# JGI-Bioinformatics/Kmernator

Hardware: AMD Instinct MI355X
Metric: total k-mers/sec at k=31, 150 bp reads (spectrum build, inputs resident in HBM) (higher is better)
Workload: dtype u64

## Files before the change

### kmernator_amd/csrc/kmr_api.hip

```cpp
#include <hip/hip_runtime.h>
#include <dlfcn.h>
#include <unistd.h>
#include <rccl/rccl.h>

#include <algorithm>
#include <atomic>
#include <cmath>
#include <cstdio>
#include <cstdlib>
#include <cstring>
#include <cctype>
#include <memory>
#include <string>
#include <type_traits>
#include <vector>

#include "../../include/kmernator_amd.h"
#include "kmr_kernels.hpp"
#include "kmr_partition.hpp"
#include "kmr_ingest.hpp"
#include "kmr_artifact.hpp"
#include "kmr_select.hpp"
#include "kmr_pairs.hpp"
#include "kmr_dump.hpp"
#include "kmr_superkmer.hpp"
#include "kmr_buckets.hpp"
#include "kmr_synth.hpp"
#define KMR_INSTANCES_EXTERN
#include "kmr_instances.hpp"

using namespace kmr;

namespace {

std::string g_create_error;

thread_local char g_oom_note[160] = "";
std::atomic<long long> g_blocks_live{0};
hipError_t dev_malloc(void **p, size_t bytes) {
	hipError_t e = hipMalloc(p, bytes);
	if (e == hipSuccess) { if (*p) g_blocks_live++; return e; }
	if (e != hipErrorOutOfMemory) return e;
	size_t fr = 0, tot = 0;
	for (int attempt = 0; attempt < 6; attempt++) {
		(void)hipGetLastError();
		hipDeviceSynchronize();
		if (hipMemGetInfo(&fr, &tot) != hipSuccess || bytes > tot) break;
		usleep(20000u << attempt);
		e = hipMalloc(p, bytes);
		if (e == hipSuccess && *p) g_blocks_live++;
		if (e != hipErrorOutOfMemory) return e;
	}
	(void)hipGetLastError();
	hipMemGetInfo(&fr, &tot);
	snprintf(g_oom_note, sizeof(g_oom_note), " [requested %.3f GB; device has %.3f GB free of %.3f GB]", bytes / 1e9, fr / 1e9, tot / 1e9);
	*p = nullptr;
	return hipErrorOutOfMemory;
}

class DevBuf {
public:
	DevBuf() = default;
	DevBuf(DevBuf &&o) noexcept : p_(o.p_), cap_(o.cap_) { o.p_ = nullptr; o.cap_ = 0; }
	DevBuf &operator=(DevBuf &&o) noexcept { if (this != &o) { reset(); std::swap(p_, o.p_); std::swap(cap_, o.cap_); } return *this; }
	~DevBuf() { reset(); }
	void reset() { if (p_) { hipFree(p_); g_blocks_live--; } p_ = nullptr; cap_ = 0; }
	hipError_t alloc(size_t bytes) {
		reset();
		void *p = nullptr;
		const hipError_t e = dev_malloc(&p, bytes);
		if (e == hipSuccess) { p_ = p; cap_ = bytes; }
		return e;
	}
	int reserve(kmr_handle *h, const char *what, size_t need, size_t bytes = 0);
	template <class T = void> T *get() const { return (T *)p_; }
	size_t cap() const { return cap_; }
	explicit operator bool() const { return p_ != nullptr; }
private:
	void *p_ = nullptr;
	size_t cap_ = 0;
};

struct DevMap {
	uint64_t nb = 0, n = 0;
	DevBuf start;
	DevBuf keys;
	DevBuf vals;
	DevBuf sweight;
	DevBuf spkt;
	DevBuf image;
	bool present = false;
};

struct HostPool {
	DevBuf base, chunk_list, chunk_count, head;
	uint32_t cap = 0; size_t chunk_bytes = 0;
	uint64_t used_ub = 0;
	uint64_t presize = 0;
};

struct HandleMem {
	DevBuf slots, extslots;
	DevBuf dP, dstats, derr;
	DevMap weak, sing;
	DevBuf ix_start, ix_keys, ix_counts;
	DevBuf scratch_stats;
	DevBuf adopt_buf;
	DevBuf trk;
	DevBuf scan_sums;
	DevBuf score_buf;
	DevBuf lut;
	DevBuf dPk;
	DevBuf d_uni;
	DevBuf qrange;
	DevBuf sk_fine_state;
	struct Early { bool active = false; uint64_t hi = 0; uint32_t min_depth = 0; DevBuf ue, cursor, fc, err; } early;
	DevBuf xo_dev;
};
struct BuildMem {
	DevBuf sk_state;
	HostPool l1;
	DevBuf work_counter;
	DevBuf l1_state; bool l1_state_dirty = false;
	DevBuf arena; size_t arena_used = 0, arena_want = 0; std::vector<DevBuf> arena_overflow;
	DevBuf linear;
	DevBuf tile_count, kcap, koff;
	DevBuf ucnt, ufirst, u_start, u_end, u_read, umax;
	DevBuf tb_bases, tb_quals, tb_rel, tb_off, tb_len;
	uint64_t tb_quals_filled = 0; int tb_quals_char = -1;
	DevBuf tb_stage[2][8];
	DevBuf uw_keys, uw_vals, us_keys, us_b8, us_pkt;
	DevBuf ue, ue2;
};
struct ExchangeMem {
	DevBuf xc_small, xc_dcounts;
	DevBuf xc_send, xc_send2, xc_recv, xc_recv2;
};

}

struct Tuning {
	uint64_t target_list = 2048;
	uint64_t sub_batch_bases = 0;
	int recycle = -1;
	int part_blocks = 0;
	double entry_share = -1.0;
	double early_entry_share = -1.0;
	uint64_t saturated_batch_bytes = 0;
	bool no_lut = false, no_narrow = false, no_l1_state = false, no_stream_lookups = false;
	uint64_t long_list_chunks = 0;
	uint64_t binned_min = 1ull << 18;
	uint64_t twobit_piece_bases = 0;
	uint64_t list_aim = 0;
	bool pow2_lists = false;
	bool no_packed_direct = false;
	bool no_uniform_count = false;
	bool no_lean_extract = false;
	bool exchange_fail_once = false;
	uint64_t dump_piece_bytes = 0;
	bool dump_timing = false;
	bool select_timing = false;
	bool pairs_timing = false;
	uint32_t pair_hash_bits = 64;
	bool no_coarse_lists = true;
};

struct kmr_handle : HandleMem, BuildMem, ExchangeMem {
	kmr_config cfg;
	Tuning tune;
	uint32_t k = 0, kb = 0, hkb = 0, W = 0;
	bool ext = false;
	int device = 0, ncu = 0;
	hipStream_t stream = nullptr;
	std::string err;
	uint32_t log2cap = 0;
	uint64_t occupied = 0;
	uint64_t pending_kmers = 0;
	uint64_t stream_base = 0, reads = 0;
	uint64_t nb_weak = 0, nb_sing = 0;
	bool finalized = false, has_singletons = true;
	kmr_handle *subtract = nullptr;
	uint64_t subtracted = 0;
	kmr_stats stats;
	bool partition_mode = false;
	bool superkmer_mode = false;
	uint64_t ix_lists = 0, ix_gen = ~0ull;
	uint64_t trk_n = 0; std::vector<uint64_t> trk_elems;
	long trk_next = 128; uint64_t trk_raw = 0, trk_good = 0; std::vector<unsigned long long> trk_bounds; std::vector<uint64_t> trk_snap_raw, trk_snap_good;
	bool sk_fast_div = false;
	bool sender_launch = false;
	bool sk_exchange = false;
	bool auto_mode = false;
	int bits1 = 0;
	uint64_t inserted_records = 0;
	uint64_t call_bases_hint = 0;
	uint32_t lut_log2 = 0;
	uint64_t lut_gen = ~0ull, map_gen = 0;
	hipStream_t tb_copy_stream = nullptr; hipEvent_t tb_ready[2] = {nullptr, nullptr}, tb_consumed[2] = {nullptr, nullptr}; bool tb_set_used[2] = {false, false};
	const SkPacked *packed_direct = nullptr;
	int uniform_q_hint = -1;
	uint32_t sk_bits = 0, sk_m = 0, sk_off = 0, sk_win = 0;
	double hP[256], hPk[256];
	uint32_t sk_uni_w = 0xffffffffu; bool sk_uni_mixed = false; bool last_count_uniform = false;
	uint32_t peer_uni_w = 0xffffffffu; bool peer_uni_mixed = false, peers_declare = false;
	uint64_t xr_lo = 0, xr_hi = ~0ull;
	uint64_t last_early_hi = 0, last_early_entries = 0;
	bool last_early_overflowed = false;
	double last_score_ms = 0, last_select_ms = 0, last_write_ms = 0;
	double last_dump_size_ms = 0, last_dump_write_ms = 0;
	double last_pairs_ms = 0, last_pairs_parse_ms = 0, last_pairs_sort_ms = 0;
	uint64_t last_pair_hash_collisions = 0;
	uint64_t last_saturated_keys = 0, last_saturated_batches = 0;
	bool qual_mixed = false;
	uint32_t sk_fine_shift = 0;
	uint32_t sk_min_override = 0;
	uint64_t xo_segcap = 0; std::vector<uint64_t> xo_counts; const void *xo_batch = nullptr; uint64_t xo_first = 0;
	void *xc_comm = nullptr; kmr_transport xc_tr = {nullptr, nullptr, nullptr};
	uint64_t xc_job_bases = 0, xc_bytes_to_peers = 0;
	hipEvent_t ev0 = nullptr, ev1 = nullptr;
	double ms[KMR_TIME_GROUPS] = {0};
	uint64_t launches[KMR_TIME_GROUPS] = {0};
	std::vector<std::pair<hipEvent_t, hipEvent_t> > pending_events[KMR_TIME_GROUPS];
};

struct kmr_picks {
	int device = 0;
	DevBuf text, picked;
	uint64_t n = 0, n_picked = 0, bytes = 0;
};

struct kmr_pairs {
	int device = 0;
	DevBuf mate, read1, read2;
	uint64_t n = 0, n_pairs = 0, n_full = 0, n_seq = 0, n_conflicts = 0;
};

struct kmr_text {
	int device = 0;
	DevBuf text;
	uint64_t kept = 0, bytes = 0;
};

struct kmr_reads {
	int device = 0;
	DevBuf bases, quals;
	DevBuf offsets;
	DevBuf name_off, name_len;
	uint64_t n = 0, total = 0, filtered = 0;
	uint32_t input_base = 0;
};

namespace {

std::string oom_note() { std::string s(g_oom_note); g_oom_note[0] = 0; return s; }

std::string hip_err_text(hipError_t e) { return std::string(hipGetErrorString(e)) + (e == hipErrorOutOfMemory ? oom_note() : std::string()); }

#define HIPCHK(h, call) do { hipError_t e_ = (call); if (e_ != hipSuccess) { \
	(h)->err = std::string(#call) + ": " + hip_err_text(e_); \
	return e_ == hipErrorOutOfMemory ? KMR_ERR_OOM : KMR_ERR_HIP; } } while (0)

int DevBuf::reserve(kmr_handle *h, const char *what, size_t need, size_t bytes) {
	if (p_ && cap_ >= need) return 0;
	if (!bytes) bytes = need;
	hipError_t e = p_ ? hipStreamSynchronize(h->stream) : hipSuccess;
	if (e == hipSuccess) e = alloc(bytes);
	if (e == hipSuccess) return 0;
	h->err = std::string("device buffer ") + what + " (" + std::to_string(bytes) + " bytes): " + hip_err_text(e);
	return e == hipErrorOutOfMemory ? KMR_ERR_OOM : KMR_ERR_HIP;
}

#ifdef KMR_DEBUG_HOOKS
bool dbg() { static const bool d = getenv("KMR_DEBUG") != nullptr; return d; }
#else
constexpr bool dbg() { return false; }
#endif

int fail(kmr_handle *h, int code, const std::string &msg) { const std::string m = code == KMR_ERR_OOM ? msg + oom_note() : msg; if (h) h->err = m; else g_create_error = m; return code; }

uint64_t min_pow2(uint64_t n) {
	uint64_t p = n;
	if (p == 0) p = 1;
	else if ((p & (p - 1)) != 0) { p--; for (size_t i = 1; i < 64; i <<= 1) p |= p >> i; p++; }
	return p;
}
uint64_t resize_buckets(uint64_t n) { if (n > 67108864ull) n = 67108864ull; return min_pow2(n); }

void quality_table(double P[256], unsigned minQ, unsigned startChar) {
	for (int raw = 0; raw < 256; raw++) {
		int i = raw - (int)startChar + 33;
		if (i < 33 + (int)minQ) P[raw] = 0.0;
		else if (i < 103) P[raw] = 1.0 - pow(10.0, ((33 - i) / 10.0));
		else P[raw] = 1.0;
	}
}

template <int N> using int_c = std::integral_constant<int, N>;
template <class F> auto with_w(const kmr_handle *h, F &&f) {
	switch (h->W) { case 1: return f(int_c<1>()); case 2: return f(int_c<2>()); case 3: return f(int_c<3>()); default: return f(int_c<4>()); }
}
template <class F> auto with_w_ext(const kmr_handle *h, F &&f) {
	return with_w(h, [&](auto W) { return h->ext ? f(W, std::true_type()) : f(W, std::false_type()); });
}
template <int W, class F> auto with_win(uint32_t win, F &&f) {
	if (W > 1 && win == 32) return f(int_c<(W > 1 ? 32 : 16)>());
	return win == 16 ? f(int_c<16>()) : (win == 8 ? f(int_c<8>()) : f(int_c<4>()));
}

size_t slot_bytes(kmr_handle *h) { return with_w(h, [](auto W) { return sizeof(Slot<W()>); }); }

ReadsView reads_view(const void *bases, const void *quals, const void *offsets, uint64_t n_reads, const void *discarded = nullptr, uint64_t stream_base = 0, uint64_t first_read_idx = 0) {
	ReadsView rv{};
	rv.bases = (const uint8_t *)bases; rv.quals = (const uint8_t *)quals; rv.offsets = (const uint64_t *)offsets; rv.discarded = (const uint8_t *)discarded;
	rv.n_reads = n_reads; rv.stream_base = stream_base; rv.first_read_idx = first_read_idx;
	return rv;
}
ReadsView reads_slice(const ReadsView &all, uint64_t r, uint64_t m) {
	ReadsView rv = all;
	rv.offsets = all.offsets + r; rv.n_reads = m; rv.discarded = all.discarded ? all.discarded + r : nullptr; rv.first_read_idx = all.first_read_idx + r;
	return rv;
}
FinalizeParams finalize_params(kmr_handle *h, uint32_t min_depth) {
	FinalizeParams f{};
	f.kb = h->hkb; f.ext_min_q = h->cfg.ext_min_quality; f.min_depth = min_depth; f.has_singletons = h->cfg.separate_singletons ? 1 : 0; f.nb_weak = h->nb_weak; f.nb_sing = h->nb_sing;
	return f;
}

DevParams dev_params(kmr_handle *h) {
	DevParams p;
	p.k = h->k; p.kb = h->hkb; p.min_weight = h->cfg.min_weight; p.fastq_start = h->cfg.fastq_start_char; p.ext_min_q = h->cfg.ext_min_quality;
	p.qzero = h->cfg.fastq_start_char + std::max<uint32_t>(1u, h->cfg.min_quality_score);
	p.subsample = h->cfg.kmer_subsample; p.rank = h->cfg.rank; p.world = h->cfg.world_size; p.num_parts = h->cfg.num_parts; p.part_idx = h->cfg.part_idx;
	p.count_sender_bad = h->sender_launch ? 1u : 0u;
	p.P = h->dP.get<double>(); p.stats = h->dstats.get<DevStats>(); p.err = h->derr.get<uint32_t>();
	p.sub_wstart = p.sub_wkeys = p.sub_sstart = p.sub_skeys = nullptr; p.sub_wvals = nullptr; p.sub_sweight = nullptr; p.sub_wnb = p.sub_snb = 0; p.sub_vw = 0;
	if (h->subtract) {
		const kmr_handle *o = h->subtract;
		if (o->weak.present && o->weak.n) { p.sub_wstart = o->weak.start.get<uint64_t>(); p.sub_wkeys = o->weak.keys.get<uint64_t>(); p.sub_wvals = o->weak.vals.get<uint32_t>(); p.sub_wnb = o->weak.nb; p.sub_vw = o->ext ? 15 : 3; }
		if (o->sing.present && o->sing.n) { p.sub_sstart = o->sing.start.get<uint64_t>(); p.sub_skeys = o->sing.keys.get<uint64_t>(); p.sub_sweight = o->sing.sweight.get<uint8_t>(); p.sub_snb = o->sing.nb; }
	}
	return p;
}

int grid_for(uint64_t n, int block = 256, int maxBlocks = 256 * 16) {
	uint64_t g = (n + block - 1) / block;
	if (g < 1) g = 1;
	if (g > (uint64_t)maxBlocks) g = maxBlocks;
	return (int)g;
}

template <int W> Table<W> table_of(kmr_handle *h) { Table<W> t; t.slots = h->slots.get<Slot<W>>(); t.ext = h->extslots.get<ExtSlot>(); t.log2cap = h->log2cap; return t; }

template <int W> int clear_table(kmr_handle *h, void *slots, ExtSlot *ext, uint32_t log2cap) {
	hipLaunchKernelGGL(table_clear_kernel<W>, dim3(grid_for(1ull << log2cap)), dim3(256), 0, h->stream, (Slot<W> *)slots, ext, 1ull << log2cap);
	HIPCHK(h, hipGetLastError());
	return 0;
}
int clear_table_any(kmr_handle *h, void *slots, ExtSlot *ext, uint32_t log2cap) { return with_w(h, [&](auto W) { return clear_table<W()>(h, slots, ext, log2cap); }); }

int alloc_table(kmr_handle *h, uint32_t log2cap, DevBuf &slots, DevBuf &ext) {
	DevBuf s, x;
	HIPCHK(h, s.alloc(slot_bytes(h) << log2cap));
	if (h->ext) HIPCHK(h, x.alloc(sizeof(ExtSlot) << log2cap));
	const int rc = clear_table_any(h, s.get(), x.get<ExtSlot>(), log2cap);
	if (rc) return rc;
	slots = std::move(s); ext = std::move(x);
	return 0;
}

int sync_state(kmr_handle *h) {
	HIPCHK(h, hipStreamSynchronize(h->stream));
	for (int which = 0; which < KMR_TIME_GROUPS; which++) {
		for (auto &pr : h->pending_events[which]) {
			float ms = 0; hipEventElapsedTime(&ms, pr.first, pr.second);
			h->ms[which] += ms; h->launches[which]++;
			hipEventDestroy(pr.first); hipEventDestroy(pr.second);
		}
		h->pending_events[which].clear();
	}
	uint32_t e = 0; DevStats s;
	HIPCHK(h, hipMemcpy(&e, h->derr.get<uint32_t>(), sizeof(e), hipMemcpyDeviceToHost));
	HIPCHK(h, hipMemcpy(&s, h->dstats.get<DevStats>(), sizeof(s), hipMemcpyDeviceToHost));
#ifdef KMR_DEBUG_HOOKS
	if (h->superkmer_mode) { if (dbg()) fprintf(stderr, "sk_extract windows: %llu general, %llu fast\n", s.claimed, s.inserted); s.claimed = 0; s.inserted = 0; }
#endif
	h->stats.raw_kmers = s.raw + s.inserted + s.sender_bad; h->stats.raw_good_kmers = s.good + s.inserted; h->stats.discarded = s.raw - s.good + s.sender_bad;
	h->occupied = s.claimed; h->pending_kmers = 0; h->subtracted = s.subtracted;
	if (e & ERR_READ_TOO_LONG) return fail(h, KMR_ERR_UNSUPPORTED, "a read is longer than the per-wavefront LDS tile (" + std::to_string(TILE_SPAN) + " bases)");
	if (e & ERR_TABLE_FULL) return fail(h, KMR_ERR_CAPACITY, "device k-mer table is full; raise kmr_config.max_table_entries / estimated_raw_kmers");
	if (e & ERR_SEGMENT_OVERFLOW) return fail(h, KMR_ERR_CAPACITY, "an owner segment overflowed seg_capacity");
	if (e & ERR_POOL_FULL) return fail(h, KMR_ERR_CAPACITY, "record pool overflow (internal sizing error)");
	if (e & ERR_ENTRIES_FULL) return fail(h, KMR_ERR_CAPACITY, "entry buffer overflow (internal sizing error)");
	return 0;
}

template <int W, bool EXT> int grow_table_t(kmr_handle *h, uint32_t newlog) {
	DevBuf ns, ne;
	int rc = alloc_table(h, newlog, ns, ne);
	if (rc) return rc;
	Table<W> src = table_of<W>(h), dst; dst.slots = ns.get<Slot<W>>(); dst.ext = ne.get<ExtSlot>(); dst.log2cap = newlog;
	hipLaunchKernelGGL((rehash_kernel<W, EXT>), dim3(grid_for(1ull << h->log2cap)), dim3(256), 0, h->stream, src, dst, h->hkb, h->derr.get<uint32_t>());
	HIPCHK(h, hipGetLastError());
	HIPCHK(h, hipStreamSynchronize(h->stream));
	h->slots = std::move(ns); h->extslots = std::move(ne); h->log2cap = newlog;
	return 0;
}
int grow_table(kmr_handle *h, uint32_t newlog) { return with_w_ext(h, [&](auto W, auto EXT) { return grow_table_t<W(), EXT()>(h, newlog); }); }

int ensure_capacity(kmr_handle *h, uint64_t incoming) {
	const uint64_t cap = 1ull << h->log2cap;
	if ((double)(h->occupied + h->pending_kmers + incoming) <= 0.85 * (double)cap) { h->pending_kmers += incoming; return 0; }
	int rc = sync_state(h);
	if (rc) return rc;
	if ((double)(h->occupied + incoming) > 0.85 * (double)cap) {
		uint32_t nl = h->log2cap;
		while ((double)(h->occupied + incoming) > 0.6 * (double)(1ull << nl)) nl++;
		rc = grow_table(h, nl);
		if (rc) return rc;
	}
	h->pending_kmers = incoming;
	return 0;
}

void time_begin(kmr_handle *h, int which, hipEvent_t *a, hipEvent_t *b) {
	hipEventCreate(a); hipEventCreate(b);
	hipEventRecord(*a, h->stream);
	(void)which;
}
void time_end(kmr_handle *h, int which, hipEvent_t a, hipEvent_t b) {
	hipEventRecord(b, h->stream);
	h->pending_events[which].push_back(std::make_pair(a, b));
}

const size_t EXTRACT_SMEM = (size_t)WAVES_PER_BLOCK * 2 * TILE_BUF;

int exclusive_scan(kmr_handle *h, const uint32_t *in, uint64_t n, uint64_t *out);

int prepare_units(kmr_handle *h, ReadsView &rv, uint32_t span = (uint32_t)TILE_SPAN) {
	rv.u_start = rv.u_end = rv.u_read = nullptr; rv.n_units = 0;
	const uint64_t n = rv.n_reads;
	if (n == 0) return 0;
	int rc = h->umax.reserve(h, "umax", 4); if (rc) return rc;
	HIPCHK(h, hipMemsetAsync(h->umax.get<unsigned int>(), 0, 4, h->stream));
	rc = h->ucnt.reserve(h, "ucnt", 4 * (n + 1)); if (rc) return rc;
	hipLaunchKernelGGL(unit_count_kernel, dim3(grid_for(n)), dim3(256), 0, h->stream, rv.offsets, n, h->k, span, h->ucnt.get<uint32_t>(), h->umax.get<unsigned int>());
	HIPCHK(h, hipGetLastError());
	unsigned int mx = 0;
	HIPCHK(h, hipMemcpyAsync(&mx, h->umax.get<unsigned int>(), 4, hipMemcpyDeviceToHost, h->stream));
	HIPCHK(h, hipStreamSynchronize(h->stream));
	if (mx <= span) return 0;
	rc = h->ufirst.reserve(h, "ufirst", 8 * (n + 1)); if (rc) return rc;
	rc = exclusive_scan(h, h->ucnt.get<uint32_t>(), n, h->ufirst.get<uint64_t>()); if (rc) return rc;
	uint64_t U = 0;
	HIPCHK(h, hipMemcpy(&U, h->ufirst.get<uint64_t>() + n, 8, hipMemcpyDeviceToHost));
	if (h->u_read.cap() < 8 * U) {
		h->u_start.reset(); h->u_end.reset(); h->u_read.reset();
		HIPCHK(h, h->u_start.alloc(8 * U)); HIPCHK(h, h->u_end.alloc(8 * U)); HIPCHK(h, h->u_read.alloc(8 * U));
	}
	hipLaunchKernelGGL(unit_fill_kernel, dim3(grid_for(n)), dim3(256), 0, h->stream, rv.offsets, n, h->k, span, h->ufirst.get<uint64_t>(), h->u_start.get<uint64_t>(), h->u_end.get<uint64_t>(), h->u_read.get<uint64_t>());
	HIPCHK(h, hipGetLastError());
	rv.u_start = h->u_start.get<uint64_t>(); rv.u_end = h->u_end.get<uint64_t>(); rv.u_read = h->u_read.get<uint64_t>(); rv.n_units = U;
	return 0;
}

template <int W, bool EXT, class Op> int launch_extract(kmr_handle *h, const ReadsView &rv, const Op &op, uint64_t max_blocks = 0) {
	const DevParams dp = dev_params(h);
	const bool sub = Op::NEEDS_WEIGHT && (dp.sub_wnb | dp.sub_snb) != 0;
	auto kern = sub ? extract_kernel<W, EXT, Op, true> : extract_kernel<W, EXT, Op, false>;
	HIPCHK(h, hipFuncSetAttribute((const void *)kern, hipFuncAttributeMaxDynamicSharedMemorySize, (int)EXTRACT_SMEM));
	if (dbg()) { int nb = 0; hipOccupancyMaxActiveBlocksPerMultiprocessor(&nb, (const void *)kern, WAVES_PER_BLOCK * 64, EXTRACT_SMEM); fprintf(stderr, "extract: %d blocks of %d waves per CU (dynamic LDS %zu)\n", nb, WAVES_PER_BLOCK, EXTRACT_SMEM);
		for (size_t tr : {(size_t)79872, (size_t)65536, (size_t)52000, (size_t)38000}) { hipOccupancyMaxActiveBlocksPerMultiprocessor(&nb, (const void *)kern, WAVES_PER_BLOCK * 64, tr); fprintf(stderr, "   with %zu bytes: %d blocks\n", tr, nb); } }
	const uint64_t tiles = ((rv.u_start ? rv.n_units : rv.n_reads) + 63) / 64;
	uint64_t blocks = (tiles + WAVES_PER_BLOCK - 1) / WAVES_PER_BLOCK;
	if (blocks == 0) return 0;
	if (max_blocks && blocks > max_blocks) blocks = max_blocks;
	if (blocks > 0x7fffffffull) return fail(h, KMR_ERR_INVALID_ARG, "too many reads in one batch");
	hipLaunchKernelGGL(kern, dim3((unsigned)blocks), dim3(WAVES_PER_BLOCK * 64), EXTRACT_SMEM, h->stream, rv, dp, op);
	HIPCHK(h, hipGetLastError());
	return 0;
}

template <int W, bool EXT> int add_reads_dev_t(kmr_handle *h, const ReadsView &rvAll, uint64_t total_bases) {
	const uint64_t n = rvAll.n_reads;
	const uint64_t avg = n ? std::max<uint64_t>(1, total_bases / n) : 1;
	uint64_t chunk = std::max<uint64_t>(64, ((1ull << 27) / avg) & ~63ull);
	std::vector<uint64_t> off2(2);
	for (uint64_t r = 0; r < n; r += chunk) {
		const uint64_t m = std::min(chunk, n - r);
		HIPCHK(h, hipMemcpyAsync(&off2[0], rvAll.offsets + r, 8, hipMemcpyDeviceToHost, h->stream));
		HIPCHK(h, hipMemcpyAsync(&off2[1], rvAll.offsets + r + m, 8, hipMemcpyDeviceToHost, h->stream));
		HIPCHK(h, hipStreamSynchronize(h->stream));
		const uint64_t bases = off2[1] - off2[0];
		int rc = ensure_capacity(h, bases);
		if (rc) return rc;
		ReadsView rv = reads_slice(rvAll, r, m);
		rc = prepare_units(h, rv); if (rc) return rc;
		InsertOp<W, EXT> op; op.table = table_of<W>(h);
		hipEvent_t a, b; time_begin(h, 0, &a, &b);
		rc = launch_extract<W, EXT>(h, rv, op);
		time_end(h, 0, a, b);
		if (rc) return rc;
	}
	return 0;
}

int add_reads_dev_any(kmr_handle *h, const ReadsView &rv, uint64_t total_bases) { return with_w_ext(h, [&](auto W, auto EXT) { return add_reads_dev_t<W(), EXT()>(h, rv, total_bases); }); }

int exclusive_scan(kmr_handle *h, const uint32_t *in, uint64_t n, uint64_t *out ) {
	const uint64_t nblocks = (n + SCAN_ITEMS - 1) / SCAN_ITEMS;
	const size_t eb = sizeof(unsigned long long);
	int rc = h->scan_sums.reserve(h, "scan_sums", eb * (nblocks + 1), eb * std::max<uint64_t>(nblocks + 1, 4096)); if (rc) return rc;
	unsigned long long *sums = h->scan_sums.get<unsigned long long>(), *total = sums + nblocks;
	hipLaunchKernelGGL(scan_block_sums_kernel, dim3((unsigned)nblocks), dim3(256), 0, h->stream, in, n, sums);
	hipLaunchKernelGGL(scan_sums_kernel, dim3(1), dim3(256), 0, h->stream, sums, nblocks, total);
	hipLaunchKernelGGL(scan_apply_kernel, dim3((unsigned)nblocks), dim3(256), 0, h->stream, in, n, sums, out);
	HIPCHK(h, hipGetLastError());
	HIPCHK(h, hipStreamSynchronize(h->stream));
	return 0;
}

int arena_alloc(kmr_handle *h, void **out, size_t bytes) {
	const size_t need = (bytes + 255) & ~(size_t)255;
	if (h->arena && h->arena_used + need <= h->arena.cap()) { *out = h->arena.get<uint8_t>() + h->arena_used; h->arena_used += need; h->arena_want += need; return 0; }
	h->arena_want += need;
	DevBuf b;
	HIPCHK(h, b.alloc(std::max<size_t>(need, 256)));
	*out = b.get();
	h->arena_overflow.push_back(std::move(b));
	return 0;
}
int arena_reset(kmr_handle *h) {
	HIPCHK(h, hipStreamSynchronize(h->stream));
	h->arena_overflow.clear();
	if (h->arena_want > h->arena.cap()) {
		if (h->arena.alloc(h->arena_want + h->arena_want / 8 + (1 << 20)) != hipSuccess) (void)hipGetLastError();
	}
	h->arena_used = 0; h->arena_want = 0;
	return 0;
}
template <class T> int arena_get(kmr_handle *h, T **out, size_t count) { return arena_alloc(h, (void **)out, count * sizeof(T)); }

void clear_map(DevMap &m) { m.image.reset(); m.n = 0; m.present = false; }


template <int W> MapView<W> view_of(const DevMap &m, uint32_t vw) {
	MapView<W> v; v.start = m.start.get<uint64_t>(); v.keys = m.keys.get<uint64_t>(); v.vals = m.vals.get<uint32_t>(); v.sweight = m.sweight.get<uint8_t>(); v.nb = m.present ? m.nb : 0; v.vw = vw;
	return v;
}

template <int W, bool EXT> int finalize_t(kmr_handle *h, uint32_t min_depth) {
	int rc = sync_state(h);
	if (rc) return rc;
	hipEvent_t ea, eb; time_begin(h, 1, &ea, &eb);
	const FinalizeParams f = finalize_params(h, min_depth);
	const bool keepSing = f.has_singletons && min_depth <= 1;
	DevBuf wcb, scb, fcb;
	HIPCHK(h, wcb.alloc(4 * h->nb_weak)); HIPCHK(h, scb.alloc(4 * h->nb_sing)); HIPCHK(h, fcb.alloc(sizeof(FinalizeCounters)));
	uint32_t *wc = wcb.get<uint32_t>(), *sc = scb.get<uint32_t>(); FinalizeCounters *fc = fcb.get<FinalizeCounters>();
	HIPCHK(h, hipMemsetAsync(wc, 0, 4 * h->nb_weak, h->stream)); HIPCHK(h, hipMemsetAsync(sc, 0, 4 * h->nb_sing, h->stream)); HIPCHK(h, hipMemsetAsync(fc, 0, sizeof(FinalizeCounters), h->stream));
	Table<W> t = table_of<W>(h);
	const int g = grid_for(1ull << h->log2cap);
	hipLaunchKernelGGL(classify_kernel<W>, dim3(g), dim3(256), 0, h->stream, t, f, wc, sc, fc);
	HIPCHK(h, hipGetLastError());
	FinalizeCounters c;
	HIPCHK(h, hipMemcpyAsync(&c, fc, sizeof(c), hipMemcpyDeviceToHost, h->stream));
	HIPCHK(h, hipStreamSynchronize(h->stream));
	h->stats.unique_kmers = c.unique;
	h->stats.singleton_kmers = f.has_singletons ? c.singletons : 0;
	DevMap &wm = h->weak, &sm = h->sing;
	wm = DevMap(); sm = DevMap();
	wm.nb = h->nb_weak; wm.n = c.weak_kept; wm.present = true;
	sm.nb = h->nb_sing; sm.n = c.sing_kept; sm.present = keepSing;
	const uint32_t vw = EXT ? 15 : 3;
	HIPCHK(h, wm.start.alloc(8 * (wm.nb + 1))); HIPCHK(h, sm.start.alloc(8 * (sm.nb + 1)));
	rc = exclusive_scan(h, wc, wm.nb, wm.start.get<uint64_t>()); if (rc) return rc;
	rc = exclusive_scan(h, sc, sm.nb, sm.start.get<uint64_t>()); if (rc) return rc;
	HIPCHK(h, wm.keys.alloc(std::max<uint64_t>(8, 8ull * W * wm.n))); HIPCHK(h, wm.vals.alloc(std::max<uint64_t>(8, 4ull * vw * wm.n)));
	HIPCHK(h, sm.keys.alloc(std::max<uint64_t>(8, 8ull * W * sm.n))); HIPCHK(h, sm.sweight.alloc(std::max<uint64_t>(8, sm.n)));
	if (EXT) HIPCHK(h, sm.spkt.alloc(std::max<uint64_t>(8, 4ull * sm.n)));
	HIPCHK(h, hipMemsetAsync(wc, 0, 4 * h->nb_weak, h->stream)); HIPCHK(h, hipMemsetAsync(sc, 0, 4 * h->nb_sing, h->stream));
	hipLaunchKernelGGL((scatter_kernel<W, EXT>), dim3(g), dim3(256), 0, h->stream, t, f, wm.start.get<uint64_t>(), wc, wm.keys.get<uint64_t>(), wm.vals.get<uint32_t>(), sm.start.get<uint64_t>(), sc, sm.keys.get<uint64_t>(), sm.sweight.get<uint8_t>(), sm.spkt.get<uint32_t>());
	HIPCHK(h, hipGetLastError());
	SortView<W> sv; sv.keys = wm.keys.get<uint64_t>(); sv.vals = wm.vals.get<uint32_t>(); sv.b8 = nullptr; sv.pkt = nullptr; sv.vw = vw;
	hipLaunchKernelGGL((sort_buckets_kernel<W, EXT ? 15 : 3>), dim3(grid_for(wm.nb, 4, 1 << 20)), dim3(256), 0, h->stream, sv, wm.start.get<uint64_t>(), wm.nb);
	if (sm.n) {
		SortView<W> ss; ss.keys = sm.keys.get<uint64_t>(); ss.vals = nullptr; ss.b8 = sm.sweight.get<uint8_t>(); ss.pkt = sm.spkt.get<uint32_t>(); ss.vw = 0;
		hipLaunchKernelGGL((sort_buckets_kernel<W, 0>), dim3(grid_for(sm.nb, 4, 1 << 20)), dim3(256), 0, h->stream, ss, sm.start.get<uint64_t>(), sm.nb);
	}
	HIPCHK(h, hipGetLastError());
	time_end(h, 1, ea, eb);
	HIPCHK(h, hipStreamSynchronize(h->stream));
	h->has_singletons = keepSing;
	if (!keepSing) { sm.n = 0; }
	h->stats.weak_entries = wm.n; h->stats.singleton_entries = keepSing ? sm.n : 0;
	h->finalized = true; h->map_gen++;
	return sync_state(h);
}

template <int W> int build_image_t(kmr_handle *h, DevMap &m, bool weakMap) {
	if (m.image) return 0;
	const uint32_t vw = h->ext ? 15 : 3;
	const uint32_t vbytes = weakMap ? (h->ext ? 60 : 12) : (h->ext ? 5 : 1);
	HIPCHK(h, m.image.alloc(8 * (2 + m.nb) + 4 * m.nb + m.n * (h->kb + vbytes)));
	hipLaunchKernelGGL(image_header_kernel, dim3(grid_for(m.nb)), dim3(256), 0, h->stream, m.image.get<uint8_t>(), m.start.get<uint64_t>(), m.nb, h->kb, vbytes);
	if (m.n) hipLaunchKernelGGL(image_entries_kernel<W>, dim3(grid_for(m.n)), dim3(256), 0, h->stream, m.image.get<uint8_t>(), m.start.get<uint64_t>(), m.nb, h->kb, vbytes,
	                           m.keys.get<uint64_t>(), weakMap ? m.vals.get<uint32_t>() : nullptr, vw, m.sweight.get<uint8_t>(), m.spkt.get<uint32_t>(), m.n);
	HIPCHK(h, hipGetLastError());
	HIPCHK(h, hipStreamSynchronize(h->stream));
	return 0;
}
int build_image(kmr_handle *h, DevMap &m, bool weakMap) { return with_w(h, [&](auto W) { return build_image_t<W()>(h, m, weakMap); }); }

template <int W> int load_image_t(kmr_handle *h, DevMap &m, bool weakMap, const uint8_t *src, uint64_t len) {
	if (len < 16) return fail(h, KMR_ERR_INVALID_ARG, "image too short");
	uint64_t nb, mask; memcpy(&nb, src, 8); memcpy(&mask, src + 8, 8);
	if (nb == 0 || (nb & (nb - 1)) || mask != nb - 1 || len < 8 * (2 + nb) + 4 * nb) return fail(h, KMR_ERR_INVALID_ARG, "bad image header");
	const uint32_t vw = h->ext ? 15 : 3;
	const uint32_t vbytes = weakMap ? (h->ext ? 60 : 12) : (h->ext ? 5 : 1);
	if ((len - 8 * (2 + nb) - 4 * nb) % (h->kb + vbytes) != 0) return fail(h, KMR_ERR_INVALID_ARG, "image size does not match k / value type");
	m = DevMap();
	m.nb = nb; m.n = (len - 8 * (2 + nb) - 4 * nb) / (h->kb + vbytes); m.present = true;
	const uint64_t *offs = (const uint64_t *)(src + 16);
	uint64_t expect = 8 * (2 + nb);
	for (uint64_t b = 0; b < nb; b++) {
		if (offs[b] != expect || expect + 4 > len) return fail(h, KMR_ERR_INVALID_ARG, "image offsets are not the packed store() layout");
		uint32_t cnt; memcpy(&cnt, src + expect, 4);
		expect += 4 + (uint64_t)cnt * (h->kb + vbytes);
		if (expect > len) return fail(h, KMR_ERR_INVALID_ARG, "image bucket runs past the end");
	}
	if (expect != len) return fail(h, KMR_ERR_INVALID_ARG, "image length mismatch");
	HIPCHK(h, m.image.alloc(len));
	HIPCHK(h, hipMemcpy(m.image.get<uint8_t>(), src, len, hipMemcpyHostToDevice));
	{
		DevBuf counts; HIPCHK(h, counts.alloc(4 * nb));
		hipLaunchKernelGGL(image_counts_kernel, dim3(grid_for(nb)), dim3(256), 0, h->stream, m.image.get<uint8_t>(), nb, counts.get<uint32_t>());
		HIPCHK(h, m.start.alloc(8 * (nb + 1)));
		int rc = exclusive_scan(h, counts.get<uint32_t>(), nb, m.start.get<uint64_t>()); if (rc) return rc;
	}
	HIPCHK(h, m.keys.alloc(std::max<uint64_t>(8, 8ull * W * m.n)));
	if (weakMap) HIPCHK(h, m.vals.alloc(std::max<uint64_t>(8, 4ull * vw * m.n)));
	else { HIPCHK(h, m.sweight.alloc(std::max<uint64_t>(8, m.n))); if (h->ext) HIPCHK(h, m.spkt.alloc(std::max<uint64_t>(8, 4 * m.n))); }
	if (m.n) hipLaunchKernelGGL(image_unpack_kernel<W>, dim3(grid_for(m.n)), dim3(256), 0, h->stream, m.image.get<uint8_t>(), m.start.get<uint64_t>(), nb, h->kb, vbytes, m.keys.get<uint64_t>(), m.vals.get<uint32_t>(), vw, m.sweight.get<uint8_t>(), m.spkt.get<uint32_t>(), m.n);
	SortView<W> sv; sv.keys = m.keys.get<uint64_t>(); sv.vals = m.vals.get<uint32_t>(); sv.b8 = m.sweight.get<uint8_t>(); sv.pkt = m.spkt.get<uint32_t>(); sv.vw = weakMap ? vw : 0;
	if (!weakMap) hipLaunchKernelGGL((sort_buckets_kernel<W, 0>), dim3(grid_for(nb, 4, 1 << 20)), dim3(256), 0, h->stream, sv, m.start.get<uint64_t>(), nb);
	else if (h->ext) hipLaunchKernelGGL((sort_buckets_kernel<W, 15>), dim3(grid_for(nb, 4, 1 << 20)), dim3(256), 0, h->stream, sv, m.start.get<uint64_t>(), nb);
	else hipLaunchKernelGGL((sort_buckets_kernel<W, 3>), dim3(grid_for(nb, 4, 1 << 20)), dim3(256), 0, h->stream, sv, m.start.get<uint64_t>(), nb);
	HIPCHK(h, hipGetLastError());
	HIPCHK(h, hipStreamSynchronize(h->stream));
	m.image.reset();

	return 0;
}

template <int W, int VW> void launch_sort(kmr_handle *h, DevMap &m, bool weakMap) {
	SortView<W> sv; sv.keys = m.keys.get<uint64_t>(); sv.vals = weakMap ? m.vals.get<uint32_t>() : nullptr; sv.b8 = m.sweight.get<uint8_t>(); sv.pkt = m.spkt.get<uint32_t>(); sv.vw = weakMap ? VW : 0;
	hipLaunchKernelGGL((sort_buckets_kernel<W, VW>), dim3(grid_for(m.nb, 4, 1 << 20)), dim3(256), 0, h->stream, sv, m.start.get<uint64_t>(), m.nb);
}
template <int W> int merge_image_t(kmr_handle *h, DevMap &m, bool weakMap, const uint8_t *src, uint64_t len) {
	DevMap t;
	int rc = load_image_t<W>(h, t, weakMap, src, len);
	if (rc) return rc;
	if (t.nb != m.nb) return fail(h, KMR_ERR_INVALID_ARG, "Can not merge two maps of differing sizes (src/Kmer.h:3210)");
	const uint32_t vw = h->ext ? 15 : 3;
	DevMap d; d.nb = m.nb; d.n = m.n + t.n; d.present = true;
	DevBuf countsb, dupb;
	HIPCHK(h, countsb.alloc(4 * m.nb)); HIPCHK(h, dupb.alloc(4));
	uint32_t *counts = countsb.get<uint32_t>(), *dup = dupb.get<uint32_t>();
	HIPCHK(h, hipMemsetAsync(dup, 0, 4, h->stream));
	HIPCHK(h, d.start.alloc(8 * (m.nb + 1)));
	hipLaunchKernelGGL(merge_counts_kernel, dim3(grid_for(m.nb)), dim3(256), 0, h->stream, m.start.get<uint64_t>(), t.start.get<uint64_t>(), m.nb, counts);
	rc = exclusive_scan(h, counts, m.nb, d.start.get<uint64_t>()); if (rc) return rc;
	HIPCHK(h, d.keys.alloc(std::max<uint64_t>(8, 8ull * W * d.n)));
	if (weakMap) HIPCHK(h, d.vals.alloc(std::max<uint64_t>(8, 4ull * vw * d.n)));
	else { HIPCHK(h, d.sweight.alloc(std::max<uint64_t>(8, d.n))); if (h->ext) HIPCHK(h, d.spkt.alloc(std::max<uint64_t>(8, 4 * d.n))); }
	if (m.n) hipLaunchKernelGGL(merge_copy_kernel<W>, dim3(grid_for(m.n)), dim3(256), 0, h->stream, m.start.get<uint64_t>(), t.start.get<uint64_t>(), false, m.nb, m.n, m.keys.get<uint64_t>(), weakMap ? m.vals.get<uint32_t>() : nullptr, vw, m.sweight.get<uint8_t>(), m.spkt.get<uint32_t>(), d.start.get<uint64_t>(), d.keys.get<uint64_t>(), d.vals.get<uint32_t>(), d.sweight.get<uint8_t>(), d.spkt.get<uint32_t>());
	if (t.n) hipLaunchKernelGGL(merge_copy_kernel<W>, dim3(grid_for(t.n)), dim3(256), 0, h->stream, t.start.get<uint64_t>(), m.start.get<uint64_t>(), true, m.nb, t.n, t.keys.get<uint64_t>(), weakMap ? t.vals.get<uint32_t>() : nullptr, vw, t.sweight.get<uint8_t>(), t.spkt.get<uint32_t>(), d.start.get<uint64_t>(), d.keys.get<uint64_t>(), d.vals.get<uint32_t>(), d.sweight.get<uint8_t>(), d.spkt.get<uint32_t>());
	if (!weakMap) launch_sort<W, 0>(h, d, false); else if (h->ext) launch_sort<W, 15>(h, d, true); else launch_sort<W, 3>(h, d, true);
	hipLaunchKernelGGL(duplicate_keys_kernel<W>, dim3(grid_for(d.nb)), dim3(256), 0, h->stream, d.start.get<uint64_t>(), d.nb, d.keys.get<uint64_t>(), dup);
	HIPCHK(h, hipGetLastError());
	uint32_t hdup = 0;
	HIPCHK(h, hipMemcpyAsync(&hdup, dup, 4, hipMemcpyDeviceToHost, h->stream)); HIPCHK(h, hipStreamSynchronize(h->stream));
	if (hdup && !weakMap) return fail(h, KMR_ERR_UNSUPPORTED, "the two singleton maps share k-mers: merging them means promoting those into the weak map (mergePromote, which the reference refuses too)");
	if (hdup) {
		DevMap d2; d2.nb = d.nb; d2.present = true;
		hipLaunchKernelGGL(merge_distinct_kernel<W>, dim3(grid_for(d.nb)), dim3(256), 0, h->stream, d.start.get<uint64_t>(), d.nb, d.keys.get<uint64_t>(), counts);
		HIPCHK(h, d2.start.alloc(8 * (d.nb + 1)));
		rc = exclusive_scan(h, counts, d.nb, d2.start.get<uint64_t>()); if (rc) return rc;
		HIPCHK(h, hipMemcpyAsync(&d2.n, d2.start.get<uint64_t>() + d.nb, 8, hipMemcpyDeviceToHost, h->stream)); HIPCHK(h, hipStreamSynchronize(h->stream));
		HIPCHK(h, d2.keys.alloc(std::max<uint64_t>(8, 8ull * W * d2.n)));
		HIPCHK(h, d2.vals.alloc(std::max<uint64_t>(8, 4ull * vw * d2.n)));
		hipLaunchKernelGGL(merge_add_kernel<W>, dim3(grid_for(d.nb)), dim3(256), 0, h->stream, d.start.get<uint64_t>(), d.nb, d.keys.get<uint64_t>(), d.vals.get<uint32_t>(), vw, d2.start.get<uint64_t>(), d2.keys.get<uint64_t>(), d2.vals.get<uint32_t>());
		HIPCHK(h, hipGetLastError()); HIPCHK(h, hipStreamSynchronize(h->stream));
		d = std::move(d2);
	}
	m = std::move(d);
	return 0;
}

template <int W> int lookup_t(kmr_handle *h, const uint8_t *packed, uint64_t n, uint32_t *counts, double *weights = nullptr) {
	const uint64_t ob = counts ? 4 : 8;
	DevBuf dk, dc;
	HIPCHK(h, dk.alloc(std::max<uint64_t>(8, n * h->kb))); HIPCHK(h, dc.alloc(std::max<uint64_t>(8, ob * n)));
	HIPCHK(h, hipMemcpyAsync(dk.get(), packed, n * h->kb, hipMemcpyHostToDevice, h->stream));
	const uint32_t vw = h->ext ? 15 : 3;
	hipLaunchKernelGGL(lookup_keys_kernel<W>, dim3(grid_for(n)), dim3(256), 0, h->stream, view_of<W>(h->weak, vw), view_of<W>(h->sing, vw), dk.get<uint8_t>(), n, h->hkb,
	                   counts ? dc.get<uint32_t>() : nullptr, counts ? nullptr : dc.get<double>());
	HIPCHK(h, hipGetLastError());
	HIPCHK(h, hipMemcpyAsync(counts ? (void *)counts : (void *)weights, dc.get(), ob * n, hipMemcpyDeviceToHost, h->stream));
	HIPCHK(h, hipStreamSynchronize(h->stream));
	return 0;
}

template <int W> LutView<W> lut_of(kmr_handle *h) {
	LutView<W> v; v.slots = nullptr; v.mask = 0; v.shift = 0;
	if (h->tune.no_lut || !h->weak.present || h->weak.n == 0) return v;
	if (!(h->lut && h->lut_gen == h->map_gen)) {
		uint32_t l2 = 10; while ((1ull << l2) < 2 * h->weak.n) l2++;
		const size_t bytes = (size_t)(W + 1) * 8 << l2;
		if (h->lut.cap() < bytes) {
			if (h->lut) { hipStreamSynchronize(h->stream); h->lut.reset(); }
			size_t fr = 0, tot = 0;
			if (hipMemGetInfo(&fr, &tot) != hipSuccess || fr < bytes + (1ull << 30) || h->lut.alloc(bytes) != hipSuccess) { (void)hipGetLastError(); return v; }
		}

		const uint32_t vw = h->ext ? 15 : 3;
		hipLaunchKernelGGL(lut_clear_kernel, dim3(4096), dim3(256), 0, h->stream, h->lut.get<uint64_t>(), 1ull << l2, (uint32_t)(W + 1));
		hipLaunchKernelGGL(lut_build_kernel<W>, dim3(grid_for(h->weak.n)), dim3(256), 0, h->stream, view_of<W>(h->weak, vw), h->weak.n, h->lut.get<uint64_t>(), (1ull << l2) - 1, 64 - l2, h->hkb);
		if (hipGetLastError() != hipSuccess) return v;
		h->lut_log2 = l2; h->lut_gen = h->map_gen;
	}
	v.slots = h->lut.get<uint64_t>(); v.mask = (1ull << h->lut_log2) - 1; v.shift = 64 - h->lut_log2;
	return v;
}

template <int W> int lookup_reads_t(kmr_handle *h, const ReadsView &rv, uint32_t *dout, const uint64_t *dout_off, bool weak_only = false) {
	LookupOp<W> op; const uint32_t vw = h->ext ? 15 : 3; op.weak_only = weak_only;
	op.lut = weak_only ? lut_of<W>(h) : LutView<W>{nullptr, 0, 0};
	op.weak = view_of<W>(h->weak, vw); op.sing = view_of<W>(h->sing, vw); op.out = dout; op.out_offsets = dout_off; op.first_read_idx = rv.first_read_idx;
	return launch_extract<W, false>(h, rv, op);
}
template <int W> int lookup_reads_weighted_t(kmr_handle *h, const ReadsView &rv, double *dout, const uint64_t *dout_off) {
	LookupWeightOp<W> op; const uint32_t vw = h->ext ? 15 : 3;
	op.weak = view_of<W>(h->weak, vw); op.sing = view_of<W>(h->sing, vw); op.out = dout; op.out_offsets = dout_off; op.first_read_idx = rv.first_read_idx;
	return launch_extract<W, false>(h, rv, op);
}

int stage_reads(kmr_handle *h, const char *bases, const uint64_t *offsets, uint64_t n, DevBuf &b, DevBuf &o) {
	const uint64_t total = n ? offsets[n] - offsets[0] : 0;
	HIPCHK(h, b.alloc(total + 64)); HIPCHK(h, o.alloc(8 * (n + 1)));
	HIPCHK(h, hipMemcpyAsync(b.get(), bases + (n ? offsets[0] : 0), total, hipMemcpyHostToDevice, h->stream));
	std::vector<uint64_t> rel(n + 1);
	for (uint64_t i = 0; i <= n; i++) rel[i] = n ? offsets[i] - offsets[0] : 0;
	HIPCHK(h, hipMemcpyAsync(o.get(), rel.data(), 8 * (n + 1), hipMemcpyHostToDevice, h->stream));
	HIPCHK(h, hipStreamSynchronize(h->stream));
	return 0;
}


#define TARGET_LIST_RECORDS (h->tune.target_list)
const double MAX_LIST_DISTINCT = 600.0;
const uint64_t L2_ITEM_CHUNKS = 16384;
const uint64_t SUB_BATCH_BASES = 1ull << 30;

size_t rec_bytes(kmr_handle *h) { return h->superkmer_mode ? 16 : 8 * h->W + (h->ext ? 16 : 8); }
uint64_t key_entries(kmr_handle *h, const DevBuf &keys) { return keys.cap() / (8ull * h->W); }
uint64_t packed_entries(kmr_handle *h, const DevBuf &ue) { return ue.cap() / (8ull * (h->W + 1)); }
int max_part_bits(kmr_handle *h) { return rec_bytes(h) <= 24 ? 10 : 9; }
PoolView pool_view(kmr_handle *h, HostPool &p) { PoolView v; v.base = p.base.get<uint8_t>(); v.chunk_list = p.chunk_list.get<uint32_t>(); v.chunk_count = p.chunk_count.get<uint32_t>(); v.head = p.head.get<unsigned int>(); v.cap = p.cap; v.err = h->derr.get<uint32_t>(); return v; }
uint32_t part_rot(kmr_handle *h) { uint32_t r = 0; while ((1ull << (r + 1)) <= h->nb_weak) r++; return r; }
template <int W, bool EXT, int LEVEL> int launch_partition(kmr_handle *h, const PartSource<W> &S, HostPool &pool, int grid, int bits, int shift) {
	auto kern = partition_direct_kernel<W, EXT, LEVEL, PD_THREADS, PD_RPT, PD_LINE>;
	const size_t smem = partition_direct_smem_bytes<W, EXT, PD_THREADS, PD_RPT, PD_LINE>(bits);
	if (dbg()) fprintf(stderr, "partition level %d W=%d bits=%d shift=%d smem=%zu grid=%d\n", LEVEL, W, bits, shift, smem, grid);
	HIPCHK(h, hipFuncSetAttribute((const void *)kern, hipFuncAttributeMaxDynamicSharedMemorySize,
	                              (int)partition_direct_smem_bytes<W, EXT, PD_THREADS, PD_RPT, PD_LINE>(max_part_bits(h))));
	hipLaunchKernelGGL(kern, dim3(grid), dim3(PD_THREADS), smem, h->stream, S, pool_view(h, pool), h->work_counter.get<unsigned int>(), bits, shift);
	HIPCHK(h, hipGetLastError());
	return 0;
}

int pool_reserve(kmr_handle *h, HostPool &p, uint64_t extra, bool keep) {
	unsigned int used = 0;
	if (!keep) p.used_ub = 0;
	if (p.head && keep) {
		if (p.base && p.used_ub + extra + 64 <= p.cap) { p.used_ub += extra; return 0; }
		HIPCHK(h, hipStreamSynchronize(h->stream)); HIPCHK(h, hipMemcpy(&used, p.head.get<unsigned int>(), 4, hipMemcpyDeviceToHost)); if (used > p.cap) used = p.cap;
	}
	p.used_ub = (uint64_t)used + extra;
	const uint64_t need = (uint64_t)used + extra + 64;
	if (need >= 0xffffffffull) return fail(h, KMR_ERR_CAPACITY, "record pool would exceed 2^32 chunks");
	if (!p.head) { HIPCHK(h, p.head.alloc(4)); HIPCHK(h, hipMemset(p.head.get(), 0, 4)); }
	if (!keep) HIPCHK(h, hipMemsetAsync(p.head.get<unsigned int>(), 0, 4, h->stream));
	if (need <= p.cap) return 0;
	uint64_t ncap = keep && used ? need + need / 4 : need;
	if (p.presize && need + p.presize < 0xffffffffull) ncap = std::max(ncap, need + p.presize);
	p.presize = 0;
	p.chunk_bytes = (size_t)CH * rec_bytes(h);
	DevBuf nb, nl, nc;
	HIPCHK(h, nb.alloc(ncap * p.chunk_bytes));
	HIPCHK(h, nl.alloc(4 * ncap)); HIPCHK(h, nc.alloc(4 * ncap));
	if (used) {
		HIPCHK(h, hipMemcpy(nb.get(), p.base.get(), (size_t)used * p.chunk_bytes, hipMemcpyDeviceToDevice));
		HIPCHK(h, hipMemcpy(nl.get(), p.chunk_list.get(), 4ull * used, hipMemcpyDeviceToDevice));
		HIPCHK(h, hipMemcpy(nc.get(), p.chunk_count.get(), 4ull * used, hipMemcpyDeviceToDevice));
		HIPCHK(h, hipDeviceSynchronize());
	}
	p.base = std::move(nb); p.chunk_list = std::move(nl); p.chunk_count = std::move(nc); p.cap = (uint32_t)ncap;
	return 0;
}


int zero_work_counter(kmr_handle *h) {
	int rc = h->work_counter.reserve(h, "work_counter", 4); if (rc) return rc;
	HIPCHK(h, hipMemsetAsync(h->work_counter.get<unsigned int>(), 0, 4, h->stream));
	return 0;
}

int num_cus(kmr_handle *h) {
	if (h->ncu <= 0) {
		hipDeviceProp_t pr; h->ncu = 256;
		if (hipGetDeviceProperties(&pr, h->device) == hipSuccess) h->ncu = pr.multiProcessorCount;
	}
	return h->ncu;
}
int part_grid(kmr_handle *h) { return num_cus(h) * 2; }
int partition_blocks(kmr_handle *h) { return h->tune.part_blocks > 0 ? h->tune.part_blocks : num_cus(h); }

template <int W, bool EXT> int ensure_l1_state(kmr_handle *h) {
	const size_t stride = partition_state_bytes<W, EXT, PD_LINE>(h->bits1), need = stride * (size_t)partition_blocks(h);
	if (h->l1_state.cap() == need) return 0;
	if (h->l1_state) HIPCHK(h, hipStreamSynchronize(h->stream));
	HIPCHK(h, h->l1_state.alloc(need));
	hipLaunchKernelGGL(partition_state_init_kernel, dim3(partition_blocks(h)), dim3(256), 0, h->stream, h->l1_state.get<uint8_t>(), stride, h->bits1, (uint32_t)partition_blocks(h));
	HIPCHK(h, hipGetLastError());
	h->l1_state_dirty = false;
	return 0;
}
template <int W, bool EXT> int flush_l1_state(kmr_handle *h) {
	if (!h->l1_state || !h->l1_state_dirty) return 0;
	int rc = pool_reserve(h, h->l1, (uint64_t)partition_blocks(h) * ((1ull << h->bits1) + 512) + 64, true); if (rc) return rc;
	rc = zero_work_counter(h); if (rc) return rc;
	PartSource<W> S; memset(&S, 0, sizeof(S));
	S.kb = h->hkb; S.rot = part_rot(h); S.state = h->l1_state.get<uint8_t>(); S.state_final = 1;
	rc = launch_partition<W, EXT, 1>(h, S, h->l1, partition_blocks(h), h->bits1, 0);
	h->l1_state_dirty = false;
	return rc;
}

template <int W, bool EXT> int partition_level1(kmr_handle *h, const void *linear, const uint64_t *ext_start, const uint32_t *ext_count,
                                      uint64_t n_ext, uint32_t ext_stride, uint64_t ext_len, uint64_t total, uint64_t max_records,
                                      unsigned long long *valid_counter = nullptr, uint32_t packed_words = 0, uint64_t ordinal_base = 0) {
	if (n_ext == 0) return 0;
	const int grid = (int)std::min<uint64_t>(partition_blocks(h), n_ext);
	if (!h->l1.base) {
		const uint64_t est = std::max<uint64_t>(max_records, h->cfg.estimated_raw_kmers / std::max<uint32_t>(1, h->cfg.world_size));
		const uint64_t launches = est / std::max<uint64_t>(1, max_records) + 2;
		const uint64_t l2_allowance = (est / CH / L2_ITEM_CHUNKS + (1ull << h->bits1) + 1) * (1ull << max_part_bits(h)) + (uint64_t)part_grid(h) * 512;
		{
			const uint64_t chunks = est / CH + launches * (uint64_t)grid * ((1ull << h->bits1) + 512) + 64 + l2_allowance;
			size_t mfree = 0, mtotal = 0;
			if (hipMemGetInfo(&mfree, &mtotal) == hipSuccess && (double)mfree < (double)chunks * CH * rec_bytes(h) * 1.02 + (double)(2ull << 30)) {
				HIPCHK(h, hipStreamSynchronize(h->stream));
				h->uw_keys.reset(); h->uw_vals.reset(); h->us_keys.reset(); h->us_b8.reset(); h->us_pkt.reset(); h->ue.reset(); h->ue2.reset();
			}
		}
		uint64_t want = est / CH + launches * (uint64_t)grid * ((1ull << h->bits1) + 512) + 64 + l2_allowance;
		{
			size_t mfree = 0, mtotal = 0;
			const double twice = (double)(want + est / CH) * CH * rec_bytes(h) * 1.02;
			if (hipMemGetInfo(&mfree, &mtotal) == hipSuccess && twice + (double)(8ull << 30) < (double)mfree * 0.5) want += est / CH;
		}
		int rc0 = pool_reserve(h, h->l1, want, true);
		if (rc0) return rc0;
	}
	int rc = pool_reserve(h, h->l1, max_records / CH + (uint64_t)grid * ((1ull << h->bits1) + 512) + 64, true);
	if (rc) return rc;
	rc = zero_work_counter(h); if (rc) return rc;
	PartSource<W> S; memset(&S, 0, sizeof(S));
	S.linear = linear; S.ext_start = ext_start; S.ext_count = ext_count; S.n_ext = n_ext; S.ext_stride = ext_stride; S.ext_len = ext_len; S.total = total;
	S.valid_counter = valid_counter; S.kb = h->hkb; S.rot = part_rot(h); S.packed_words = packed_words; S.ordinal_base = ordinal_base;
	if (!h->tune.no_l1_state) {
		rc = ensure_l1_state<W, EXT>(h); if (rc) return rc;
		S.state = h->l1_state.get<uint8_t>(); S.state_final = 0; h->l1_state_dirty = true;
	}
	hipEvent_t ta, tb; time_begin(h, KMR_TIME_PARTITION1, &ta, &tb);
	rc = launch_partition<W, EXT, 1>(h, S, h->l1, grid, h->bits1, 0);
	time_end(h, KMR_TIME_PARTITION1, ta, tb);
	return rc;
}

void choose_bits1(kmr_handle *h, uint64_t records_hint) {
	uint64_t est = std::max<uint64_t>(records_hint, h->cfg.estimated_raw_kmers / std::max<uint32_t>(1, h->cfg.world_size));
	const int mb = max_part_bits(h);
	int T = 0; while (T < 2 * mb && (est >> T) > TARGET_LIST_RECORDS) T++;
	h->bits1 = std::max(0, std::min(mb, T + 2 - mb));
}

template <int W, bool EXT> int extract_by_owner_t(kmr_handle *h, const ReadsView &rvAll, uint64_t total_bases, void *dev_records, uint64_t seg_capacity, void *dev_seg_counts, uint32_t *dev_pos = nullptr) {
	const uint64_t n = rvAll.n_reads;
	const uint64_t avg = n ? std::max<uint64_t>(1, total_bases / n) : 1;
	const uint64_t chunk = std::max<uint64_t>(64, (SUB_BATCH_BASES / avg) & ~63ull);
	for (uint64_t r = 0; r < n; r += chunk) {
		const uint64_t m = std::min(chunk, n - r);
		ReadsView rv = reads_slice(rvAll, r, m);
		int rc = prepare_units(h, rv); if (rc) return rc;
		const uint64_t nu = rv.u_start ? rv.n_units : m;
		rc = h->kcap.reserve(h, "kcap", 4 * std::max<uint64_t>(nu + 1, 16)); if (rc) return rc;
		rc = h->koff.reserve(h, "koff", 8 * std::max<uint64_t>(nu + 1, 16)); if (rc) return rc;
		hipLaunchKernelGGL(kmer_capacity_kernel, dim3(grid_for(nu)), dim3(256), 0, h->stream, rv, h->k, h->kcap.get<uint32_t>());
		HIPCHK(h, hipGetLastError());
		rc = exclusive_scan(h, h->kcap.get<uint32_t>(), nu, h->koff.get<uint64_t>()); if (rc) return rc;
		uint64_t total_cap = 0;
		HIPCHK(h, hipMemcpy(&total_cap, h->koff.get<uint64_t>() + nu, 8, hipMemcpyDeviceToHost));
		const uint64_t tiles = (nu + 63) / 64;
		rc = h->linear.reserve(h, "linear", sizeof(typename PoolRec<W, EXT>::type) * std::max<uint64_t>(total_cap, 16)); if (rc) return rc;
		rc = h->tile_count.reserve(h, "tile_count", 4 * std::max<uint64_t>(tiles, 16)); if (rc) return rc;
		LinearOp<W, EXT, false> op; op.records = (typename PoolRec<W, EXT>::type *)h->linear.get(); op.koff = h->koff.get<uint64_t>(); op.tile_count = h->tile_count.get<uint32_t>(); op.first_read_idx = rv.first_read_idx;
		h->sender_launch = dev_pos == nullptr;
		rc = launch_extract<W, EXT>(h, rv, op);
		h->sender_launch = false;
		if (rc) return rc;
		rc = zero_work_counter(h); if (rc) return rc;
		const int grid = (int)std::min<uint64_t>((uint64_t)num_cus(h) * 8, tiles);
		OwnerFn of; of.m = 0; of.off = of.win = of.list_bits = 0;
		if (h->superkmer_mode && h->sk_exchange) { of.m = h->sk_m; of.off = h->sk_off; of.win = h->sk_win; of.list_bits = h->sk_bits; }
		if (dev_pos)
			hipLaunchKernelGGL((owner_scatter_kernel<W, EXT, true>), dim3(grid), dim3(OWNER_THREADS), 0, h->stream, (const typename PoolRec<W, EXT>::type *)h->linear.get(), h->koff.get<uint64_t>(), h->tile_count.get<uint32_t>(), tiles, h->hkb,
			                   h->cfg.world_size, (uint32_t *)dev_records, seg_capacity, (unsigned long long *)dev_seg_counts, h->work_counter.get<unsigned int>(), h->derr.get<uint32_t>(), dev_pos, of);
		else
			hipLaunchKernelGGL((owner_scatter_kernel<W, EXT>), dim3(grid), dim3(OWNER_THREADS), 0, h->stream, (const typename PoolRec<W, EXT>::type *)h->linear.get(), h->koff.get<uint64_t>(), h->tile_count.get<uint32_t>(), tiles, h->hkb,
			                   h->cfg.world_size, (uint32_t *)dev_records, seg_capacity, (unsigned long long *)dev_seg_counts, h->work_counter.get<unsigned int>(), h->derr.get<uint32_t>(), (uint32_t *)nullptr, of);
		HIPCHK(h, hipGetLastError());
	}
	return 0;
}

template <int W, bool EXT> int add_reads_partition_t(kmr_handle *h, const ReadsView &rvAll, uint64_t total_bases) {
	const uint64_t n = rvAll.n_reads;
	if (!h->l1.head) choose_bits1(h, total_bases);
	const uint64_t avg = n ? std::max<uint64_t>(1, total_bases / n) : 1;
	const uint64_t sub_bases = h->tune.sub_batch_bases ? h->tune.sub_batch_bases : SUB_BATCH_BASES;
	const uint64_t chunk = std::max<uint64_t>(64, (sub_bases / avg) & ~63ull);
	for (uint64_t r = 0; r < n; r += chunk) {
		const uint64_t m = std::min(chunk, n - r);
		ReadsView rv = reads_slice(rvAll, r, m);
		int rc = prepare_units(h, rv); if (rc) return rc;
		const uint64_t nu = rv.u_start ? rv.n_units : m;
		rc = h->kcap.reserve(h, "kcap", 4 * std::max<uint64_t>(nu + 1, 16)); if (rc) return rc;
		rc = h->koff.reserve(h, "koff", 8 * std::max<uint64_t>(nu + 1, 16)); if (rc) return rc;
		hipLaunchKernelGGL(kmer_capacity_kernel, dim3(grid_for(nu)), dim3(256), 0, h->stream, rv, h->k, h->kcap.get<uint32_t>());
		HIPCHK(h, hipGetLastError());
		rc = exclusive_scan(h, h->kcap.get<uint32_t>(), nu, h->koff.get<uint64_t>()); if (rc) return rc;
		uint64_t total_cap = 0;
		HIPCHK(h, hipMemcpy(&total_cap, h->koff.get<uint64_t>() + nu, 8, hipMemcpyDeviceToHost));
		const uint64_t tiles = (nu + 63) / 64;
		rc = h->linear.reserve(h, "linear", rec_bytes(h) * std::max<uint64_t>(total_cap, 16)); if (rc) return rc;
		rc = h->tile_count.reserve(h, "tile_count", 4 * std::max<uint64_t>(tiles, 16)); if (rc) return rc;
		LinearOp<W, EXT> op; op.records = (typename PoolRec<W, EXT>::type *)h->linear.get(); op.koff = h->koff.get<uint64_t>(); op.tile_count = h->tile_count.get<uint32_t>(); op.first_read_idx = rv.first_read_idx;
		hipEvent_t a, b, a2, b2; time_begin(h, KMR_TIME_BUILD, &a, &b);
		time_begin(h, KMR_TIME_EXTRACT, &a2, &b2);
		rc = launch_extract<W, EXT>(h, rv, op);
		time_end(h, KMR_TIME_EXTRACT, a2, b2);
#ifdef KMR_DEBUG_HOOKS
		if (!rc && getenv("KMR_DEBUG_SAME_TILE")) {
			const uint64_t distinct = std::max<uint64_t>(1, strtoull(getenv("KMR_DEBUG_SAME_TILE"), nullptr, 10));
			hipLaunchKernelGGL(same_tile_kernel, dim3(grid_for(tiles)), dim3(256), 0, h->stream, h->koff.get<uint64_t>(), tiles, distinct, total_cap / std::max<uint64_t>(tiles, 1));
		}
#endif
		if (!rc) rc = partition_level1<W, EXT>(h, h->linear.get(), h->koff.get<uint64_t>(), h->tile_count.get<uint32_t>(), tiles, 64, 0, 0, total_cap);
		time_end(h, KMR_TIME_BUILD, a, b);
		if (rc) return rc;
	}
	return 0;
}
int add_reads_partition(kmr_handle *h, const ReadsView &rv, uint64_t total_bases) { return with_w_ext(h, [&](auto W, auto EXT) { return add_reads_partition_t<W(), EXT()>(h, rv, total_bases); }); }

int build_csr(kmr_handle *h, HostPool &p, uint64_t nl, uint32_t first, uint64_t **list_start, uint64_t **list_chunks, uint32_t *n_chunks_out) {
	unsigned int used = 0;
	HIPCHK(h, hipStreamSynchronize(h->stream));
	HIPCHK(h, hipMemcpy(&used, p.head.get<unsigned int>(), 4, hipMemcpyDeviceToHost));
	if (used > p.cap) used = p.cap;
	used = used > first ? used - first : 0;
	uint32_t *cnt;
	{ int arc = arena_get(h, &cnt, nl); if (arc) return arc; arc = arena_get(h, list_start, nl + 1); if (arc) return arc;
	  arc = arena_get(h, list_chunks, std::max<unsigned>(used, 1)); if (arc) return arc; }
	HIPCHK(h, hipMemsetAsync(cnt, 0, 4 * nl, h->stream));
	const unsigned csr_grid = (unsigned)(((uint64_t)used + CSR_THREADS * CSR_ITEMS - 1) / (CSR_THREADS * CSR_ITEMS));
	if (used) hipLaunchKernelGGL(chunk_hist_kernel, dim3(csr_grid), dim3(CSR_THREADS), 0, h->stream, p.chunk_list.get<uint32_t>() + first, used, cnt, (uint32_t)nl);
	int rc = exclusive_scan(h, cnt, nl, *list_start); if (rc) return rc;
	HIPCHK(h, hipMemsetAsync(cnt, 0, 4 * nl, h->stream));
	if (used) hipLaunchKernelGGL(chunk_scatter_kernel, dim3(csr_grid), dim3(CSR_THREADS), 0, h->stream, p.chunk_list.get<uint32_t>() + first, p.chunk_count.get<uint32_t>() + first, used, first, *list_start, cnt, *list_chunks, (uint32_t)nl);
	HIPCHK(h, hipGetLastError());
	*n_chunks_out = used;
	if (dbg()) {
		unsigned long long hv[2] = {0, 0};
		DevBuf db; HIPCHK(h, db.alloc(16)); HIPCHK(h, hipMemset(db.get(), 0, 16));
		unsigned long long *d = db.get<unsigned long long>();
		if (used) hipLaunchKernelGGL(pool_records_kernel, dim3(grid_for(used)), dim3(256), 0, h->stream, p.chunk_list.get<uint32_t>(), p.chunk_count.get<uint32_t>(), used, d, d + 1);
		HIPCHK(h, hipStreamSynchronize(h->stream));
		HIPCHK(h, hipMemcpy(hv, d, 16, hipMemcpyDeviceToHost));
		fprintf(stderr, "build_csr: lists %llu chunks %u valid %llu records %llu (expected %llu)\n", (unsigned long long)nl, used, hv[1], hv[0], (unsigned long long)h->stats.raw_good_kmers);
		unsigned long long vv[3] = {0, 0, 0};
		int bits = 0; while ((1ull << bits) < nl) bits++;
		DevBuf vb; HIPCHK(h, vb.alloc(24)); HIPCHK(h, hipMemset(vb.get(), 0, 24));
		unsigned long long *v = vb.get<unsigned long long>();
		PoolView pvw = pool_view(h, p);
		with_w_ext(h, [&](auto W, auto EXT) { hipLaunchKernelGGL((verify_lists_kernel<W(), EXT()>), dim3(4096), dim3(256), 0, h->stream, pvw, *list_start, *list_chunks, nl, bits, h->hkb, part_rot(h), v, v + 1, v + 2); });
		HIPCHK(h, hipStreamSynchronize(h->stream));
		HIPCHK(h, hipMemcpy(vv, v, 24, hipMemcpyDeviceToHost));
		fprintf(stderr, "verify_lists: records via CSR %llu misfiled %llu zero-weight %llu\n", vv[0], vv[1], vv[2]);
	}
	return 0;
}

int finish_maps_from_entries(kmr_handle *h, uint32_t *wc, uint32_t *sc, uint64_t wslots, uint64_t sslots, uint64_t wn, uint64_t sn, bool keepSing, bool weak_uncounted = false);
CountOut count_out(kmr_handle *h, bool packed, unsigned long long *cursors, uint32_t *wc, uint32_t *sc, FinalizeCounters *fc);

template <int W, bool EXT, int LOG2S, bool NARROW = false> int launch_count(kmr_handle *h, int grid, const uint64_t *ls, const uint64_t *lc, uint64_t nl, const CountOut &out, const FinalizeParams &f, int list_filter) {
	auto kern = count_kernel<W, EXT, LOG2S, NARROW>;
	const size_t smem = count_smem_bytes<W, EXT, LOG2S, NARROW>();
	HIPCHK(h, hipFuncSetAttribute((const void *)kern, hipFuncAttributeMaxDynamicSharedMemorySize, (int)smem));
	hipLaunchKernelGGL(kern, dim3(grid), dim3(COUNT_THREADS), smem, h->stream, pool_view(h, h->l1), ls, lc, nl, out, f, h->work_counter.get<unsigned int>(), list_filter);
	return 0;
}

template <int W, bool EXT> int finalize_partition_t(kmr_handle *h, uint32_t min_depth) {
	int rc = sync_state(h);
	if (rc) return rc;
	hipEvent_t ea, eb; time_begin(h, 1, &ea, &eb);
	const uint64_t G = h->stats.raw_good_kmers;
	const FinalizeParams f = finalize_params(h, min_depth);
	const bool keepSing = f.has_singletons && min_depth <= 1;
	if (!h->l1.head) { rc = pool_reserve(h, h->l1, 0, false); if (rc) return rc; }
	rc = arena_reset(h); if (rc) return rc;
	rc = flush_l1_state<W, EXT>(h); if (rc) return rc;
	const uint64_t nl1 = 1ull << h->bits1;
	uint64_t *ls1 = nullptr; uint64_t *lc1 = nullptr; uint32_t nch1 = 0;
	rc = build_csr(h, h->l1, nl1, 0, &ls1, &lc1, &nch1); if (rc) return rc;
	double distinct_share = 1.0, repeated_share = 0.5;
	if (G) {
		unsigned long long *dpr, hpr[4] = {0, 0, 0, 0};
		const uint32_t n_probes = (uint32_t)std::min<uint64_t>(PROBE_LISTS, nl1);
		const size_t tbytes = 8 * ((size_t)n_probes * PROBE_SLOTS + 4);
		rc = arena_alloc(h, (void **)&dpr, tbytes); if (rc) return rc;
		HIPCHK(h, hipMemsetAsync(dpr, 0, tbytes, h->stream));
		hipLaunchKernelGGL((distinct_probe_kernel<W, EXT>), dim3(n_probes * PROBE_SPLIT), dim3(256), 0, h->stream, pool_view(h, h->l1), ls1, lc1, nl1, h->hkb, part_rot(h),
		                   (int)h->bits1, n_probes, dpr + 4, dpr);
		HIPCHK(h, hipGetLastError());
		HIPCHK(h, hipMemcpyAsync(hpr, dpr, 32, hipMemcpyDeviceToHost, h->stream)); HIPCHK(h, hipStreamSynchronize(h->stream));
		if (hpr[0] >= 256) { distinct_share = std::min(1.0, std::max(0.01, (double)hpr[1] / (double)hpr[0])); repeated_share = std::min(0.5, (double)hpr[2] / (double)hpr[0]); }
		if (dbg()) fprintf(stderr, "distinct probe: %llu records, %llu distinct (%llu repeated) -> shares %.3f %.3f\n", hpr[0], hpr[1], hpr[2], distinct_share, repeated_share);
	}
	const int mb = max_part_bits(h);
	int T = 0; while (T < 40 && ((G >> T) > TARGET_LIST_RECORDS || (double)(G >> T) * distinct_share > MAX_LIST_DISTINCT)) T++;
	T = std::min(T, 28);
	int cur_bits = h->bits1;
	uint64_t *ls2 = ls1, *lc2 = lc1;
	uint32_t valid_from = 0;
	for (int level = 2; cur_bits < T; level++) {
		const int nbits = std::min(mb, T - cur_bits);
		const uint64_t nl_prev = 1ull << cur_bits;
		std::vector<uint64_t> hs(nl_prev + 1);
		HIPCHK(h, hipMemcpy(hs.data(), ls2, 8 * (nl_prev + 1), hipMemcpyDeviceToHost));
		std::vector<uint64_t> ib, ie; std::vector<uint32_t> il;
		for (uint64_t l = 0; l < nl_prev; l++) {
			const uint64_t nch = hs[l + 1] - hs[l];
			if (!nch) continue;
			const uint64_t nit = (nch + L2_ITEM_CHUNKS - 1) / L2_ITEM_CHUNKS, per = (nch + nit - 1) / nit;
			for (uint64_t c = hs[l]; c < hs[l + 1]; c += per) { ib.push_back(c); ie.push_back(std::min(hs[l + 1], c + per)); il.push_back((uint32_t)l); }
		}
		if (ib.empty()) { cur_bits += nbits; rc = build_csr(h, h->l1, 1ull << cur_bits, valid_from, &ls2, &lc2, &nch1); if (rc) return rc; continue; }
		const uint64_t partials = ib.size() * (1ull << nbits) + (uint64_t)part_grid(h) * 512 + 64;
		unsigned int head_before = 0;
		HIPCHK(h, hipMemcpy(&head_before, h->l1.head.get<unsigned int>(), 4, hipMemcpyDeviceToHost));
		const bool recycle = h->tune.recycle >= 0 ? h->tune.recycle != 0 : (uint64_t)head_before + G / CH + partials + 64 > h->l1.cap;
		h->l1.used_ub = head_before;
		rc = pool_reserve(h, h->l1, (recycle ? 0 : G / CH) + partials, true); if (rc) return rc;
		uint64_t *dib, *die; uint32_t *dil;
		rc = arena_get(h, &dib, ib.size()); if (rc) return rc; rc = arena_get(h, &die, ie.size()); if (rc) return rc; rc = arena_get(h, &dil, il.size()); if (rc) return rc;
		HIPCHK(h, hipMemcpyAsync(dib, ib.data(), 8 * ib.size(), hipMemcpyHostToDevice, h->stream)); HIPCHK(h, hipMemcpyAsync(die, ie.data(), 8 * ie.size(), hipMemcpyHostToDevice, h->stream));
		HIPCHK(h, hipMemcpyAsync(dil, il.data(), 4 * il.size(), hipMemcpyHostToDevice, h->stream));
		rc = zero_work_counter(h); if (rc) return rc;
		PartSource<W> S; memset(&S, 0, sizeof(S));
		S.src = pool_view(h, h->l1); S.list_chunks = lc2; S.item_begin = dib; S.item_end = die; S.item_list = dil; S.n_items = ib.size(); S.kb = h->hkb; S.rot = part_rot(h);
		S.recycle = recycle ? 1 : 0;
		const int grid = (int)std::min<uint64_t>(partition_blocks(h), ib.size());
		if (dbg()) fprintf(stderr, "level %d: %d bits after %d, %zu items, %s\n", level, nbits, cur_bits, ib.size(), recycle ? "recycling chunks" : "fresh chunks");
		hipEvent_t ta, tb; time_begin(h, KMR_TIME_PARTITION2, &ta, &tb);
		rc = launch_partition<W, EXT, 2>(h, S, h->l1, grid, nbits, cur_bits);
		time_end(h, KMR_TIME_PARTITION2, ta, tb);
		if (rc) return rc;
		HIPCHK(h, hipStreamSynchronize(h->stream));
		cur_bits += nbits;
		if (!recycle) valid_from = head_before;
		rc = build_csr(h, h->l1, 1ull << cur_bits, valid_from, &ls2, &lc2, &nch1); if (rc) return rc;
	}
	const uint64_t nl2 = 1ull << cur_bits;
	const int count_log2s = (!EXT && (double)(G >> cur_bits) * distinct_share > MAX_LIST_DISTINCT) ? 11 : COUNT_LOG2S;
	if (dbg()) fprintf(stderr, "count pass: %llu lists of ~%llu records, table 2^%d\n", (unsigned long long)nl2, (unsigned long long)(G >> cur_bits), count_log2s);
	const uint32_t vw = EXT ? 15 : 3;
	const uint64_t slack = (uint64_t)part_grid(h) * 8 * 8192 + 16;
	const uint64_t wbound = f.has_singletons ? G / 2 : G, sbound = keepSing ? G : 0;
	const uint64_t wmax = wbound + wbound / 8 + slack, smax = keepSing ? sbound + sbound / 8 + slack : 16;
	uint64_t wcap = std::min<uint64_t>(wmax, (uint64_t)((double)G * (f.has_singletons ? repeated_share : distinct_share) * 1.5) + G / 64 + slack);
	uint64_t scap = keepSing ? std::min<uint64_t>(smax, (uint64_t)((double)G * std::max(0.0, distinct_share - repeated_share) * 1.5) + G / 64 + slack) : 16;
	if (h->tune.entry_share >= 0) {
		const double sh = h->tune.entry_share;
		wcap = std::min<uint64_t>(wmax, (uint64_t)((double)G * sh) + 16384); if (keepSing) scap = std::min<uint64_t>(smax, (uint64_t)((double)G * sh) + 16384);
		h->uw_keys.reset(); h->uw_vals.reset(); h->us_keys.reset(); h->us_b8.reset(); h->us_pkt.reset();
	}
	wcap = std::max(wcap, key_entries(h, h->uw_keys)); scap = std::max(scap, key_entries(h, h->us_keys));
	uint32_t *wc = nullptr, *sc = nullptr; FinalizeCounters *fc = nullptr; unsigned long long *cursors = nullptr;
	rc = arena_get(h, &wc, h->nb_weak); if (rc) return rc; rc = arena_get(h, &sc, h->nb_sing); if (rc) return rc;
	rc = arena_get(h, &fc, 1); if (rc) return rc; rc = arena_get(h, &cursors, 2); if (rc) return rc;
	FinalizeCounters c; unsigned long long cur[2];
	hipEvent_t tca, tcb; time_begin(h, KMR_TIME_COUNT, &tca, &tcb);
	for (int attempt = 0; ; attempt++) {
	{
		const double need = (key_entries(h, h->uw_keys) < wcap ? (8.0 * W + 4.0 * vw) * (double)wcap : 0.0) + (key_entries(h, h->us_keys) < scap ? (8.0 * W + 1.0) * (double)scap : 0.0);
		size_t mfree = 0, mtotal = 0;
		if (need > 0 && h->linear && hipMemGetInfo(&mfree, &mtotal) == hipSuccess && (double)mfree < need + (double)G * 0.3 * (8.0 * W + 12.0) + (double)(2ull << 30)) {
			HIPCHK(h, hipStreamSynchronize(h->stream));
			h->linear.reset();
		}
	}
	if (key_entries(h, h->uw_keys) < wcap || !h->uw_vals) {
		h->uw_keys.reset(); h->uw_vals.reset();
		HIPCHK(h, h->uw_keys.alloc(8ull * W * wcap)); HIPCHK(h, h->uw_vals.alloc(4ull * vw * wcap));
	}
	if (key_entries(h, h->us_keys) < scap || !h->us_b8 || (EXT && !h->us_pkt)) {
		h->us_keys.reset(); h->us_b8.reset(); h->us_pkt.reset();
		HIPCHK(h, h->us_keys.alloc(8ull * W * scap)); HIPCHK(h, h->us_b8.alloc(scap)); if (EXT) HIPCHK(h, h->us_pkt.alloc(4 * scap));
	}
	HIPCHK(h, hipMemsetAsync(wc, 0, 4 * h->nb_weak, h->stream)); HIPCHK(h, hipMemsetAsync(sc, 0, 4 * h->nb_sing, h->stream));
	HIPCHK(h, hipMemsetAsync(fc, 0, sizeof(FinalizeCounters), h->stream)); HIPCHK(h, hipMemsetAsync(cursors, 0, 16, h->stream));
	const CountOut out = count_out(h, false, cursors, wc, sc, fc);
	rc = zero_work_counter(h); if (rc) return rc;
	#ifdef KMR_DEBUG_HOOKS
	const int count_reps = getenv("KMR_COUNT_CHECK") ? atoi(getenv("KMR_COUNT_CHECK")) : 0;
#else
	const int count_reps = 0;
#endif
	for (int cr = 0; cr <= count_reps; cr++) {
		if (cr) {
			FinalizeCounters c0; unsigned long long cur0[2];
			HIPCHK(h, hipStreamSynchronize(h->stream));
			HIPCHK(h, hipMemcpy(&c0, fc, sizeof(c0), hipMemcpyDeviceToHost)); HIPCHK(h, hipMemcpy(cur0, cursors, 16, hipMemcpyDeviceToHost));
			fprintf(stderr, "count pass %d: unique %llu singletons %llu weak_kept %llu sing_kept %llu slots %llu/%llu\n", cr - 1, (unsigned long long)c0.unique,
			        (unsigned long long)c0.singletons, (unsigned long long)c0.weak_kept, (unsigned long long)c0.sing_kept, cur0[0], cur0[1]);
			HIPCHK(h, hipMemsetAsync(wc, 0, 4 * h->nb_weak, h->stream)); HIPCHK(h, hipMemsetAsync(sc, 0, 4 * h->nb_sing, h->stream));
			HIPCHK(h, hipMemsetAsync(fc, 0, sizeof(FinalizeCounters), h->stream)); HIPCHK(h, hipMemsetAsync(cursors, 0, 16, h->stream));
			rc = zero_work_counter(h); if (rc) return rc;
		}
		const int grid = (int)std::min<uint64_t>((uint64_t)part_grid(h) * 2, nl2);
		if (count_log2s == 11) {
			rc = launch_count<W, EXT, 11>(h, grid, ls2, lc2, nl2, out, f, 0); if (rc) return rc;
		} else if (EXT && W == 1 && !h->tune.no_narrow) {
			rc = launch_count<W, EXT, COUNT_LOG2S, true>(h, grid, ls2, lc2, nl2, out, f, 1); if (rc) return rc;
			HIPCHK(h, hipGetLastError());
			rc = zero_work_counter(h); if (rc) return rc;
			hipLaunchKernelGGL(max_list_chunks_kernel, dim3(grid_for(nl2)), dim3(256), 0, h->stream, ls2, nl2, h->work_counter.get<unsigned int>());
			unsigned int longest = 0;
			HIPCHK(h, hipMemcpyAsync(&longest, h->work_counter.get<unsigned int>(), 4, hipMemcpyDeviceToHost, h->stream));
			HIPCHK(h, hipStreamSynchronize(h->stream));
			rc = zero_work_counter(h); if (rc) return rc;
			if (longest > COUNT_NARROW_CHUNKS) { rc = launch_count<W, EXT, COUNT_LOG2S>(h, std::min(grid, part_grid(h)), ls2, lc2, nl2, out, f, 2); if (rc) return rc; }
		} else {
			rc = launch_count<W, EXT, COUNT_LOG2S>(h, grid, ls2, lc2, nl2, out, f, 0); if (rc) return rc;
		}
		HIPCHK(h, hipGetLastError());
	}
	uint32_t cerr = 0;
	HIPCHK(h, hipMemcpyAsync(&c, fc, sizeof(c), hipMemcpyDeviceToHost, h->stream)); HIPCHK(h, hipMemcpyAsync(cur, cursors, 16, hipMemcpyDeviceToHost, h->stream));
	HIPCHK(h, hipMemcpyAsync(&cerr, h->derr.get<uint32_t>(), 4, hipMemcpyDeviceToHost, h->stream));
	HIPCHK(h, hipStreamSynchronize(h->stream));
	if (!(cerr & ERR_ENTRIES_FULL) || (wcap >= wmax && scap >= smax) || attempt >= 8) break;
	cerr &= ~(uint32_t)ERR_ENTRIES_FULL;
	HIPCHK(h, hipMemcpy(h->derr.get<uint32_t>(), &cerr, 4, hipMemcpyHostToDevice));
	wcap = std::min<uint64_t>(wmax, wcap * 2); if (keepSing) scap = std::min<uint64_t>(smax, scap * 2);
	if (dbg()) fprintf(stderr, "count pass: entry buffers too small, retrying with %llu / %llu\n", (unsigned long long)wcap, (unsigned long long)scap);
	}
	time_end(h, KMR_TIME_COUNT, tca, tcb);
	{
		uint32_t cerr2 = 0;
		HIPCHK(h, hipMemcpy(&cerr2, h->derr.get<uint32_t>(), 4, hipMemcpyDeviceToHost));
		if (cerr2 & ERR_ENTRIES_FULL) { time_end(h, 1, ea, eb); return fail(h, KMR_ERR_CAPACITY, "entry buffers of the count pass overflowed at their upper bound (internal sizing error)"); }
	}

	h->stats.unique_kmers = c.unique;
	h->stats.singleton_kmers = f.has_singletons ? c.singletons : 0;
	hipEvent_t tma, tmb; time_begin(h, KMR_TIME_BUCKETS, &tma, &tmb);
	rc = finish_maps_from_entries(h, wc, sc, cur[0], cur[1], c.weak_kept, c.sing_kept, keepSing);
	time_end(h, KMR_TIME_BUCKETS, tma, tmb);
	if (rc) return rc;
	time_end(h, 1, ea, eb);
	h->has_singletons = keepSing;
	h->stats.weak_entries = h->weak.n; h->stats.singleton_entries = keepSing ? h->sing.n : 0;
	h->finalized = true; h->map_gen++;
	rc = sync_state(h);
	if (!rc && !h->arena_overflow.empty()) rc = arena_reset(h);
	return rc;
}

template <int W> int binned_buckets_t(kmr_handle *h, uint64_t wslots, uint64_t wn, bool &done) {
	done = false;
	DevMap &wm = h->weak;
	const uint64_t nb = wm.nb;
	uint32_t B = 0; while ((1ull << (B + 1)) <= nb) B++;
	if (h->ext || wn < h->tune.binned_min || wn == 0 || (1ull << B) != nb || wslots >= (1ull << 40)) return 0;
	uint32_t g = 0; while (g < std::min<uint32_t>(B, BB_MAX_GROUP_BITS) && (wn >> (B - g)) < 512) g++;
	const uint32_t R = B - g;
	if (R < 1 || R > 2 * BB_MAX_BITS || (wn >> R) > 1024) return 0;
	const uint32_t bits1 = R <= (uint32_t)BB_MAX_BITS ? R : (R + 1) / 2, bits2 = R - bits1;
	const uint64_t bins1 = 1ull << bits1, groups = 1ull << R;
	uint32_t *hist1 = nullptr, *hist2 = nullptr, *pad1 = nullptr; uint64_t *start1 = nullptr, *gstart = nullptr; unsigned long long *cursor = nullptr; unsigned int *dmax = nullptr;
	int rc = arena_get(h, &hist1, bins1); if (rc) return rc;
	rc = arena_get(h, &start1, bins1 + 1); if (rc) return rc;
	rc = arena_get(h, &cursor, groups); if (rc) return rc;
	rc = arena_get(h, &dmax, 1); if (rc) return rc;
	if (bits2) { rc = arena_get(h, &hist2, groups); if (rc) return rc; rc = arena_get(h, &pad1, bins1); if (rc) return rc; rc = arena_get(h, &gstart, groups + 1); if (rc) return rc; }
	HIPCHK(h, hipMemsetAsync(hist1, 0, 4 * bins1, h->stream)); HIPCHK(h, hipMemsetAsync(dmax, 0, 4, h->stream));
	BbInput in1; in1.entries = h->ue.get<uint64_t>(); in1.seg_start = nullptr; in1.seg_count = nullptr; in1.n_seg = 1; in1.n_slots = wslots; in1.holes = 1;
	auto hist_grid = [&](uint64_t n_slots, uint32_t &tpb) { const uint64_t tiles = (n_slots + BB_TILE - 1) / BB_TILE; tpb = (uint32_t)std::max<uint64_t>(1, (tiles + 2047) / 2048); return (unsigned)((tiles + tpb - 1) / tpb); };
	auto scatter_grid = [&](uint64_t n_slots) { const uint64_t tiles = (n_slots + BB_TILE - 1) / BB_TILE; return (unsigned)std::min<uint64_t>(tiles, (uint64_t)num_cus(h) * 8); };
	auto scratch = [&](uint64_t entries) { return h->ue2.reserve(h, "ue2", 8ull * (W + 1) * entries); };
	auto group_launch = [&](const uint64_t *entries, const uint64_t *gs, const uint32_t *gc) -> int {
		int rc2 = wm.keys.reserve(h, "weak map keys", std::max<uint64_t>(8ull * W * wn, 8)); if (rc2) return rc2;
		rc2 = wm.vals.reserve(h, "weak map vals", std::max<uint64_t>(12ull * wn, 8)); if (rc2) return rc2;
		auto gk = bb_group_kernel<W>;
		HIPCHK(h, hipFuncSetAttribute((const void *)gk, hipFuncAttributeMaxDynamicSharedMemorySize, (int)bb_group_smem_bytes<W>()));
		int per_cu = 0;
		if (hipOccupancyMaxActiveBlocksPerMultiprocessor(&per_cu, (const void *)gk, BB_GROUP_THREADS, bb_group_smem_bytes<W>()) != hipSuccess || per_cu < 1) per_cu = 4;
		if (dbg()) fprintf(stderr, "bb_group<W=%d>: %d blocks per CU, %llu groups\n", W, per_cu, (unsigned long long)groups);
		hipLaunchKernelGGL(gk, dim3((unsigned)std::min<uint64_t>(groups, (uint64_t)num_cus(h) * per_cu)), dim3(BB_GROUP_THREADS), bb_group_smem_bytes<W>(), h->stream, entries, wm.keys.get<uint64_t>(), wm.vals.get<uint32_t>(), gs, gc, groups, g, h->hkb, nb, wm.start.get<uint64_t>(), wn, h->derr.get<uint32_t>());
		HIPCHK(h, hipGetLastError());
		return 0;
	};
	const uint32_t shift1 = B - bits1;
	uint32_t tpb = 1; unsigned grid = hist_grid(wslots, tpb);
	hipLaunchKernelGGL(bb_hist_kernel<W>, dim3(grid), dim3(BB_THREADS), 0, h->stream, in1, shift1, bits1, h->hkb, nb, tpb, hist1);
	unsigned int mx = 0;
	if (!bits2) {
		hipLaunchKernelGGL(bb_pad_kernel, dim3(grid_for(bins1)), dim3(256), 0, h->stream, (const uint32_t *)hist1, bins1, (uint32_t *)nullptr, dmax);
		HIPCHK(h, hipMemcpyAsync(&mx, dmax, 4, hipMemcpyDeviceToHost, h->stream));
		rc = exclusive_scan(h, hist1, bins1, start1); if (rc) return rc;
		if (mx > bb_group_cap<W>()) return 0;
		rc = scratch(wn); if (rc) return rc;
		hipLaunchKernelGGL(bb_cursor_init_kernel, dim3(grid_for(bins1)), dim3(256), 0, h->stream, (const uint64_t *)start1, bins1, cursor);
		hipLaunchKernelGGL(bb_scatter_kernel<W>, dim3(scatter_grid(wslots)), dim3(BB_THREADS), 0, h->stream, in1, shift1, bits1, h->hkb, nb, cursor, h->ue2.get<uint64_t>());
		rc = group_launch(h->ue2.get<uint64_t>(), start1, hist1); if (rc) return rc;
		done = true;
		return 0;
	}
	hipLaunchKernelGGL(bb_pad_kernel, dim3(grid_for(bins1)), dim3(256), 0, h->stream, (const uint32_t *)hist1, bins1, pad1, dmax);
	rc = exclusive_scan(h, pad1, bins1, start1); if (rc) return rc;
	uint64_t padded_total = 0;
	HIPCHK(h, hipMemcpy(&padded_total, start1 + bins1, 8, hipMemcpyDeviceToHost));
	rc = scratch(std::max(padded_total, wn)); if (rc) return rc;
	hipLaunchKernelGGL(bb_cursor_init_kernel, dim3(grid_for(bins1)), dim3(256), 0, h->stream, (const uint64_t *)start1, bins1, cursor);
	hipLaunchKernelGGL(bb_scatter_kernel<W>, dim3(scatter_grid(wslots)), dim3(BB_THREADS), 0, h->stream, in1, shift1, bits1, h->hkb, nb, cursor, h->ue2.get<uint64_t>());
	BbInput in2; in2.entries = h->ue2.get<uint64_t>(); in2.seg_start = start1; in2.seg_count = hist1; in2.n_seg = (uint32_t)bins1; in2.n_slots = padded_total; in2.holes = 0;
	const uint32_t shift2 = g;
	HIPCHK(h, hipMemsetAsync(hist2, 0, 4 * groups, h->stream)); HIPCHK(h, hipMemsetAsync(dmax, 0, 4, h->stream));
	grid = hist_grid(padded_total, tpb);
	hipLaunchKernelGGL(bb_hist_kernel<W>, dim3(grid), dim3(BB_THREADS), 0, h->stream, in2, shift2, bits2, h->hkb, nb, tpb, hist2);
	hipLaunchKernelGGL(bb_pad_kernel, dim3(grid_for(groups)), dim3(256), 0, h->stream, (const uint32_t *)hist2, groups, (uint32_t *)nullptr, dmax);
	HIPCHK(h, hipMemcpyAsync(&mx, dmax, 4, hipMemcpyDeviceToHost, h->stream));
	rc = exclusive_scan(h, hist2, groups, gstart); if (rc) return rc;
	if (mx > bb_group_cap<W>() || packed_entries(h, h->ue) < wn) return 0;
	hipLaunchKernelGGL(bb_cursor_init_kernel, dim3(grid_for(groups)), dim3(256), 0, h->stream, (const uint64_t *)gstart, groups, cursor);
	hipLaunchKernelGGL(bb_scatter_kernel<W>, dim3(scatter_grid(padded_total)), dim3(BB_THREADS), 0, h->stream, in2, shift2, bits2, h->hkb, nb, cursor, h->ue.get<uint64_t>());
	rc = group_launch(h->ue.get<uint64_t>(), gstart, hist2); if (rc) return rc;
	done = true;
	return 0;
}

template <int W> int finish_maps_t(kmr_handle *h, uint32_t *wc, uint32_t *sc, uint64_t wslots, uint64_t sslots, uint64_t wn, uint64_t sn, bool keepSing, bool weak_uncounted) {
	const uint32_t vw = h->ext ? 15 : 3;
	DevMap &wm = h->weak, &sm = h->sing;
	clear_map(wm); clear_map(sm);
	wm.nb = h->nb_weak; wm.n = wn; wm.present = true;
	sm.nb = h->nb_sing; sm.n = keepSing ? sn : 0; sm.present = keepSing;
	int rc = wm.start.reserve(h, "weak map start", 8 * (wm.nb + 1)); if (rc) return rc;
	rc = sm.start.reserve(h, "singleton map start", 8 * (sm.nb + 1)); if (rc) return rc;
	bool weakDone = false;
	if (weak_uncounted) {
		rc = binned_buckets_t<W>(h, wslots, wn, weakDone); if (rc) return rc;
		if (!weakDone) {
			if (key_entries(h, h->uw_keys) < wslots || !h->uw_vals) {
				h->uw_keys.reset(); h->uw_vals.reset();
				const uint64_t cap = std::max<uint64_t>(wslots, 16);
				HIPCHK(h, h->uw_keys.alloc(8ull * W * cap)); HIPCHK(h, h->uw_vals.alloc(12ull * cap));
			}
			HIPCHK(h, hipMemsetAsync(wc, 0, 4 * wm.nb, h->stream));
			if (wslots) hipLaunchKernelGGL(bb_unpack_kernel<W>, dim3(grid_for(wslots)), dim3(256), 0, h->stream, (const uint64_t *)h->ue.get<uint64_t>(), wslots, h->hkb, wm.nb, (uint64_t *)h->uw_keys.get(), (uint32_t *)h->uw_vals.get(), wc);
			HIPCHK(h, hipGetLastError());
		}
	}
	if (!weakDone) { rc = exclusive_scan(h, wc, wm.nb, wm.start.get<uint64_t>()); if (rc) return rc; }
	if (keepSing) { rc = exclusive_scan(h, sc, sm.nb, sm.start.get<uint64_t>()); if (rc) return rc; }
	else HIPCHK(h, hipMemsetAsync(sm.start.get<uint64_t>(), 0, 8 * (sm.nb + 1), h->stream));
	if (!weakDone) {
		rc = wm.keys.reserve(h, "weak map keys", std::max<uint64_t>(8ull * W * wm.n, 8)); if (rc) return rc;
		rc = wm.vals.reserve(h, "weak map vals", std::max<uint64_t>(4ull * vw * wm.n, 8)); if (rc) return rc;
	}
	rc = sm.keys.reserve(h, "singleton map keys", std::max<uint64_t>(8ull * W * sm.n, 8)); if (rc) return rc;
	rc = sm.sweight.reserve(h, "singleton map sweight", std::max<uint64_t>(sm.n, 8)); if (rc) return rc;
	if (h->ext) { rc = sm.spkt.reserve(h, "singleton map spkt", std::max<uint64_t>(4 * sm.n, 8)); if (rc) return rc; }
	HIPCHK(h, hipMemsetAsync(wc, 0, 4 * wm.nb, h->stream)); HIPCHK(h, hipMemsetAsync(sc, 0, 4 * sm.nb, h->stream));
	if (weakDone) {  }
	else if (wm.n && vw > 4) hipLaunchKernelGGL((entry_scatter_kernel<W, true>), dim3(grid_for(wslots)), dim3(256), 0, h->stream, (const uint64_t *)h->uw_keys.get(), (const uint32_t *)h->uw_vals.get(),
	                            (const uint8_t *)nullptr, (const uint32_t *)nullptr, wslots, vw, h->hkb, wm.nb, wm.start.get<uint64_t>(), wc, wm.keys.get<uint64_t>(), wm.vals.get<uint32_t>(), (uint8_t *)nullptr, (uint32_t *)nullptr);
	else if (wm.n) {
		unsigned long long *cur64 = nullptr;
		if (h->superkmer_mode && arena_get(h, &cur64, wm.nb) == 0) HIPCHK(h, hipMemcpyAsync(cur64, wm.start.get<uint64_t>(), 8 * wm.nb, hipMemcpyDeviceToDevice, h->stream));
		else cur64 = nullptr;
		hipLaunchKernelGGL(entry_scatter_kernel<W>, dim3(grid_for(wslots)), dim3(256), 0, h->stream, (const uint64_t *)h->uw_keys.get(), (const uint32_t *)h->uw_vals.get(),
		                            (const uint8_t *)nullptr, (const uint32_t *)nullptr, wslots, vw, h->hkb, wm.nb, wm.start.get<uint64_t>(), wc, wm.keys.get<uint64_t>(), wm.vals.get<uint32_t>(), (uint8_t *)nullptr, (uint32_t *)nullptr, cur64, 6);
	}
	if (sm.n) hipLaunchKernelGGL(entry_scatter_kernel<W>, dim3(grid_for(sslots)), dim3(256), 0, h->stream, (const uint64_t *)h->us_keys.get(), (const uint32_t *)nullptr,
	                            (const uint8_t *)h->us_b8.get(), (const uint32_t *)h->us_pkt.get(), sslots, 0u, h->hkb, sm.nb, sm.start.get<uint64_t>(), sc, sm.keys.get<uint64_t>(), (uint32_t *)nullptr, sm.sweight.get<uint8_t>(), h->ext ? sm.spkt.get<uint32_t>() : (uint32_t *)nullptr);
	HIPCHK(h, hipGetLastError());
	SortView<W> sv; sv.keys = wm.keys.get<uint64_t>(); sv.vals = wm.vals.get<uint32_t>(); sv.b8 = nullptr; sv.pkt = nullptr; sv.vw = vw;
	if (weakDone) {  }
	else if (h->ext) hipLaunchKernelGGL((sort_buckets_kernel<W, 15>), dim3(grid_for(wm.nb, 4, 1 << 20)), dim3(256), 0, h->stream, sv, wm.start.get<uint64_t>(), wm.nb);
	else hipLaunchKernelGGL((sort_buckets_kernel<W, 3>), dim3(grid_for(wm.nb, 4, 1 << 20)), dim3(256), 0, h->stream, sv, wm.start.get<uint64_t>(), wm.nb);
	if (sm.n) {
		SortView<W> ss; ss.keys = sm.keys.get<uint64_t>(); ss.vals = nullptr; ss.b8 = sm.sweight.get<uint8_t>(); ss.pkt = h->ext ? sm.spkt.get<uint32_t>() : nullptr; ss.vw = 0;
		hipLaunchKernelGGL((sort_buckets_kernel<W, 0>), dim3(grid_for(sm.nb, 4, 1 << 20)), dim3(256), 0, h->stream, ss, sm.start.get<uint64_t>(), sm.nb);
	}
	HIPCHK(h, hipGetLastError());
	HIPCHK(h, hipStreamSynchronize(h->stream));
	return 0;
}
int finish_maps_from_entries(kmr_handle *h, uint32_t *wc, uint32_t *sc, uint64_t wslots, uint64_t sslots, uint64_t wn, uint64_t sn, bool keepSing, bool weak_uncounted) {
	return with_w(h, [&](auto W) { return finish_maps_t<W()>(h, wc, sc, wslots, sslots, wn, sn, keepSing, weak_uncounted); });
}
int finalize_partition(kmr_handle *h, uint32_t min_depth) { return with_w_ext(h, [&](auto W, auto EXT) { return finalize_partition_t<W(), EXT()>(h, min_depth); }); }
template <int W, bool EXT> int insert_records_partition_t(kmr_handle *h, const void *recs, uint64_t n) {
	if (!h->l1.head) choose_bits1(h, n);
	hipEvent_t a, b; time_begin(h, 0, &a, &b);
	int rc = partition_level1<W, EXT>(h, recs, nullptr, nullptr, (n + 8191) / 8192, 0, 8192, n, n, &h->dstats.get<DevStats>()->inserted,
	                             2 * W + (h->ext ? 2 : 1), h->stream_base);
	time_end(h, 0, a, b);
	return rc;
}
int insert_records_partition(kmr_handle *h, const void *recs, uint64_t n) { return with_w_ext(h, [&](auto W, auto EXT) { return insert_records_partition_t<W(), EXT()>(h, recs, n); }); }
bool sk_geometry(uint32_t k, uint32_t m_wish, uint32_t &win, uint32_t &m, uint32_t &off, uint32_t win_max = 16) {
	for (uint32_t w : {32u, 16u, 8u, 4u}) {
		if (w > win_max) continue;
		if (w == 32u && (k < 45u || (m_wish && m_wish < 14u))) continue;
		if (k < w + 9) continue;
		uint32_t mm = std::min<uint32_t>(m_wish ? m_wish : 16u, k - w + 1);
		if (mm > 16) mm = 16;
		if (((k - mm + 1 - w) & 1u) != 0) mm--;
		if (mm < 10 && !m_wish) continue;
		if (mm < 4) continue;
		win = w; m = mm; off = (k - mm + 1 - w) / 2;
		return true;
	}
	return false;
}
const uint64_t SK_EXTRACT_WAVES_PER_CU = std::max(2 * SK_WAVES, SKL_MIN_BLOCKS * SKL_WAVES);
template <int W, int WIN, bool FILT, bool EXT = false> int launch_sk_extract(kmr_handle *h, const ReadsView &rv, const SkParams &sp, const DevParams *override_params = nullptr) {
	auto kern = sk_extract_kernel<W, WIN, FILT, EXT>;
	HIPCHK(h, hipFuncSetAttribute((const void *)kern, hipFuncAttributeMaxDynamicSharedMemorySize, (int)SK_EXTRACT_SMEM));
	const uint64_t tiles = ((rv.u_start ? rv.n_units : rv.n_reads) + 63) / 64;
	uint64_t blocks = (tiles + SK_WAVES - 1) / SK_WAVES;
	if (blocks == 0) return 0;
	blocks = std::min<uint64_t>(blocks, (uint64_t)num_cus(h) * 2);
	if (dbg()) { int nb = 0; hipOccupancyMaxActiveBlocksPerMultiprocessor(&nb, (const void *)kern, SK_WAVES * 64, SK_EXTRACT_SMEM); fprintf(stderr, "sk_extract<W=%d,WIN=%d>: %d blocks of %d waves per CU (LDS %zu), grid %llu, m=%u off=%u bits=%u\n", W, WIN, nb, SK_WAVES, SK_EXTRACT_SMEM, (unsigned long long)blocks, sp.m, sp.off, sp.list_bits); }
	hipLaunchKernelGGL(kern, dim3((unsigned)blocks), dim3(SK_WAVES * 64), SK_EXTRACT_SMEM, h->stream, rv, override_params ? *override_params : dev_params(h), sp, pool_view(h, h->l1));
	HIPCHK(h, hipGetLastError());
	return 0;
}
uint32_t sk_dbg_flags(const char *name);
bool sp_debug_extract(kmr_handle *h) { (void)h; return sk_dbg_flags("KMR_SK_EXTRACT_DBG") != 0; }
template <int W, int WIN, bool PACKED = false> int launch_sk_extract_lean(kmr_handle *h, const ReadsView &rv, const SkParams &sp, float wK, const DevParams *override_params = nullptr, const SkPacked *packed = nullptr) {
	auto kern = sk_extract_lean_kernel<W, WIN, PACKED>;
	SkPacked pkd{};
	if (PACKED) pkd = *packed;
	HIPCHK(h, hipFuncSetAttribute((const void *)kern, hipFuncAttributeMaxDynamicSharedMemorySize, (int)SKL_EXTRACT_SMEM));
	const uint64_t tiles = ((rv.u_start ? rv.n_units : rv.n_reads) + 63) / 64;
	uint64_t blocks = (tiles + SKL_WAVES - 1) / SKL_WAVES;
	if (blocks == 0) return 0;
	blocks = std::min<uint64_t>(blocks, (uint64_t)num_cus(h) * SKL_MIN_BLOCKS);
	hipLaunchKernelGGL(kern, dim3((unsigned)blocks), dim3(SKL_WAVES * 64), SKL_EXTRACT_SMEM, h->stream, rv, override_params ? *override_params : dev_params(h), sp, pool_view(h, h->l1), wK, pkd);
	HIPCHK(h, hipGetLastError());
	return 0;
}
int sk_uniform_weight(kmr_handle *h, const ReadsView &rv, bool &lean, float &wK) {
	lean = false; wK = 1.0f;
	if (h->tune.no_lean_extract) return 0;
	if (!rv.quals && h->uniform_q_hint < 0) { lean = true; return 0; }
	if (h->qual_mixed || rv.n_reads == 0) return 0;
	if (h->uniform_q_hint >= 0) {
		const unsigned int q0 = (unsigned int)h->uniform_q_hint;
		if (q0 == 127) { lean = true; wK = 1.0f; return 0; }
		if (!(h->hP[q0] > 0.0)) return 0;
		lean = true; wK = (float)h->hPk[q0];
		return 0;
	}
	{ int rc = h->qrange.reserve(h, "qrange", 8); if (rc) return rc; }
	const unsigned int init[2] = {255u, 0u};
	HIPCHK(h, hipMemcpyAsync(h->qrange.get<unsigned int>(), init, 8, hipMemcpyHostToDevice, h->stream));
	hipLaunchKernelGGL(sk_qual_range_kernel, dim3(num_cus(h) * 8), dim3(256), 0, h->stream, rv.quals, rv.offsets, rv.n_reads, h->qrange.get<unsigned int>());
	HIPCHK(h, hipGetLastError());
	unsigned int got[2] = {0, 0};
	HIPCHK(h, hipMemcpyAsync(got, h->qrange.get<unsigned int>(), 8, hipMemcpyDeviceToHost, h->stream));
	HIPCHK(h, hipStreamSynchronize(h->stream));
	if (got[0] != got[1]) { h->qual_mixed = got[0] < got[1]; return 0; }
	const unsigned int q0 = got[0];
	if (q0 == 127) { lean = true; wK = 1.0f; return 0; }
	if (!(h->hP[q0] > 0.0)) return 0;
	lean = true; wK = (float)h->hPk[q0];
	return 0;
}
uint32_t sk_dbg_flags(const char *name) {
#ifdef KMR_DEBUG_HOOKS
	const char *e = getenv(name); return e ? (uint32_t)atoi(e) : 0u;
#else
	(void)name; return 0u;
#endif
}
SkParams sk_params(kmr_handle *h) { SkParams sp; sp.dbg = sk_dbg_flags("KMR_SK_EXTRACT_DBG"); sp.keep_all_owners = h->sk_exchange ? 1u : 0u; sp.track = nullptr; sp.m = h->sk_m; sp.off = h->sk_off; sp.list_bits = h->sk_bits; sp.state = h->sk_state.get<unsigned long long>(); sp.Pk = h->dPk.get<double>(); sp.Rp = h->dPk.get<double>() + 256; sp.fast_div = h->sk_fast_div ? 1u : 0u; return sp; }
template <int W> int add_reads_superkmer_t(kmr_handle *h, const ReadsView &rvAll, uint64_t total_bases) {
	const uint64_t n = rvAll.n_reads;
	const DevParams dp = dev_params(h);
	const bool filt = dp.subsample > 1 || dp.num_parts > 1 || (dp.sub_wnb | dp.sub_snb) != 0 || (dp.world > 1 && !h->sk_exchange);
	bool lean = false; float wK = 1.0f;
	if (!filt && !h->ext && !sp_debug_extract(h)) { int rcq = sk_uniform_weight(h, rvAll, lean, wK); if (rcq) return rcq; }
	if (h->packed_direct && (!lean || h->cfg.size_tracker)) return fail(h, KMR_ERR_STATE, "internal: a packed batch handed to an extraction that wants text");
	if (rvAll.n_reads) {
		uint32_t wb; memcpy(&wb, &wK, 4);
		if (!lean) h->sk_uni_mixed = true;
		else if (h->sk_uni_w == SK_UNI_NONE) h->sk_uni_w = wb;
		else if (h->sk_uni_w != wb) h->sk_uni_mixed = true;
	}
	if (!h->sk_state) {
		const uint64_t est = h->cfg.estimated_raw_kmers ? h->cfg.estimated_raw_kmers : std::max<uint64_t>(total_bases, h->call_bases_hint) * std::max<uint32_t>(1, h->cfg.world_size);
		const uint64_t per_list = h->ext ? (W > 1 ? 400 : 600) : ((h->tune.target_list == 2048 && W > 1) ? 700 : h->tune.target_list * 3 / 4);
		uint32_t bits = 6; while (bits < 24 && (est >> bits) > per_list) bits++;
		h->sk_fine_shift = 0;
		if (h->sk_exchange && h->cfg.world_size > 1 && !h->tune.no_coarse_lists) {
			uint32_t sh = 0; while ((1u << sh) < h->cfg.world_size) sh++;
			if (bits >= 6 + sh) { h->sk_fine_shift = sh; bits -= sh; }
		}
		h->sk_bits = bits;
		if (h->cfg.world_size <= 1 && !h->sk_exchange && h->tune.target_list == 2048 && !h->tune.pow2_lists) {
			const uint64_t aim = h->tune.list_aim ? h->tune.list_aim : (W == 1 ? (h->ext ? 800 : (lean ? 1450 : 1700)) : per_list * 19 / 20);
			const uint64_t nlists = (est / aim + 63) & ~63ull;
			if (nlists > 64 && (nlists < (1ull << bits) || h->tune.list_aim) && nlists < (1ull << 31)) h->sk_bits = (uint32_t)nlists;
		}
		const uint64_t nl0 = sk_list_count(h->sk_bits);
		HIPCHK(h, h->sk_state.alloc(8 * nl0));
		hipLaunchKernelGGL(sk_state_init_kernel, dim3(grid_for(nl0)), dim3(256), 0, h->stream, h->sk_state.get<unsigned long long>(), nl0);
		HIPCHK(h, hipGetLastError());
	}
	const uint64_t avg = n ? std::max<uint64_t>(1, total_bases / n) : 1;
	const uint64_t sub_bases = h->tune.sub_batch_bases ? h->tune.sub_batch_bases : (1ull << 31);
	const uint64_t chunk = std::max<uint64_t>(64, (sub_bases / avg) & ~63ull);
	if (h->cfg.size_tracker && n) {
		h->trk_n = 0;
		{ int rc = h->trk.reserve(h, "trk", n * sizeof(SkTrackRec)); if (rc) return rc; }
		HIPCHK(h, hipMemsetAsync(h->trk.get<SkTrackRec>(), 0, n * sizeof(SkTrackRec), h->stream));
	}
	for (uint64_t r = 0; r < n; r += chunk) {
		const uint64_t m = std::min(chunk, n - r);
		ReadsView rv = reads_slice(rvAll, r, m);
		int rc = prepare_units(h, rv, h->packed_direct ? SK_PACKED_SPAN : (uint32_t)TILE_SPAN); if (rc) return rc;
		const uint64_t bases = m * avg + avg;
		if (!h->l1.base && r == 0 && h->cfg.world_size <= 1 && !h->sk_exchange && (h->cfg.estimated_raw_kmers || h->call_bases_hint > total_bases)) {
			const double job_bases = h->cfg.estimated_raw_kmers ? (double)h->cfg.estimated_raw_kmers * (double)avg / (double)(avg > h->k ? avg - h->k + 1 : 1) : (double)h->call_bases_hint;
			const double rest = job_bases - (double)total_bases;
			size_t fr = 0, tot = 0;
			if (rest > 0 && hipMemGetInfo(&fr, &tot) == hipSuccess) {
				const uint64_t want = (uint64_t)(rest * (h->ext ? 2.0 : 1.0) * (lean ? 0.3 : 0.65) / SK_CHUNK_G);
				h->l1.presize = std::min<uint64_t>(want, (uint64_t)(fr / 4) / ((size_t)CH * rec_bytes(h)));
			}
		}
		rc = pool_reserve(h, h->l1, (h->ext ? 2 : 1) * bases / SK_CHUNK_G + ((h->l1.base && !h->sk_exchange) ? 0 : sk_list_count(h->sk_bits)) + (uint64_t)num_cus(h) * SK_EXTRACT_WAVES_PER_CU * 130 + 64, true); if (rc) return rc;
		hipEvent_t a, b, a2, b2; time_begin(h, KMR_TIME_BUILD, &a, &b); time_begin(h, KMR_TIME_EXTRACT, &a2, &b2);
		SkParams sp = sk_params(h);
		if (h->cfg.size_tracker) sp.track = h->trk.get<SkTrackRec>() + r;
		if (h->packed_direct) {
			SkPacked pkd = *h->packed_direct; pkd.off += r; if (pkd.mk_off) pkd.mk_off += r;
			rc = with_win<W>(h->sk_win, [&](auto WIN) { return launch_sk_extract_lean<W, WIN(), true>(h, rv, sp, wK, nullptr, &pkd); });
		} else rc = with_win<W>(h->sk_win, [&](auto WIN) {
			if (h->ext) return filt ? launch_sk_extract<W, WIN(), true, true>(h, rv, sp) : launch_sk_extract<W, WIN(), false, true>(h, rv, sp);
			if (filt) return launch_sk_extract<W, WIN(), true>(h, rv, sp);
			return lean ? launch_sk_extract_lean<W, WIN()>(h, rv, sp, wK) : launch_sk_extract<W, WIN(), false>(h, rv, sp);
		});
		time_end(h, KMR_TIME_EXTRACT, a2, b2); time_end(h, KMR_TIME_BUILD, a, b);
		if (rc) return rc;
	}
	if (h->cfg.size_tracker && n) {
		std::vector<SkTrackRec> recs(n);
		HIPCHK(h, hipMemcpyAsync(recs.data(), h->trk.get<SkTrackRec>(), n * sizeof(SkTrackRec), hipMemcpyDeviceToHost, h->stream));
		HIPCHK(h, hipStreamSynchronize(h->stream));
		std::vector<SkBoundary> bd; std::vector<uint64_t> good_before;
		const bool walkable = (dp.sub_wnb | dp.sub_snb) == 0;
		for (uint64_t r = 0; r < n; r++) {
			while ((uint64_t)h->trk_next <= h->trk_raw + recs[r].raw) {
				SkBoundary b; b.read = r; b.t = (uint32_t)((uint64_t)h->trk_next - h->trk_raw); b.good = 0; b.ordinal = 0;
				if (!walkable) { b.t = recs[r].raw; b.good = recs[r].good; b.ordinal = recs[r].end_ordinal; }
				bd.push_back(b); good_before.push_back(h->trk_good);
				h->trk_snap_raw.push_back(walkable ? (uint64_t)h->trk_next : h->trk_raw + recs[r].raw);
				h->trk_next = (long)((double)h->trk_next * 1.05);
				if (!walkable) break;
			}
			if (!walkable) while ((uint64_t)h->trk_next <= h->trk_raw + recs[r].raw) h->trk_next = (long)((double)h->trk_next * 1.05);
			h->trk_raw += recs[r].raw; h->trk_good += recs[r].good;
		}
		if (h->trk_bounds.size() + bd.size() > SK_TRACK_MAX) return fail(h, KMR_ERR_UNSUPPORTED, "size tracker: more than 512 elements");
		if (!bd.empty() && walkable) {
			DevBuf dbdb; HIPCHK(h, dbdb.alloc(bd.size() * sizeof(SkBoundary)));
			SkBoundary *dbd = dbdb.get<SkBoundary>();
			hipError_t e = hipMemcpyAsync(dbd, bd.data(), bd.size() * sizeof(SkBoundary), hipMemcpyHostToDevice, h->stream);
			if (e == hipSuccess) {
				ReadsView rv = rvAll; rv.u_start = rv.u_end = rv.u_read = nullptr; rv.n_units = 0;
				hipLaunchKernelGGL(sk_track_boundary_kernel<W>, dim3((unsigned)((bd.size() + 63) / 64)), dim3(64), 0, h->stream, rv, dp, dbd, (uint32_t)bd.size());
				e = hipGetLastError();
			}
			if (e == hipSuccess) e = hipMemcpyAsync(bd.data(), dbd, bd.size() * sizeof(SkBoundary), hipMemcpyDeviceToHost, h->stream);
			if (e == hipSuccess) e = hipStreamSynchronize(h->stream);
			if (e != hipSuccess) return fail(h, KMR_ERR_HIP, std::string("size tracker boundaries: ") + hipGetErrorString(e));
		}
		for (size_t i = 0; i < bd.size(); i++) { h->trk_bounds.push_back(bd[i].ordinal); h->trk_snap_good.push_back(good_before[i] + bd[i].good); }
	}
	return 0;
}
int add_reads_superkmer(kmr_handle *h, const ReadsView &rv, uint64_t total_bases) { return with_w(h, [&](auto W) { return add_reads_superkmer_t<W()>(h, rv, total_bases); }); }
static const uint64_t SAT_BATCH_BYTES = 1ull << 30;
static const uint64_t SAT_BATCH_KEYS = (1ull << 23) - 1;
static const uint64_t SAT_PAIR_BYTES = 24;
template <int W> int saturated_fix_t(kmr_handle *h, const uint64_t *ls, const uint64_t *lc, uint64_t nl, unsigned long long n_clamped, unsigned long long n_sightings, uint32_t has_singletons) {
	DevMap &wm = h->weak;
	h->last_saturated_keys = 0; h->last_saturated_batches = 0;
	if (!n_clamped || !wm.n) return 0;
	uint32_t list_bits = 0; while ((1ull << list_bits) < nl) list_bits++;
	if ((1ull << list_bits) != nl) list_bits = (uint32_t)nl;
	auto no_mem = [&](const char *what, size_t bytes) { return fail(h, KMR_ERR_OOM, std::string("saturated-key pass (weights of k-mers seen 256 times or more): no device memory for ") + what + " (" + std::to_string(bytes) + " bytes)"); };
	auto dalloc = [](DevBuf &b, size_t bytes) { return b.alloc(std::max<size_t>(bytes, 256)); };
	DevBuf bfound, bentry, blist;
	if (dalloc(bfound, 8) != hipSuccess) return no_mem("a counter", 8);
	unsigned long long *dfound = bfound.get<unsigned long long>(); uint64_t *d_entry = nullptr; uint32_t *d_list = nullptr;
	uint64_t cap = std::min<uint64_t>(wm.n, 4 * n_clamped + 1024);
	unsigned long long found = 0;
	for (;;) {
		if (dalloc(bentry, 8 * cap) != hipSuccess || dalloc(blist, 4 * cap) != hipSuccess) return no_mem("the key list", 12 * cap);
		d_entry = bentry.get<uint64_t>(); d_list = blist.get<uint32_t>();
		HIPCHK(h, hipMemsetAsync(dfound, 0, 8, h->stream));
		hipLaunchKernelGGL(sat_find_kernel<W>, dim3(grid_for(wm.n)), dim3(256), 0, h->stream, (const uint64_t *)wm.keys.get<uint64_t>(), (const uint32_t *)wm.vals.get<uint32_t>(), wm.n, h->sk_m, h->sk_off, h->sk_win, list_bits, dfound, cap, d_entry, d_list, h->ext ? 15u : 3u);
		HIPCHK(h, hipGetLastError());
		HIPCHK(h, hipMemcpyAsync(&found, dfound, 8, hipMemcpyDeviceToHost, h->stream)); HIPCHK(h, hipStreamSynchronize(h->stream));
		if (found <= cap) break;
		cap = found;
	}
	if (!found) return 0;
	std::vector<uint64_t> entry(found); std::vector<uint32_t> lst(found);
	HIPCHK(h, hipMemcpy(entry.data(), d_entry, 8 * found, hipMemcpyDeviceToHost)); HIPCHK(h, hipMemcpy(lst.data(), d_list, 4 * found, hipMemcpyDeviceToHost));
	std::vector<uint64_t> order(found);
	for (uint64_t i = 0; i < found; i++) order[i] = i;
	std::sort(order.begin(), order.end(), [&](uint64_t a, uint64_t b) { return lst[a] != lst[b] ? lst[a] < lst[b] : entry[a] < entry[b]; });
	std::vector<uint64_t> sentry(found); std::vector<uint32_t> dl; std::vector<uint64_t> le0, le1;
	for (uint64_t i = 0; i < found; i++) {
		sentry[i] = entry[order[i]];
		const uint32_t l = lst[order[i]];
		if (dl.empty() || dl.back() != l) { dl.push_back(l); le0.push_back(i); le1.push_back(i + 1); } else le1.back() = i + 1;
	}
	std::vector<uint64_t>().swap(entry); std::vector<uint32_t>().swap(lst); std::vector<uint64_t>().swap(order);
	HIPCHK(h, hipMemcpy(d_entry, sentry.data(), 8 * found, hipMemcpyHostToDevice));
	HIPCHK(h, hipMemcpy(d_list, dl.data(), 4 * dl.size(), hipMemcpyHostToDevice));
	std::vector<uint64_t> c0(dl.size()), c1(dl.size());
	{
		DevBuf bc0, bc1;
		if (dalloc(bc0, 8 * dl.size()) != hipSuccess || dalloc(bc1, 8 * dl.size()) != hipSuccess) return no_mem("the chunk ranges", 16 * dl.size());
		hipLaunchKernelGGL(sat_gather_kernel, dim3(grid_for(dl.size())), dim3(256), 0, h->stream, ls, (const uint32_t *)d_list, (uint64_t)dl.size(), bc0.get<uint64_t>(), bc1.get<uint64_t>());
		HIPCHK(h, hipGetLastError());
		HIPCHK(h, hipMemcpy(c0.data(), bc0.get<uint64_t>(), 8 * dl.size(), hipMemcpyDeviceToHost)); HIPCHK(h, hipMemcpy(c1.data(), bc1.get<uint64_t>(), 8 * dl.size(), hipMemcpyDeviceToHost));
	}
	blist = DevBuf();
	struct Seg { uint32_t li; uint64_t e0, e1, est; };
	std::vector<Seg> segs;
	uint64_t all_chunks = 0;
	for (size_t i = 0; i < dl.size(); i++) all_chunks += c1[i] - c0[i];
	const double per_chunk = all_chunks ? (double)n_sightings / (double)all_chunks : 0.0;
	for (size_t i = 0; i < dl.size(); i++)
		for (uint64_t a = le0[i]; a < le1[i]; a += SAT_BATCH_KEYS) {
			const uint64_t b = std::min<uint64_t>(le1[i], a + SAT_BATCH_KEYS);
			const double share = (double)(b - a) / (double)(le1[i] - le0[i]);
			segs.push_back(Seg{(uint32_t)i, a, b, (uint64_t)(per_chunk * (double)(c1[i] - c0[i]) * share) + 1});
		}
	const uint64_t budget = h->tune.saturated_batch_bytes ? h->tune.saturated_batch_bytes : SAT_BATCH_BYTES;
	uint64_t batches = 0;
	for (size_t s0 = 0; s0 < segs.size(); ) {
		size_t s1 = s0 + 1; uint64_t est = segs[s0].est;
		while (s1 < segs.size() && segs[s1].e1 - segs[s0].e0 <= SAT_BATCH_KEYS && (est + segs[s1].est) * SAT_PAIR_BYTES <= budget) est += segs[s1++].est;
		const uint64_t k0 = segs[s0].e0, nk = segs[s1 - 1].e1 - k0;
		std::vector<uint64_t> items;
		for (size_t g = s0; g < s1; g++)
			for (uint64_t a = c0[segs[g].li]; a < c1[segs[g].li]; a += 256) { items.push_back(a); items.push_back(std::min(c1[segs[g].li], a + 256)); items.push_back(segs[g].e0 - k0); items.push_back(segs[g].e1 - k0); }
		const size_t ni = items.size() / 4;
		std::vector<uint64_t> soa(4 * ni);
		for (size_t i = 0; i < ni; i++) for (int q = 0; q < 4; q++) soa[q * ni + i] = items[4 * i + q];
		uint64_t pcap = est + est / 4 + 1024;
		for (int attempt = 0; ni; attempt++) {
			DevBuf bitems, bk_in, bk_out, bv_in, bv_out, btmp;
			if (dalloc(bitems, 32 * ni) != hipSuccess) return no_mem("its work items", 32 * ni);
			uint64_t *d_items = bitems.get<uint64_t>();
			HIPCHK(h, hipMemcpy(d_items, soa.data(), 32 * ni, hipMemcpyHostToDevice));
			if (dalloc(bk_in, 8 * pcap) != hipSuccess || dalloc(bk_out, 8 * pcap) != hipSuccess || dalloc(bv_in, 4 * pcap) != hipSuccess || dalloc(bv_out, 4 * pcap) != hipSuccess)
				return no_mem("the sightings of one batch", SAT_PAIR_BYTES * pcap);
			unsigned long long *pk_in = bk_in.get<unsigned long long>(), *pk_out = bk_out.get<unsigned long long>(); uint32_t *pv_in = bv_in.get<uint32_t>(), *pv_out = bv_out.get<uint32_t>();
			HIPCHK(h, hipMemsetAsync(dfound, 0, 8, h->stream));
			int rc = zero_work_counter(h); if (rc) return rc;
			hipLaunchKernelGGL(sat_collect_kernel<W>, dim3((unsigned)std::min<uint64_t>(ni, (uint64_t)num_cus(h) * 4)), dim3(256), 0, h->stream, pool_view(h, h->l1), lc, h->k, (const uint64_t *)wm.keys.get<uint64_t>(), (const uint64_t *)(d_entry + k0),
			                   (const uint64_t *)d_items, (const uint64_t *)(d_items + ni), (const uint64_t *)(d_items + 2 * ni), (const uint64_t *)(d_items + 3 * ni), (uint64_t)ni, dfound, pcap, pk_in, pv_in, h->work_counter.get<unsigned int>());
			HIPCHK(h, hipGetLastError());
			unsigned long long n_pairs = 0;
			HIPCHK(h, hipMemcpyAsync(&n_pairs, dfound, 8, hipMemcpyDeviceToHost, h->stream)); HIPCHK(h, hipStreamSynchronize(h->stream));
			if (n_pairs > pcap) {
				if (attempt) return fail(h, KMR_ERR_CAPACITY, "saturated-key pass: sightings of a batch changed between two passes (internal error)");
				pcap = n_pairs;
				continue;
			}
			size_t tmp_bytes = 0;
			if (kmr::sort_pairs_u64_u32(nullptr, &tmp_bytes, pk_in, pk_out, pv_in, pv_out, n_pairs, h->stream) != 0) return fail(h, KMR_ERR_HIP, "saturated-key pass: radix sort (size query)");
			if (dalloc(btmp, tmp_bytes) != hipSuccess) return no_mem("the sort's temporary storage", tmp_bytes);
			if (kmr::sort_pairs_u64_u32(btmp.get(), &tmp_bytes, pk_in, pk_out, pv_in, pv_out, n_pairs, h->stream) != 0) return fail(h, KMR_ERR_HIP, "saturated-key pass: radix sort");
			hipLaunchKernelGGL(sat_reduce_kernel, dim3((unsigned)std::min<uint64_t>(nk, 4096)), dim3(256), 0, h->stream, (const unsigned long long *)pk_out, (const uint32_t *)pv_out, (uint64_t)n_pairs, (const uint64_t *)(d_entry + k0), (uint64_t)nk, has_singletons, wm.vals.get<uint32_t>(), h->ext ? 15u : 3u);
			HIPCHK(h, hipGetLastError());
			HIPCHK(h, hipStreamSynchronize(h->stream));
			break;
		}
		batches++;
		s0 = s1;
	}
	h->last_saturated_keys = found; h->last_saturated_batches = batches;
	return 0;
}


template <int W> int sk_count_uniform(kmr_handle *h, bool tracking, bool &uni, uint32_t &uni_wbits) {
	uni = false; uni_wbits = 0;
	if (tracking || h->ext || h->sk_uni_mixed || h->tune.no_uniform_count) return 0;
	if (W > 1 && (h->k & 31u) == 0) return 0;
	uint32_t w = h->sk_uni_w; bool mixed = false;
	if (h->peer_uni_mixed) mixed = true;
	else if (h->peer_uni_w != SK_UNI_NONE) { if (w == SK_UNI_NONE) w = h->peer_uni_w; else if (w != h->peer_uni_w) mixed = true; }
	if (h->d_uni) {
		uint32_t dv[2] = {SK_UNI_NONE, 0u};
		HIPCHK(h, hipMemcpy(dv, h->d_uni.get<uint32_t>(), 8, hipMemcpyDeviceToHost));
		if (dv[1]) mixed = true;
		else if (dv[0] != SK_UNI_NONE) { if (w == SK_UNI_NONE) w = dv[0]; else if (w != dv[0]) mixed = true; }
	}
	if (!mixed && w != SK_UNI_NONE) { uni = true; uni_wbits = w; }
	return 0;
}
template <int W> SkLong<W> sk_own_lists(kmr_handle *h, bool refined) {
	SkLong<W> lg{};
	lg.list_first = 0; lg.list_stride = 1;
	if (h->sk_exchange && h->cfg.world_size > 1 && !refined) { lg.list_first = h->cfg.rank; lg.list_stride = h->cfg.world_size; }
	return lg;
}
template <int W> struct SkCountLaunch {
	void (*kern)(PoolView, const uint64_t *, const uint64_t *, uint64_t, uint32_t, CountOut, FinalizeParams, unsigned int *, uint32_t, SkTrackView, SkLong<W>);
	size_t smem;
};
template <int W, int LOG2S, bool TRACK, bool EXT, bool UNI> SkCountLaunch<W> sk_count_form() { return {sk_count_kernel<W, LOG2S, TRACK, EXT, UNI>, sk_count_smem_bytes<W, LOG2S, TRACK, EXT, UNI>()}; }
template <int W> int sk_count_select(kmr_handle *h, bool ext, bool tracking, bool uni, SkCountLaunch<W> &k) {
	k = ext ? sk_count_form<W, COUNT_LOG2S_EXT, false, true, false>() : (tracking ? sk_count_form<W, COUNT_LOG2S, true, false, false>() :
	    (uni ? sk_count_form<W, COUNT_LOG2S, false, false, true>() : sk_count_form<W, COUNT_LOG2S, false, false, false>()));
	const auto kern = k.kern; const size_t smem = k.smem;
	HIPCHK(h, hipFuncSetAttribute((const void *)kern, hipFuncAttributeMaxDynamicSharedMemorySize, (int)smem));
	return 0;
}

template <int W> struct SkFinalize {
	FinalizeParams f{}; bool keepSing = false, ext = false, tracking = false, refined = false, uni = false;
	uint64_t nl = 1; uint64_t *ls = nullptr, *lc = nullptr; uint32_t nch = 0;
	uint64_t wcap = 0, scap = 0, wmax = 0, smax = 0;
	uint32_t *wc = nullptr, *sc = nullptr; FinalizeCounters *fc = nullptr; unsigned long long *cursors = nullptr;
	SkTrackView tv{};
	SkLong<W> lgMain{}, lgItems{}; uint64_t n_items = 0;
	uint64_t early_slots = 0; FinalizeCounters early_c{};
	FinalizeCounters c{}; unsigned long long cur[2] = {0, 0};
};

int sk_refine_lists(kmr_handle *h, uint64_t &nl) {
	const uint32_t fine_bits = h->sk_bits + h->sk_fine_shift;
	const uint64_t nlf = 1ull << fine_bits;
	unsigned int head = 0;
	HIPCHK(h, hipStreamSynchronize(h->stream));
	HIPCHK(h, hipMemcpy(&head, h->l1.head.get<unsigned int>(), 4, hipMemcpyDeviceToHost));
	if (head > h->l1.cap) head = h->l1.cap;
	int rc = h->sk_fine_state.reserve(h, "sk_fine_state", 8 * nlf); if (rc) return rc;
	hipLaunchKernelGGL(sk_state_init_kernel, dim3(grid_for(nlf)), dim3(256), 0, h->stream, h->sk_fine_state.get<unsigned long long>(), nlf);
	const int rgrid = (int)std::min<uint64_t>(((uint64_t)head + SK_REFINE_WAVES - 1) / SK_REFINE_WAVES + 1, (uint64_t)num_cus(h) * 8);
	rc = pool_reserve(h, h->l1, (uint64_t)head * 2 + nlf / h->cfg.world_size + (uint64_t)rgrid * SK_REFINE_WAVES * 130 + 64, true); if (rc) return rc;
	if (head) hipLaunchKernelGGL(sk_refine_kernel, dim3(rgrid), dim3(SK_REFINE_WAVES * 64), 0, h->stream, pool_view(h, h->l1), head, fine_bits, h->sk_fine_state.get<unsigned long long>());
	hipLaunchKernelGGL(sk_close_kernel, dim3(grid_for(nlf)), dim3(256), 0, h->stream, h->sk_fine_state.get<unsigned long long>(), nlf, h->l1.chunk_count.get<uint32_t>(), h->l1.cap);
	HIPCHK(h, hipGetLastError());
	nl = nlf;
	return 0;
}
template <int W> int sk_entry_buffers(kmr_handle *h, SkFinalize<W> &p, uint64_t G) {
	const FinalizeParams &f = p.f; const bool keepSing = p.keepSing;
	const uint64_t slack = (uint64_t)num_cus(h) * 4 * 8192 + 16;
	const uint64_t wbound = f.has_singletons ? G / 2 : G, sbound = keepSing ? G : 0;
	const bool adopted = h->sk_exchange && h->cfg.world_size > 1;
	p.wmax = adopted ? (1ull << 40) : wbound + wbound / 8 + slack; p.smax = keepSing ? (adopted ? (1ull << 40) : sbound + sbound / 8 + slack) : 16;
	p.wcap = std::min<uint64_t>(p.wmax, G / (f.has_singletons ? 8 : 3) + slack); p.scap = keepSing ? std::min<uint64_t>(p.smax, G / 3 + slack) : 16;
	if (h->tune.entry_share >= 0) { p.wcap = std::min<uint64_t>(p.wmax, (uint64_t)((double)G * h->tune.entry_share) + 16384); if (keepSing) p.scap = std::min<uint64_t>(p.smax, (uint64_t)((double)G * h->tune.entry_share) + 16384);
		h->ue.reset(); h->us_keys.reset(); h->us_b8.reset(); h->us_pkt.reset(); }
	p.wcap = std::max(p.wcap, p.ext ? key_entries(h, h->uw_keys) : packed_entries(h, h->ue)); p.scap = std::max(p.scap, key_entries(h, h->us_keys));
	int rc = arena_get(h, &p.wc, h->nb_weak); if (rc) return rc; rc = arena_get(h, &p.sc, h->nb_sing); if (rc) return rc;
	rc = arena_get(h, &p.fc, 1); if (rc) return rc; rc = arena_get(h, &p.cursors, 2); if (rc) return rc;
	return 0;
}
int sk_track_view(kmr_handle *h, SkTrackView &tv) {
	const std::vector<unsigned long long> &bounds = h->trk_bounds;
	if (bounds.size() > SK_TRACK_MAX) return fail(h, KMR_ERR_UNSUPPORTED, "size tracker: more than 512 elements");
	unsigned long long *db = nullptr; unsigned int *dd = nullptr;
	int rc = arena_get(h, &db, bounds.size() + 1); if (rc) return rc;
	rc = arena_get(h, &dd, 2 * (bounds.size() + 1)); if (rc) return rc;
	if (!bounds.empty()) HIPCHK(h, hipMemcpyAsync(db, bounds.data(), 8 * bounds.size(), hipMemcpyHostToDevice, h->stream));
	tv.bounds = db; tv.n = (uint32_t)bounds.size(); tv.d_unique = dd; tv.d_single = dd + bounds.size() + 1;
	return 0;
}
int sk_track_elements(kmr_handle *h, const SkTrackView &tv, uint32_t has_singletons) {
	std::vector<unsigned int> dd(2 * (tv.n + 1), 0);
	HIPCHK(h, hipMemcpy(dd.data(), tv.d_unique, 8 * (tv.n + 1), hipMemcpyDeviceToHost));
	h->trk_elems.clear();
	uint64_t uniq = 0; int64_t single = 0;
	const uint64_t sub = h->cfg.kmer_subsample > 1 ? h->cfg.kmer_subsample : 1;
	for (uint32_t i = 0; i < tv.n; i++) {
		uniq += dd[i]; single += (int32_t)dd[tv.n + 1 + i];
		h->trk_elems.push_back(h->trk_snap_raw[i] * sub); h->trk_elems.push_back(h->trk_snap_good[i] * sub);
		h->trk_elems.push_back(uniq * sub); h->trk_elems.push_back(has_singletons ? (uint64_t)single * sub : 0);
	}
	return 0;
}
template <int W> int sk_early_takeover(kmr_handle *h, SkFinalize<W> &p, uint32_t min_depth, bool &device_error) {
	device_error = false;
	FinalizeCounters &early_c = p.early_c;
	h->last_early_hi = 0; h->last_early_entries = 0; h->last_early_overflowed = false;
	if (!h->early.active) return 0;
	uint32_t eerr = 0;
	HIPCHK(h, hipMemcpy(&eerr, h->early.err.get<uint32_t>(), 4, hipMemcpyDeviceToHost));
	unsigned long long ecur = 0;
	HIPCHK(h, hipMemcpy(&ecur, h->early.cursor.get<unsigned long long>(), 8, hipMemcpyDeviceToHost)); HIPCHK(h, hipMemcpy(&early_c, h->early.fc.get(), sizeof(early_c), hipMemcpyDeviceToHost));
	if (eerr & ~(uint32_t)ERR_ENTRIES_FULL) {
		uint32_t e = 0; HIPCHK(h, hipMemcpy(&e, h->derr.get<uint32_t>(), 4, hipMemcpyDeviceToHost)); e |= eerr & ~(uint32_t)ERR_ENTRIES_FULL;
		HIPCHK(h, hipMemcpy(h->derr.get<uint32_t>(), &e, 4, hipMemcpyHostToDevice)); h->early.active = false;
		device_error = true;
		return 0;
	}
	const bool overflowed = (eerr & ERR_ENTRIES_FULL) || ecur > packed_entries(h, h->early.ue);
	const bool ok = !overflowed && h->early.min_depth == min_depth && !p.tracking && !p.ext && !p.keepSing && !p.refined;
	h->last_early_overflowed = overflowed;
	if (ok) {
		p.early_slots = ecur;
		h->last_early_hi = h->early.hi; h->last_early_entries = early_c.weak_kept;
		const uint64_t stride0 = p.lgMain.list_stride, first0 = p.lgMain.list_first;
		uint64_t first = h->early.hi;
		if (stride0 > 1) first += (first0 + stride0 - first % stride0) % stride0;
		p.lgMain.list_first = first;
	} else { h->early.active = false; memset(&early_c, 0, sizeof(early_c)); }
	return 0;
}
template <int W> int sk_long_items(kmr_handle *h, SkFinalize<W> &p) {
	p.lgItems = p.lgMain; p.n_items = 0;
	const uint64_t LONG_CHUNKS = p.ext ? std::min<uint64_t>(h->tune.long_list_chunks ? h->tune.long_list_chunks : SK_EXT_LONG_CHUNKS, SK_EXT_LONG_CHUNKS) : (h->tune.long_list_chunks ? h->tune.long_list_chunks : 1024), PIECE = std::max<uint64_t>(1, LONG_CHUNKS / 2);
	if (p.tracking || p.nch <= LONG_CHUNKS) return 0;
	const uint64_t cap = (uint64_t)p.nch / PIECE + 2 * 1024 + 16;
	uint64_t *ic0 = nullptr, *ic1 = nullptr; unsigned long long *dn = nullptr;
	int rc = arena_get(h, &ic0, cap); if (rc) return rc; rc = arena_get(h, &ic1, cap); if (rc) return rc; rc = arena_get(h, &dn, 1); if (rc) return rc;
	HIPCHK(h, hipMemsetAsync(dn, 0, 8, h->stream));
	hipLaunchKernelGGL(sk_long_items_kernel, dim3(grid_for(p.nl)), dim3(256), 0, h->stream, p.ls, p.nl, LONG_CHUNKS, PIECE, ic0, ic1, cap, dn);
	HIPCHK(h, hipGetLastError());
	unsigned long long hn = 0;
	HIPCHK(h, hipMemcpyAsync(&hn, dn, 8, hipMemcpyDeviceToHost, h->stream)); HIPCHK(h, hipStreamSynchronize(h->stream));
	if (hn > cap) return fail(h, KMR_ERR_CAPACITY, "long-list work items (internal sizing error)");
	p.n_items = hn;
	if (p.n_items) {
		p.lgMain.long_threshold = LONG_CHUNKS;
		p.lgItems.item_c0 = ic0; p.lgItems.item_c1 = ic1; p.lgItems.n_items = p.n_items; p.lgItems.merge_used = dn;
	}
	return 0;
}
CountOut count_out(kmr_handle *h, bool packed, unsigned long long *cursors, uint32_t *wc, uint32_t *sc, FinalizeCounters *fc) {
	CountOut out{};
	if (packed) { out.wentries = h->ue.get<uint64_t>(); out.wcap = packed_entries(h, h->ue); }
	else { out.wkeys = h->uw_keys.get<uint64_t>(); out.wvals = h->uw_vals.get<uint32_t>(); out.wcap = key_entries(h, h->uw_keys); out.spkt = h->us_pkt.get<uint32_t>(); out.weakCount = wc; }
	out.wcursor = cursors; out.scursor = cursors + 1;
	out.skeys = h->us_keys.get<uint64_t>(); out.sweight = h->us_b8.get<uint8_t>(); out.scap = key_entries(h, h->us_keys);
	out.singCount = sc; out.fc = fc; out.err = h->derr.get<uint32_t>();
	return out;
}
template <int W> int sk_count_pass(kmr_handle *h, SkFinalize<W> &p, bool &overflowed) {
	overflowed = false;
	const bool ext = p.ext, keepSing = p.keepSing, tracking = p.tracking; const uint32_t vw = ext ? 15 : 3;
	uint64_t &wcap = p.wcap, &scap = p.scap; const uint64_t wmax = p.wmax, smax = p.smax, nl = p.nl, n_items = p.n_items;
	uint32_t *wc = p.wc, *sc = p.sc; FinalizeCounters *fc = p.fc; unsigned long long *cursors = p.cursors;
	FinalizeCounters &c = p.c; unsigned long long *cur = p.cur; const SkTrackView &tv = p.tv; const FinalizeParams &f = p.f;
	int rc = 0;
	uint32_t merge_log2 = 16;
	hipEvent_t tca, tcb; time_begin(h, KMR_TIME_COUNT, &tca, &tcb);
	for (int attempt = 0; ; attempt++) {
		if (!ext && packed_entries(h, h->ue) < wcap) { h->ue.reset(); HIPCHK(h, h->ue.alloc(8ull * (W + 1) * wcap)); }
		if (ext && (key_entries(h, h->uw_keys) < wcap || !h->uw_vals)) {
			h->uw_keys.reset(); h->uw_vals.reset();
			HIPCHK(h, h->uw_keys.alloc(8ull * W * wcap)); HIPCHK(h, h->uw_vals.alloc(4ull * vw * wcap));
		}
		if (key_entries(h, h->us_keys) < scap || !h->us_b8 || (ext && !h->us_pkt)) {
			h->us_keys.reset(); h->us_b8.reset(); h->us_pkt.reset();
			HIPCHK(h, h->us_keys.alloc(8ull * W * scap)); HIPCHK(h, h->us_b8.alloc(scap)); if (ext) HIPCHK(h, h->us_pkt.alloc(4 * scap));
		}
		HIPCHK(h, hipMemsetAsync(wc, 0, 4 * h->nb_weak, h->stream)); HIPCHK(h, hipMemsetAsync(sc, 0, 4 * h->nb_sing, h->stream));
		HIPCHK(h, hipMemsetAsync(fc, 0, sizeof(FinalizeCounters), h->stream)); HIPCHK(h, hipMemsetAsync(cursors, 0, 16, h->stream));
		const CountOut out = count_out(h, !ext, cursors, wc, sc, fc);
		rc = zero_work_counter(h); if (rc) return rc;
		const int grid = (int)std::min<uint64_t>((uint64_t)num_cus(h) * 4, (nl / p.lgMain.list_stride + SK_LBATCH) / SK_LBATCH);
		SkCountLaunch<W> k;
		rc = sk_count_select<W>(h, ext, tracking, p.uni, k); if (rc) return rc;
		if (tracking) HIPCHK(h, hipMemsetAsync(tv.d_unique, 0, 8 * (tv.n + 1), h->stream));
		if (dbg()) { int nb = 0; hipOccupancyMaxActiveBlocksPerMultiprocessor(&nb, (const void *)k.kern, SKC_THREADS, k.smem); fprintf(stderr, "sk_count<W=%d>: %d blocks per CU (LDS %zu), %llu lists, %u chunks\n", W, nb, k.smem, (unsigned long long)nl, p.nch); }
		hipLaunchKernelGGL(k.kern, dim3(grid), dim3(SKC_THREADS), k.smem, h->stream, pool_view(h, h->l1), p.ls, p.lc, nl, h->k, out, f, h->work_counter.get<unsigned int>(), sk_dbg_flags("KMR_SK_COUNT_DBG"), tv, p.lgMain);
		HIPCHK(h, hipGetLastError());
		DevBuf mslots, mext;
		if (n_items) {
			SkLong<W> &lgItems = p.lgItems;
			if (mslots.alloc(sizeof(Slot<W>) << merge_log2) != hipSuccess) return fail(h, KMR_ERR_OOM, "merge table of the long lists");
			if (ext && mext.alloc(sizeof(ExtSlot) << merge_log2) != hipSuccess) return fail(h, KMR_ERR_OOM, "merge table of the long lists");
			hipLaunchKernelGGL(table_clear_kernel<W>, dim3(grid_for(1ull << merge_log2)), dim3(256), 0, h->stream, mslots.get<Slot<W>>(), mext.get<ExtSlot>(), 1ull << merge_log2);
			lgItems.merge.slots = mslots.get<Slot<W>>(); lgItems.merge.ext = mext.get<ExtSlot>(); lgItems.merge.log2cap = merge_log2;
			HIPCHK(h, hipMemsetAsync(lgItems.merge_used, 0, 8, h->stream));
			rc = zero_work_counter(h); if (rc) return rc;
			const int grid2 = (int)std::min<uint64_t>((uint64_t)num_cus(h) * 4, n_items);
			hipLaunchKernelGGL(k.kern, dim3(grid2), dim3(SKC_THREADS), k.smem, h->stream, pool_view(h, h->l1), p.ls, p.lc, nl, h->k, out, f, h->work_counter.get<unsigned int>(), sk_dbg_flags("KMR_SK_COUNT_DBG"), tv, lgItems);
			hipLaunchKernelGGL(sk_merge_emit_kernel<W>, dim3(grid_for(1ull << merge_log2)), dim3(256), 0, h->stream, lgItems.merge, out, f);
			if (hipGetLastError() != hipSuccess) return fail(h, KMR_ERR_HIP, "long-list launches");
		}
		uint32_t cerr = 0;
		HIPCHK(h, hipMemcpyAsync(&c, fc, sizeof(c), hipMemcpyDeviceToHost, h->stream)); HIPCHK(h, hipMemcpyAsync(cur, cursors, 16, hipMemcpyDeviceToHost, h->stream));
		HIPCHK(h, hipMemcpyAsync(&cerr, h->derr.get<uint32_t>(), 4, hipMemcpyDeviceToHost, h->stream));
		HIPCHK(h, hipStreamSynchronize(h->stream));
		if (n_items && (cerr & ERR_TABLE_FULL) && merge_log2 < 30) {
			cerr &= ~(uint32_t)(ERR_TABLE_FULL | ERR_ENTRIES_FULL);
			HIPCHK(h, hipMemcpy(h->derr.get<uint32_t>(), &cerr, 4, hipMemcpyHostToDevice));
			merge_log2 += 3;
			continue;
		}
		if (!(cerr & ERR_ENTRIES_FULL)) break;
		if ((wcap >= wmax && scap >= smax) || attempt >= 8) { overflowed = true; break; }
		cerr &= ~(uint32_t)ERR_ENTRIES_FULL;
		HIPCHK(h, hipMemcpy(h->derr.get<uint32_t>(), &cerr, 4, hipMemcpyHostToDevice));
		wcap = std::min<uint64_t>(wmax, wcap * 2); if (keepSing) scap = std::min<uint64_t>(smax, scap * 2);
		if (dbg()) fprintf(stderr, "sk count pass: entry buffers too small, retrying with %llu / %llu\n", (unsigned long long)wcap, (unsigned long long)scap);
	}
	time_end(h, KMR_TIME_COUNT, tca, tcb);
	return 0;
}
template <int W> int sk_append_early(kmr_handle *h, SkFinalize<W> &p) {
	FinalizeCounters &c = p.c; const FinalizeCounters &early_c = p.early_c; unsigned long long *cur = p.cur; const uint64_t early_slots = p.early_slots;
	const size_t eb = 8ull * (W + 1);
	if (cur[0] + early_slots > packed_entries(h, h->ue)) {
		DevBuf bigger;
		HIPCHK(h, bigger.alloc(eb * (cur[0] + early_slots + 4096)));
		HIPCHK(h, hipMemcpyAsync(bigger.get(), h->ue.get(), eb * cur[0], hipMemcpyDeviceToDevice, h->stream)); HIPCHK(h, hipStreamSynchronize(h->stream));
		h->ue = std::move(bigger);
	}
	HIPCHK(h, hipMemcpyAsync((uint8_t *)h->ue.get<uint64_t>() + eb * cur[0], h->early.ue.get<uint64_t>(), eb * early_slots, hipMemcpyDeviceToDevice, h->stream));
	cur[0] += early_slots;
	c.unique += early_c.unique; c.singletons += early_c.singletons; c.weak_kept += early_c.weak_kept; c.sing_kept += early_c.sing_kept;
	c.saturated += early_c.saturated; c.sat_sightings += early_c.sat_sightings;
	h->stats.unique_kmers = c.unique; h->stats.singleton_kmers = p.f.has_singletons ? c.singletons : 0;
	return 0;
}

template <int W> int finalize_superkmer_t(kmr_handle *h, uint32_t min_depth) {
	int rc = sync_state(h);
	if (rc) return rc;
	hipEvent_t ea, eb; time_begin(h, 1, &ea, &eb);
	SkFinalize<W> p;
	p.f = finalize_params(h, min_depth);
	p.keepSing = p.f.has_singletons && min_depth <= 1;
	p.ext = h->ext;
	p.tracking = h->cfg.size_tracker != 0;
	if (!h->l1.head) { rc = pool_reserve(h, h->l1, 0, false); if (rc) return rc; }
	rc = arena_reset(h); if (rc) return rc;
	p.nl = h->sk_state ? sk_list_count(h->sk_bits) : 1;
	if (h->sk_state) {
		hipLaunchKernelGGL(sk_close_kernel, dim3(grid_for(p.nl)), dim3(256), 0, h->stream, h->sk_state.get<unsigned long long>(), p.nl, h->l1.chunk_count.get<uint32_t>(), h->l1.cap);
		HIPCHK(h, hipGetLastError());
	}
	p.refined = h->sk_state && h->sk_fine_shift > 0;
	if (p.refined) { rc = sk_refine_lists(h, p.nl); if (rc) return rc; }
	rc = build_csr(h, h->l1, p.nl, 0, &p.ls, &p.lc, &p.nch); if (rc) return rc;
	rc = sk_entry_buffers<W>(h, p, h->stats.raw_good_kmers); if (rc) return rc;
	rc = sk_count_uniform<W>(h, p.tracking, p.uni, p.f.uni_wbits); if (rc) return rc;
	h->last_count_uniform = p.uni;
	if (p.tracking) { rc = sk_track_view(h, p.tv); if (rc) return rc; }
	p.lgMain = sk_own_lists<W>(h, p.refined);
	bool device_error = false;
	rc = sk_early_takeover<W>(h, p, min_depth, device_error); if (rc) return rc;
	if (device_error) { time_end(h, 1, ea, eb); return sync_state(h); }
	rc = sk_long_items<W>(h, p); if (rc) return rc;
	bool overflowed = false;
	rc = sk_count_pass<W>(h, p, overflowed); if (rc) return rc;
	if (overflowed) { time_end(h, 1, ea, eb); return fail(h, KMR_ERR_CAPACITY, "entry buffers of the count pass overflowed at their upper bound (internal sizing error)"); }
	h->stats.unique_kmers = p.c.unique;
	h->stats.singleton_kmers = p.f.has_singletons ? p.c.singletons : 0;
	if (p.tracking) { rc = sk_track_elements(h, p.tv, p.f.has_singletons); if (rc) return rc; }
	if (p.early_slots) { rc = sk_append_early<W>(h, p); if (rc) return rc; }
	h->early.active = false;
	hipEvent_t tma, tmb; time_begin(h, KMR_TIME_BUCKETS, &tma, &tmb);
	rc = finish_maps_from_entries(h, p.wc, p.sc, p.cur[0], p.cur[1], p.c.weak_kept, p.c.sing_kept, p.keepSing, !p.ext);
	time_end(h, KMR_TIME_BUCKETS, tma, tmb);
	if (rc) return rc;
	h->last_saturated_keys = 0; h->last_saturated_batches = 0;
	if (p.c.saturated) { rc = saturated_fix_t<W>(h, p.ls, p.lc, p.nl, p.c.saturated, p.c.sat_sightings, p.f.has_singletons); if (rc) return rc; }
	time_end(h, 1, ea, eb);
	h->has_singletons = p.keepSing;
	h->stats.weak_entries = h->weak.n; h->stats.singleton_entries = p.keepSing ? h->sing.n : 0;
	h->finalized = true; h->map_gen++;
	rc = sync_state(h);
	if (!rc && !h->arena_overflow.empty()) rc = arena_reset(h);
	return rc;
}
template <int W> int count_prefix_superkmer_t(kmr_handle *h, uint32_t min_depth, uint64_t hi) {
	int rc = sync_state(h); if (rc) return rc;
	FinalizeParams f = finalize_params(h, min_depth);
	const bool keepSing = f.has_singletons && min_depth <= 1;
	h->early.active = false;
	if (h->ext || h->cfg.size_tracker || keepSing || (h->sk_state && h->sk_fine_shift > 0) || !h->sk_state) return KMR_OK;
	const uint64_t nl = sk_list_count(h->sk_bits);
	if (hi > nl) hi = nl;
	if (hi == 0) return KMR_OK;
	rc = arena_reset(h); if (rc) return rc;
	hipLaunchKernelGGL(sk_close_kernel, dim3(grid_for(nl)), dim3(256), 0, h->stream, h->sk_state.get<unsigned long long>(), nl, h->l1.chunk_count.get<uint32_t>(), h->l1.cap);
	HIPCHK(h, hipGetLastError());
	uint64_t *ls = nullptr, *lc = nullptr; uint32_t nch = 0;
	rc = build_csr(h, h->l1, nl, 0, &ls, &lc, &nch); if (rc) return rc;
	const uint64_t G = h->stats.raw_good_kmers;
	const uint64_t slack = (uint64_t)num_cus(h) * 4 * 8192 + 16;
	uint64_t want = (uint64_t)((double)G * ((double)hi / (double)nl) / (f.has_singletons ? 6.0 : 2.5)) + slack;
	if (h->tune.early_entry_share >= 0) { want = (uint64_t)((double)G * h->tune.early_entry_share) + 16384; h->early.ue.reset(); }
	rc = h->early.ue.reserve(h, "early count ue", 8ull * (W + 1) * want); if (rc) return rc;
	rc = h->early.cursor.reserve(h, "early count cursor", 16); if (rc) return rc;
	rc = h->early.fc.reserve(h, "early count fc", sizeof(FinalizeCounters)); if (rc) return rc;
	rc = h->early.err.reserve(h, "early count error word", 4); if (rc) return rc;
	HIPCHK(h, hipMemsetAsync(h->early.cursor.get<unsigned long long>(), 0, 16, h->stream)); HIPCHK(h, hipMemsetAsync(h->early.fc.get(), 0, sizeof(FinalizeCounters), h->stream));
	HIPCHK(h, hipMemsetAsync(h->early.err.get<uint32_t>(), 0, 4, h->stream));
	bool uni = false;
	if (!h->peer_uni_mixed) { rc = sk_count_uniform<W>(h, false, uni, f.uni_wbits); if (rc) return rc; }
	const SkTrackView tv{};
	SkLong<W> lg = sk_own_lists<W>(h, false);
	lg.long_threshold = h->tune.long_list_chunks ? h->tune.long_list_chunks : 1024;
	uint32_t *sc = nullptr;
	rc = arena_get(h, &sc, h->nb_sing); if (rc) return rc;
	HIPCHK(h, hipMemsetAsync(sc, 0, 4 * h->nb_sing, h->stream));
	CountOut out{};
	out.wentries = h->early.ue.get<uint64_t>(); out.wcursor = h->early.cursor.get<unsigned long long>(); out.wcap = packed_entries(h, h->early.ue);
	out.scursor = h->early.cursor.get<unsigned long long>() + 1;
	out.singCount = sc; out.fc = (FinalizeCounters *)h->early.fc.get(); out.err = h->early.err.get<uint32_t>();
	rc = zero_work_counter(h); if (rc) return rc;
	const uint64_t n_work = hi > lg.list_first ? (hi - lg.list_first + lg.list_stride - 1) / lg.list_stride : 0;
	if (n_work) {
		const int grid = (int)std::min<uint64_t>((uint64_t)num_cus(h) * 4, (n_work + SK_LBATCH) / SK_LBATCH);
		SkCountLaunch<W> k;
		rc = sk_count_select<W>(h, false, false, uni, k); if (rc) return rc;
		hipEvent_t a, b; time_begin(h, KMR_TIME_COUNT, &a, &b);
		hipLaunchKernelGGL(k.kern, dim3(grid), dim3(SKC_THREADS), k.smem, h->stream, pool_view(h, h->l1), ls, lc, hi, h->k, out, f, h->work_counter.get<unsigned int>(), sk_dbg_flags("KMR_SK_COUNT_DBG"), tv, lg);
		time_end(h, KMR_TIME_COUNT, a, b);
		HIPCHK(h, hipGetLastError());
	}
	h->early.active = true; h->early.hi = hi; h->early.min_depth = min_depth;
	return KMR_OK;
}
int count_prefix_superkmer(kmr_handle *h, uint32_t min_depth, uint64_t hi) { return with_w(h, [&](auto W) { return count_prefix_superkmer_t<W()>(h, min_depth, hi); }); }
int finalize_superkmer(kmr_handle *h, uint32_t min_depth) { return with_w(h, [&](auto W) { return finalize_superkmer_t<W()>(h, min_depth); }); }

template <class M> void release(kmr_handle *h) { static_cast<M &>(*h) = M(); }

void free_partition_state(kmr_handle *h) {
	release<BuildMem>(h);
	if (h->tb_copy_stream) { hipStreamDestroy(h->tb_copy_stream); h->tb_copy_stream = nullptr; for (int a = 0; a < 2; a++) { hipEventDestroy(h->tb_ready[a]); hipEventDestroy(h->tb_consumed[a]); h->tb_set_used[a] = false; } }
}

}

extern "C" {

uint32_t kmr_abi_version(void) { return KMR_ABI_VERSION; }

int kmr_config_init(kmr_config *c) {
	if (!c) return KMR_ERR_INVALID_ARG;
	memset(c, 0, sizeof(*c));
	c->struct_size = sizeof(*c);
	c->value_kind = KMR_VALUE_COUNT_DIR; c->min_weight = 0.10f; c->min_quality_score = 3; c->fastq_start_char = 33;
	c->ext_min_quality = 20; c->separate_singletons = 1; c->kmer_subsample = 1; c->device = -1; c->rank = 0; c->world_size = 1;
	c->estimated_depth = 20.0; c->estimated_error_rate = 0.35; c->kmers_per_bucket = 32; c->num_parts = 1; c->part_idx = 0;
	return KMR_OK;
}

const char *kmr_last_error(const kmr_handle *h) { return h ? h->err.c_str() : g_create_error.c_str(); }

int kmr_create(const kmr_config *cfg, kmr_handle **out) {
	if (!cfg || !out) return fail(nullptr, KMR_ERR_INVALID_ARG, "null argument");
	*out = nullptr;
	if (cfg->struct_size != sizeof(kmr_config)) return fail(nullptr, KMR_ERR_INVALID_ARG, "kmr_config.struct_size mismatch (ABI)");
	if (cfg->k < 1 || cfg->k > 128) return fail(nullptr, KMR_ERR_INVALID_ARG, "k must be in 1..128");
	if (cfg->world_size < 1 || cfg->rank >= cfg->world_size) return fail(nullptr, KMR_ERR_INVALID_ARG, "bad rank/world_size");
	if (cfg->value_kind > KMR_VALUE_EXT) return fail(nullptr, KMR_ERR_INVALID_ARG, "bad value_kind");
	if (cfg->hash_kind > KMR_HASH_LOOKUP8) return fail(nullptr, KMR_ERR_INVALID_ARG, "bad hash_kind");
	int ndev = 0;
	if (hipGetDeviceCount(&ndev) != hipSuccess || ndev == 0) return fail(nullptr, KMR_ERR_NO_DEVICE, "no HIP device: this library has no CPU path");
	kmr_handle *h = new kmr_handle();
	h->cfg = *cfg;
	if (h->cfg.kmer_subsample == 0) h->cfg.kmer_subsample = 1;
	if (h->cfg.num_parts == 0) h->cfg.num_parts = 1;
	h->k = cfg->k; h->kb = (cfg->k + 3) / 4; h->W = (h->kb + 7) / 8; h->ext = cfg->value_kind == KMR_VALUE_EXT;
	h->hkb = h->kb | (cfg->hash_kind << 16);
	memset(&h->stats, 0, sizeof(h->stats));
	int rc = 0;
	do {
		if (cfg->device >= 0) { if (hipSetDevice(cfg->device) != hipSuccess) { rc = fail(nullptr, KMR_ERR_NO_DEVICE, "hipSetDevice failed"); break; } }
		if (hipGetDevice(&h->device) != hipSuccess) { rc = fail(nullptr, KMR_ERR_NO_DEVICE, "hipGetDevice failed"); break; }
		if (hipStreamCreate(&h->stream) != hipSuccess) { rc = fail(nullptr, KMR_ERR_HIP, "hipStreamCreate failed"); break; }
		uint64_t w = cfg->num_buckets_weak, s = cfg->num_buckets_singleton;
		const double depth = cfg->estimated_depth > 0 ? cfg->estimated_depth : 20.0;
		const uint32_t kpb = cfg->kmers_per_bucket ? cfg->kmers_per_bucket : 32;
		const uint64_t raw = cfg->estimated_raw_kmers / (cfg->world_size > 1 ? cfg->world_size : 1);
		if (w == 0) { unsigned long est = (unsigned long)(int)(raw / depth); w = est / kpb + 1; }
		if (s == 0) { unsigned long est = cfg->separate_singletons ? (unsigned long)(raw * cfg->estimated_error_rate) : 1; s = est / kpb + 1; }
		h->nb_weak = resize_buckets(w); h->nb_sing = resize_buckets(s);
		h->has_singletons = cfg->separate_singletons != 0;
		uint64_t want = cfg->max_table_entries ? (uint64_t)(cfg->max_table_entries / 0.7) : (uint64_t)(cfg->estimated_raw_kmers * 0.45 / 0.6);
		if (cfg->world_size > 1 && !cfg->max_table_entries) want /= cfg->world_size;
		uint32_t lg = 16; while ((1ull << lg) < want && lg < 40) lg++;
		h->log2cap = lg;
		double P[256]; quality_table(P, cfg->min_quality_score, cfg->fastq_start_char);
		if (h->dP.alloc(sizeof(P)) != hipSuccess || h->dstats.alloc(sizeof(DevStats)) != hipSuccess || h->derr.alloc(4) != hipSuccess) { rc = fail(nullptr, KMR_ERR_OOM, "hipMalloc failed"); break; }
		hipMemcpy(h->dP.get<double>(), P, sizeof(P), hipMemcpyHostToDevice); hipMemset(h->dstats.get<DevStats>(), 0, sizeof(DevStats)); hipMemset(h->derr.get<uint32_t>(), 0, 4);
		if (cfg->build_mode > 3) { rc = fail(nullptr, KMR_ERR_INVALID_ARG, "bad build_mode"); break; }
		h->partition_mode = cfg->build_mode != 1;
		uint32_t wish_w = 0, wish_m = 0, wish_o = 0;
		const bool sk_auto = cfg->build_mode == 0 && cfg->world_size <= 1 && sk_geometry(h->k, 0, wish_w, wish_m, wish_o);
		h->auto_mode = cfg->build_mode == 0;
		const bool sk_ready = sk_geometry(h->k, 0, wish_w, wish_m, wish_o);
		if (cfg->build_mode == 3 || sk_auto || sk_ready) {
			if (!sk_geometry(h->k, 0, h->sk_win, h->sk_m, h->sk_off)) { rc = fail(nullptr, KMR_ERR_UNSUPPORTED, "build_mode 3 (super-k-mer lists) needs k >= 13"); break; }
			h->superkmer_mode = cfg->build_mode == 3 || sk_auto;
			double Pk[256];
			for (int cidx = 0; cidx < 256; cidx++) { double wv = 1.0; for (uint32_t jj = 0; jj < h->k; jj++) wv *= P[cidx]; Pk[cidx] = wv; }
			memcpy(h->hPk, Pk, sizeof(Pk)); memcpy(h->hP, P, sizeof(h->hP));
			if (h->dPk.alloc(2 * sizeof(Pk)) != hipSuccess) { rc = fail(nullptr, KMR_ERR_OOM, "hipMalloc failed"); break; }
			hipMemcpy(h->dPk.get<double>(), Pk, sizeof(Pk), hipMemcpyHostToDevice);
			double Rp[256]; bool fast = true;
			for (int cidx = 0; cidx < 256; cidx++) Rp[cidx] = P[cidx] != 0.0 ? 1.0 / P[cidx] : 0.0;
			for (int a = 0; a < 256 && fast; a++) for (int b = 0; b < 256; b++) {
				if (P[a] == 0.0 || P[b] == 0.0) continue;
				const double q0 = P[a] * Rp[b];
				if (std::fma(std::fma(-q0, P[b], P[a]), Rp[b], q0) != P[a] / P[b]) { fast = false; break; }
			}
			h->sk_fast_div = fast;
			hipMemcpy(h->dPk.get<double>() + 256, Rp, sizeof(Rp), hipMemcpyHostToDevice);
		}
		if (cfg->size_tracker && (!h->superkmer_mode || h->ext || cfg->world_size > 1)) { rc = fail(nullptr, KMR_ERR_UNSUPPORTED, "size_tracker: kept by the super-k-mer build (build_mode 0 / 3, direction-counting values, k >= 13) of a single partition"); break; }
		if (!h->partition_mode) {
			rc = alloc_table(h, h->log2cap, h->slots, h->extslots);
			if (rc) { g_create_error = h->err; break; }
		}
		if (hipStreamSynchronize(h->stream) != hipSuccess) { rc = fail(nullptr, KMR_ERR_HIP, std::string("table clear failed: ") + hipGetErrorString(hipGetLastError())); break; }
	} while (0);
	if (rc) { kmr_destroy(h); return rc; }
	*out = h;
	return KMR_OK;
}

static void exchange_destroy_comm(kmr_handle *h);
void kmr_destroy(kmr_handle *h) {
	if (!h) return;
	if (h->stream) hipStreamSynchronize(h->stream);
	for (int which = 0; which < KMR_TIME_GROUPS; which++) for (auto &pr : h->pending_events[which]) { hipEventDestroy(pr.first); hipEventDestroy(pr.second); }
	release<HandleMem>(h);
	free_partition_state(h);
	exchange_destroy_comm(h);
	release<ExchangeMem>(h);
	if (h->stream) hipStreamDestroy(h->stream);
	delete h;
}

int kmr_num_buckets(const kmr_handle *h, int which, uint64_t *out) {
	if (!h || !out) return KMR_ERR_INVALID_ARG;
	if (which == KMR_MAP_WEAK) *out = h->finalized && h->weak.present ? h->weak.nb : h->nb_weak;
	else if (which == KMR_MAP_SINGLETON) *out = h->finalized && h->sing.present ? h->sing.nb : h->nb_sing;
	else return KMR_ERR_UNSUPPORTED;
	return KMR_OK;
}

int kmr_reset(kmr_handle *h) {
	if (!h) return KMR_ERR_INVALID_ARG;
	hipSetDevice(h->device);
	HIPCHK(h, hipStreamSynchronize(h->stream));
	clear_map(h->weak); clear_map(h->sing);
	int rc = 0;
	if (h->partition_mode) {
		if (h->l1.head) HIPCHK(h, hipMemsetAsync(h->l1.head.get<unsigned int>(), 0, 4, h->stream));
		h->l1.used_ub = 0;
		h->inserted_records = 0;
		h->qual_mixed = false;
		h->sk_uni_w = SK_UNI_NONE; h->sk_uni_mixed = false; h->peer_uni_w = SK_UNI_NONE; h->peer_uni_mixed = false; h->peers_declare = false;
		h->xr_lo = 0; h->xr_hi = ~0ull; h->early.active = false;
		if (h->d_uni) { const uint32_t init[2] = {SK_UNI_NONE, 0u}; HIPCHK(h, hipMemcpyAsync(h->d_uni.get<uint32_t>(), init, 8, hipMemcpyHostToDevice, h->stream)); HIPCHK(h, hipStreamSynchronize(h->stream)); }
		if (h->sk_state) hipLaunchKernelGGL(sk_state_init_kernel, dim3(grid_for(sk_list_count(h->sk_bits))), dim3(256), 0, h->stream, h->sk_state.get<unsigned long long>(), sk_list_count(h->sk_bits));
		if (h->l1_state) {
			hipLaunchKernelGGL(partition_state_init_kernel, dim3(partition_blocks(h)), dim3(256), 0, h->stream, h->l1_state.get<uint8_t>(),
			                   h->l1_state.cap() / (size_t)partition_blocks(h), h->bits1, (uint32_t)partition_blocks(h));
			h->l1_state_dirty = false;
		}
	} else {
		if (!h->slots) rc = alloc_table(h, h->log2cap, h->slots, h->extslots);
		else rc = clear_table_any(h, h->slots.get(), h->extslots.get<ExtSlot>(), h->log2cap);
		if (rc) return rc;
	}
	HIPCHK(h, hipMemsetAsync(h->dstats.get<DevStats>(), 0, sizeof(DevStats), h->stream));
	HIPCHK(h, hipMemsetAsync(h->derr.get<uint32_t>(), 0, 4, h->stream));
	memset(&h->stats, 0, sizeof(h->stats));
	h->occupied = h->pending_kmers = 0; h->stream_base = 0; h->reads = 0; h->subtracted = 0; h->xc_job_bases = 0; h->xc_bytes_to_peers = 0;
	h->trk_n = 0; h->trk_elems.clear();
	h->trk_next = 128; h->trk_raw = h->trk_good = 0; h->trk_bounds.clear(); h->trk_snap_raw.clear(); h->trk_snap_good.clear();
	h->finalized = false; h->map_gen++; h->has_singletons = h->cfg.separate_singletons != 0;
	return KMR_OK;
}
int kmr_release_table(kmr_handle *h) {
	if (!h) return KMR_ERR_INVALID_ARG;
	if (!h->finalized) return fail(h, KMR_ERR_STATE, "kmr_release_table before kmr_finalize");
	hipSetDevice(h->device);
	h->slots.reset(); h->extslots.reset();
	if (h->partition_mode) free_partition_state(h);
	return KMR_OK;
}

void *kmr_stream(kmr_handle *h) { return h ? (void *)h->stream : nullptr; }

int kmr_set_stream_origin(kmr_handle *h, uint64_t ordinal) {
	if (!h) return KMR_ERR_INVALID_ARG;
	if (h->finalized) return fail(h, KMR_ERR_STATE, "kmr_set_stream_origin after kmr_finalize");
	if (ordinal > MAX_STREAM_ORDINAL) return fail(h, KMR_ERR_CAPACITY, "stream ordinals have 40 bits");
	h->stream_base = ordinal;
	return KMR_OK;
}

int kmr_tune(kmr_handle *h, const char *knob, double value) {
	if (!h || !knob) return KMR_ERR_INVALID_ARG;
	const std::string k(knob);
	if (k == "target_list_records") h->tune.target_list = value >= 1 ? (uint64_t)value : 2048;
	else if (k == "sub_batch_bases") h->tune.sub_batch_bases = value >= 1 ? (uint64_t)value : 0;
	else if (k == "recycle_chunks") h->tune.recycle = value < 0 ? -1 : (value != 0 ? 1 : 0);
	else if (k == "partition_blocks") h->tune.part_blocks = value >= 1 ? (int)value : 0;
	else if (k == "entry_share") h->tune.entry_share = value;
	else if (k == "early_entry_share") h->tune.early_entry_share = value;
	else if (k == "saturated_batch_bytes") h->tune.saturated_batch_bytes = value >= 1 ? (uint64_t)value : 0;
	else if (k == "lookup_table") h->tune.no_lut = value == 0;
	else if (k == "stream_lookups") h->tune.no_stream_lookups = value == 0;
	else if (k == "long_list_chunks") h->tune.long_list_chunks = value < 2 ? 2 : (uint64_t)value;
	else if (k == "lean_extract") h->tune.no_lean_extract = value == 0;
	else if (k == "uniform_count") h->tune.no_uniform_count = value == 0;
	else if (k == "packed_direct") h->tune.no_packed_direct = value == 0;
	else if (k == "pow2_lists") h->tune.pow2_lists = value != 0;
	else if (k == "list_aim") h->tune.list_aim = value >= 1 ? (uint64_t)value : 0;
	else if (k == "twobit_piece_bases") h->tune.twobit_piece_bases = (uint64_t)value;
	else if (k == "exchange_fail_once") h->tune.exchange_fail_once = value != 0;
	else if (k == "binned_buckets_min") h->tune.binned_min = value >= 0 ? (uint64_t)value : ~0ull;
	else if (k == "coarse_lists") h->tune.no_coarse_lists = value == 0;
	else if (k == "select_timing") h->tune.select_timing = value != 0;
	else if (k == "dump_timing") h->tune.dump_timing = value != 0;
	else if (k == "pairs_timing") h->tune.pairs_timing = value != 0;
	else if (k == "pair_hash_bits") h->tune.pair_hash_bits = value >= 1 && value < 64 ? (uint32_t)value : 64;
	else if (k == "dump_piece_bytes") h->tune.dump_piece_bytes = value >= 1 ? (uint64_t)value : 0;
	else if (k == "narrow_tallies") h->tune.no_narrow = value == 0;
	else if (k == "keep_level1_state") h->tune.no_l1_state = value == 0;
	else if (k == "superkmer_window") {
		if (h->superkmer_mode && !h->sk_state) { uint32_t w, m, o; if (!sk_geometry(h->k, 0, w, m, o, (uint32_t)value)) return fail(h, KMR_ERR_INVALID_ARG, "no minimizer geometry under that window"); h->sk_win = w; h->sk_m = m; h->sk_off = o; }
	}
	else if (k == "superkmer_minimizer") {
		if (h->superkmer_mode && !h->sk_state) { uint32_t w, m, o; if (!sk_geometry(h->k, (uint32_t)value, w, m, o)) return fail(h, KMR_ERR_INVALID_ARG, "no minimizer geometry for that length"); h->sk_win = w; h->sk_m = m; h->sk_off = o; }
	}
	else return fail(h, KMR_ERR_INVALID_ARG, "unknown tuning knob '" + k + "'");
	return KMR_OK;
}

int kmr_build_info(kmr_handle *h, const char *what, double *value) {
	if (!h || !what || !value) return KMR_ERR_INVALID_ARG;
	const std::string k(what);
	if (k == "lists") *value = h->sk_state ? (double)sk_list_count(h->sk_bits) : 0.0;
	else if (k == "uniform_count") *value = h->last_count_uniform ? 1.0 : 0.0;
	else if (k == "chunk_pool_chunks") *value = (double)h->l1.cap;
	else if (k == "superkmer_window") *value = (double)h->sk_win;
	else if (k == "early_lists") *value = (double)h->last_early_hi;
	else if (k == "early_entries") *value = (double)h->last_early_entries;
	else if (k == "early_overflowed") *value = h->last_early_overflowed ? 1.0 : 0.0;
	else if (k == "saturated_keys") *value = (double)h->last_saturated_keys;
	else if (k == "saturated_batches") *value = (double)h->last_saturated_batches;
	else if (k == "device_blocks_live") *value = (double)g_blocks_live.load();
	else if (k == "filter_score_ms") *value = h->last_score_ms;
	else if (k == "select_ms") *value = h->last_select_ms;
	else if (k == "select_write_ms") *value = h->last_write_ms;
	else if (k == "pairs_ms") *value = h->last_pairs_ms;
	else if (k == "pairs_parse_ms") *value = h->last_pairs_parse_ms;
	else if (k == "pairs_sort_ms") *value = h->last_pairs_sort_ms;
	else if (k == "pair_hash_collisions") *value = (double)h->last_pair_hash_collisions;
	else if (k == "dump_size_ms") *value = h->last_dump_size_ms;
	else if (k == "dump_write_ms") *value = h->last_dump_write_ms;
	else return fail(h, KMR_ERR_INVALID_ARG, "unknown build figure '" + k + "'");
	return KMR_OK;
}

int kmr_sync(kmr_handle *h) { if (!h) return KMR_ERR_INVALID_ARG; hipSetDevice(h->device); return sync_state(h); }

int kmr_add_reads_dev(kmr_handle *h, const void *dev_bases, const void *dev_quals, const void *dev_offsets, uint64_t n_reads,
                      uint64_t total_bases, uint64_t first_global_read_idx, const void *dev_discarded) {
	if (!h) return KMR_ERR_INVALID_ARG;
	if (h->finalized) return fail(h, KMR_ERR_STATE, "kmr_add_reads after kmr_finalize");
	if (n_reads == 0) return KMR_OK;
	if (!dev_bases || !dev_offsets) return fail(h, KMR_ERR_INVALID_ARG, "null device buffer");
	hipSetDevice(h->device);
	const ReadsView rv = reads_view(dev_bases, dev_quals, dev_offsets, n_reads, dev_discarded, h->stream_base, first_global_read_idx);
	if (h->stream_base + total_bases > MAX_STREAM_ORDINAL) return fail(h, KMR_ERR_CAPACITY, "more than 2^40 input bases on one handle");
	if (h->partition_mode && !h->superkmer_mode && !h->ext && h->stream_base + total_bases > (1ull << 32))
		return fail(h, KMR_ERR_CAPACITY, "build_mode 2 orders occurrences by a 32-bit stream ordinal: at most 2^32 input bases per handle without extension values (use build_mode 0 / 3 or 1)");
	int rc = h->superkmer_mode ? add_reads_superkmer(h, rv, total_bases) : (h->partition_mode ? add_reads_partition(h, rv, total_bases) : add_reads_dev_any(h, rv, total_bases));
	h->stream_base += total_bases; h->reads += n_reads; h->stats.reads = h->reads;
	return rc;
}

static hipError_t tb_stage_copy(kmr_handle *h, int set, int which, const void *src, size_t bytes, void **dst) {
	DevBuf &buf = h->tb_stage[set][which];
	if (buf.cap() < bytes + 128) {
		if (buf) { hipError_t e0 = hipStreamSynchronize(h->stream); if (e0 != hipSuccess) return e0; }
		hipError_t e = buf.alloc(bytes + bytes / 8 + 4096); if (e != hipSuccess) return e;
	}
	*dst = buf.get();
	return bytes ? hipMemcpyAsync(buf.get(), src, bytes, hipMemcpyHostToDevice, h->tb_copy_stream) : hipSuccess;
}
static int tb_pipeline_ready(kmr_handle *h) {
	if (h->tb_copy_stream) return 0;
	HIPCHK(h, hipStreamCreateWithFlags(&h->tb_copy_stream, hipStreamNonBlocking));
	for (int i = 0; i < 2; i++) { HIPCHK(h, hipEventCreateWithFlags(&h->tb_ready[i], hipEventDisableTiming)); HIPCHK(h, hipEventCreateWithFlags(&h->tb_consumed[i], hipEventDisableTiming)); }
	return 0;
}

#define TBCHK(call) do { hipError_t e_ = (call); if (e_ != hipSuccess) { hipStreamSynchronize(h->tb_copy_stream); hipStreamSynchronize(h->stream); h->err = std::string(#call) + ": " + hip_err_text(e_); return e_ == hipErrorOutOfMemory ? KMR_ERR_OOM : KMR_ERR_HIP; } } while (0)
}
template <class Stage, class Feed> static int tb_feed_pieces(kmr_handle *h, const uint64_t *offsets, uint64_t n_reads, Stage &&stage, Feed &&feed) {
	{ int rcp = tb_pipeline_ready(h); if (rcp) return rcp; }
	const uint64_t piece_bases = h->tune.twobit_piece_bases ? h->tune.twobit_piece_bases : (1ull << 28);
	int rc = KMR_OK; int set = 0;
	h->call_bases_hint = n_reads ? offsets[n_reads] - offsets[0] : 0;
	struct HintReset { kmr_handle *h; ~HintReset() { h->call_bases_hint = 0; } } hint_reset{h};
	for (uint64_t r0 = 0; r0 < n_reads && rc == KMR_OK; set ^= 1) {
		uint64_t r1 = r0 + 1;
		while (r1 < n_reads && offsets[r1 + 1] - offsets[r0] <= piece_bases) r1++;
		if (h->tb_set_used[set]) TBCHK(hipStreamWaitEvent(h->tb_copy_stream, h->tb_consumed[set], 0));
		{ int rcs = stage(set, r0, r1); if (rcs) return rcs; }
		TBCHK(hipEventRecord(h->tb_ready[set], h->tb_copy_stream));
		TBCHK(hipStreamWaitEvent(h->stream, h->tb_ready[set], 0));
		rc = feed(r0, r1);
		TBCHK(hipEventRecord(h->tb_consumed[set], h->stream)); h->tb_set_used[set] = true;
		r0 = r1;
	}
	hipStreamSynchronize(h->tb_copy_stream);
	if (!rc) rc = sync_state(h);
	else hipStreamSynchronize(h->stream);
	return rc;
}
extern "C" {

int kmr_add_reads(kmr_handle *h, const char *bases, const char *quals, const uint64_t *offsets, uint64_t n_reads,
                  uint64_t first_global_read_idx, const uint8_t *discarded) {
	if (!h) return KMR_ERR_INVALID_ARG;
	if (h->finalized) return fail(h, KMR_ERR_STATE, "kmr_add_reads after kmr_finalize");
	if (n_reads == 0) return KMR_OK;
	if (!bases || !offsets) return fail(h, KMR_ERR_INVALID_ARG, "null buffer");
	hipSetDevice(h->device);
	void *db = nullptr, *dq = nullptr, *doff = nullptr, *dd = nullptr;
	auto stage = [&](int set, uint64_t r0, uint64_t r1) -> int {
		const uint64_t m = r1 - r0, total = offsets[r1] - offsets[r0];
		dq = nullptr; dd = nullptr;
		TBCHK(tb_stage_copy(h, set, 0, bases + offsets[r0], total, &db)); TBCHK(tb_stage_copy(h, set, 2, offsets + r0, 8 * (m + 1), &doff));
		if (quals) TBCHK(tb_stage_copy(h, set, 6, quals + offsets[r0], total, &dq));
		if (discarded) TBCHK(tb_stage_copy(h, set, 7, discarded + r0, m, &dd));
		TBCHK(hipMemsetAsync((uint8_t *)db + total, 0, 64, h->tb_copy_stream)); if (dq) TBCHK(hipMemsetAsync((uint8_t *)dq + total, 0, 64, h->tb_copy_stream));
		return KMR_OK;
	};
	auto feed = [&](uint64_t r0, uint64_t r1) {
		return kmr_add_reads_dev(h, (uint8_t *)db - offsets[r0], dq ? (uint8_t *)dq - offsets[r0] : nullptr, doff, r1 - r0, offsets[r1] - offsets[r0], first_global_read_idx + r0, dd);
	};
	return tb_feed_pieces(h, offsets, n_reads, stage, feed);
}

static bool sk_packed_direct_ok(kmr_handle *h, bool has_quals, int uniform_quality) {
	if (!h->superkmer_mode || h->ext || h->cfg.size_tracker || h->tune.no_lean_extract || h->tune.no_packed_direct || sp_debug_extract(h) || has_quals || h->qual_mixed) return false;
	const DevParams dp = dev_params(h);
	if (dp.subsample > 1 || dp.num_parts > 1 || (dp.sub_wnb | dp.sub_snb) != 0 || (dp.world > 1 && !h->sk_exchange)) return false;
	return uniform_quality == 0 || uniform_quality == 127 || h->hP[uniform_quality] > 0.0;
}
int kmr_add_reads_twobit_dev(kmr_handle *h, const void *dev_twobit, const void *dev_twobit_offsets, const void *dev_offsets,
                             const void *dev_markup_offsets, const void *dev_markup_pos, const void *dev_markup_char,
                             const void *dev_quals, int uniform_quality, uint64_t n_reads, uint64_t total_bases,
                             uint64_t first_global_read_idx, const void *dev_discarded) {
	if (!h) return KMR_ERR_INVALID_ARG;
	if (h->finalized) return fail(h, KMR_ERR_STATE, "kmr_add_reads after kmr_finalize");
	if (n_reads == 0) return KMR_OK;
	if (!dev_twobit || !dev_offsets) return fail(h, KMR_ERR_INVALID_ARG, "null device buffer");
	if (dev_markup_offsets && (!dev_markup_pos || !dev_markup_char)) return fail(h, KMR_ERR_INVALID_ARG, "markup offsets without markups");
	if (uniform_quality < 0 || uniform_quality > 255 || (dev_quals && uniform_quality)) return fail(h, KMR_ERR_INVALID_ARG, "uniform_quality: 0, or the one quality character of a batch without a quality array");
	hipSetDevice(h->device);
	const bool direct = sk_packed_direct_ok(h, dev_quals != nullptr, uniform_quality);
	if (!direct && h->tb_bases.cap() < total_bases + 64) {
		if (h->tb_bases) HIPCHK(h, hipStreamSynchronize(h->stream));
		HIPCHK(h, h->tb_bases.alloc(total_bases + 64));
		HIPCHK(h, hipMemsetAsync(h->tb_bases.get<uint8_t>(), 0, total_bases + 64, h->stream));
	}
	if (h->tb_len.cap() < 4 * (n_reads + 1)) {
		if (h->tb_len) HIPCHK(h, hipStreamSynchronize(h->stream));
		h->tb_rel.reset(); h->tb_off.reset(); h->tb_len.reset();
		HIPCHK(h, h->tb_rel.alloc(8 * (n_reads + 1))); HIPCHK(h, h->tb_off.alloc(8 * (n_reads + 1))); HIPCHK(h, h->tb_len.alloc(4 * (n_reads + 1)));
	}
	const uint64_t *tboff = (const uint64_t *)dev_twobit_offsets;
	if (!tboff) {
		hipLaunchKernelGGL(twobit_bytes_kernel, dim3(grid_for(n_reads)), dim3(256), 0, h->stream, (const uint64_t *)dev_offsets, n_reads, h->tb_len.get<uint32_t>());
		HIPCHK(h, hipGetLastError());
		int rc = exclusive_scan(h, h->tb_len.get<uint32_t>(), n_reads, h->tb_off.get<uint64_t>()); if (rc) return rc;
		tboff = h->tb_off.get<uint64_t>();
	}
	if (direct) {
		hipLaunchKernelGGL(offsets_rel_kernel, dim3(grid_for(n_reads + 1)), dim3(256), 0, h->stream, (const uint64_t *)dev_offsets, n_reads, h->tb_rel.get<uint64_t>());
		HIPCHK(h, hipGetLastError());
		if (h->stream_base + total_bases > MAX_STREAM_ORDINAL) return fail(h, KMR_ERR_CAPACITY, "more than 2^40 input bases on one handle");
		const ReadsView rv = reads_view(nullptr, nullptr, h->tb_rel.get<uint64_t>(), n_reads, dev_discarded, h->stream_base, first_global_read_idx);
		SkPacked pkd; pkd.bytes = (const uint8_t *)dev_twobit; pkd.off = tboff; pkd.mk_off = (const uint64_t *)dev_markup_offsets; pkd.mk_pos = (const uint32_t *)dev_markup_pos; pkd.mk_char = (const uint8_t *)dev_markup_char;
		h->packed_direct = &pkd; h->uniform_q_hint = uniform_quality ? uniform_quality : -1;
		const int rc = add_reads_superkmer(h, rv, total_bases);
		h->packed_direct = nullptr; h->uniform_q_hint = -1;
		h->stream_base += total_bases; h->reads += n_reads; h->stats.reads = h->reads;
		return rc;
	}
	hipLaunchKernelGGL(twobit_unpack_kernel, dim3((unsigned)std::min<uint64_t>((n_reads + 255) / 256, (uint64_t)num_cus(h) * 32)), dim3(256), 0, h->stream,
	                   (const uint8_t *)dev_twobit, tboff, (const uint64_t *)dev_offsets, n_reads, h->tb_bases.get<uint8_t>(), h->tb_rel.get<uint64_t>());
	HIPCHK(h, hipGetLastError());
	if (dev_markup_offsets) {
		hipLaunchKernelGGL(twobit_markup_kernel, dim3(grid_for(n_reads)), dim3(256), 0, h->stream, (const uint64_t *)dev_markup_offsets, (const uint32_t *)dev_markup_pos,
		                   (const uint8_t *)dev_markup_char, (const uint64_t *)h->tb_rel.get<uint64_t>(), n_reads, h->tb_bases.get<uint8_t>());
		HIPCHK(h, hipGetLastError());
	}
	const void *q = dev_quals;
	if (!dev_quals && uniform_quality) {
		if (h->tb_quals.cap() < total_bases + 64) {
			if (h->tb_quals) HIPCHK(h, hipStreamSynchronize(h->stream));
			HIPCHK(h, h->tb_quals.alloc(total_bases + 64)); h->tb_quals_filled = 0; h->tb_quals_char = -1;
		}
		if (h->tb_quals_char != uniform_quality || h->tb_quals_filled < total_bases) {
			HIPCHK(h, hipMemsetAsync(h->tb_quals.get(), uniform_quality, h->tb_quals.cap(), h->stream));
			h->tb_quals_char = uniform_quality; h->tb_quals_filled = h->tb_quals.cap();
		}
		q = h->tb_quals.get<uint8_t>();
	}
	h->uniform_q_hint = (!dev_quals && uniform_quality) ? uniform_quality : -1;
	const int rc = kmr_add_reads_dev(h, h->tb_bases.get<uint8_t>(), q, h->tb_rel.get<uint64_t>(), n_reads, total_bases, first_global_read_idx, dev_discarded);
	h->uniform_q_hint = -1;
	return rc;
}

int kmr_add_reads_twobit(kmr_handle *h, const uint8_t *twobit, const uint64_t *twobit_offsets, const uint64_t *offsets,
                         const uint64_t *markup_offsets, const uint32_t *markup_pos, const char *markup_char,
                         const char *quals, int uniform_quality, uint64_t n_reads, uint64_t first_global_read_idx, const uint8_t *discarded) {
	if (!h) return KMR_ERR_INVALID_ARG;
	if (h->finalized) return fail(h, KMR_ERR_STATE, "kmr_add_reads after kmr_finalize");
	if (n_reads == 0) return KMR_OK;
	if (!twobit || !twobit_offsets || !offsets) return fail(h, KMR_ERR_INVALID_ARG, "null buffer");
	hipSetDevice(h->device);
	void *dtb = nullptr, *dto = nullptr, *doff = nullptr, *dmo = nullptr, *dmp = nullptr, *dmc = nullptr, *dq = nullptr, *dd = nullptr;
	auto stage = [&](int set, uint64_t r0, uint64_t r1) -> int {
		const uint64_t m = r1 - r0, total = offsets[r1] - offsets[r0], tbytes = twobit_offsets[r1] - twobit_offsets[r0];
		const uint64_t nm = markup_offsets ? markup_offsets[r1] - markup_offsets[r0] : 0;
		dmo = dmp = dmc = dq = dd = nullptr;
		TBCHK(tb_stage_copy(h, set, 0, twobit + twobit_offsets[r0], tbytes, &dtb)); TBCHK(tb_stage_copy(h, set, 1, twobit_offsets + r0, 8 * (m + 1), &dto)); TBCHK(tb_stage_copy(h, set, 2, offsets + r0, 8 * (m + 1), &doff));
		dtb = (uint8_t *)dtb - twobit_offsets[r0];
		if (nm) {
			TBCHK(tb_stage_copy(h, set, 3, markup_offsets + r0, 8 * (m + 1), &dmo)); TBCHK(tb_stage_copy(h, set, 4, markup_pos + markup_offsets[r0], 4 * nm, &dmp)); TBCHK(tb_stage_copy(h, set, 5, markup_char + markup_offsets[r0], nm, &dmc));
			dmp = (uint32_t *)dmp - markup_offsets[r0]; dmc = (uint8_t *)dmc - markup_offsets[r0];
// ... 1624 lines not shown
```

Measured before the change: 55.79 billion.

## Use pinned host read-back block and merge host synchronizations across build stages

Adds a pinned host block to the handle for all small device-to-host read-backs, replacing pageable hipMemcpy calls with async copies into pinned memory. It also removes or defers several stream synchronizations: the unit-length probe is issued early and shares the wait of the quality-range check, exclusive_scan can skip its sync inside build_csr, and the long-list item count is read alongside the count-pass counters rather than with its own sync. The aim is to cut host-device round trips and launch gaps in the superkmer build and finalize path, at the cost of more complex control flow around when pinned values become valid.

Result: no change. 56.15 billion (median of 6 runs) (+0.7%).

```diff
diff --git a/kmernator_amd/csrc/kmr_api.hip b/kmernator_amd/csrc/kmr_api.hip
--- a/kmernator_amd/csrc/kmr_api.hip
+++ b/kmernator_amd/csrc/kmr_api.hip
@@ -165,8 +165,15 @@
 	bool no_coarse_lists = true;
 };
 
+struct HostPin {
+	uint32_t err, cerr; unsigned int qrange[2], umax, mx;
+	unsigned long long hn, padded_total, cur[2];
+	DevStats stats; FinalizeCounters c;
+};
+
 struct kmr_handle : HandleMem, BuildMem, ExchangeMem {
 	kmr_config cfg;
+	HostPin *pin = nullptr;
 	Tuning tune;
 	uint32_t k = 0, kb = 0, hkb = 0, W = 0;
 	bool ext = false;
@@ -369,7 +376,10 @@
 }
 
 int sync_state(kmr_handle *h) {
+	HIPCHK(h, hipMemcpyAsync(&h->pin->err, h->derr.get<uint32_t>(), sizeof(uint32_t), hipMemcpyDeviceToHost, h->stream));
+	HIPCHK(h, hipMemcpyAsync(&h->pin->stats, h->dstats.get<DevStats>(), sizeof(DevStats), hipMemcpyDeviceToHost, h->stream));
 	HIPCHK(h, hipStreamSynchronize(h->stream));
+	const uint32_t e = h->pin->err; DevStats s = h->pin->stats;
 	for (int which = 0; which < KMR_TIME_GROUPS; which++) {
 		for (auto &pr : h->pending_events[which]) {
 			float ms = 0; hipEventElapsedTime(&ms, pr.first, pr.second);
@@ -378,9 +388,6 @@
 		}
 		h->pending_events[which].clear();
 	}
-	uint32_t e = 0; DevStats s;
-	HIPCHK(h, hipMemcpy(&e, h->derr.get<uint32_t>(), sizeof(e), hipMemcpyDeviceToHost));
-	HIPCHK(h, hipMemcpy(&s, h->dstats.get<DevStats>(), sizeof(s), hipMemcpyDeviceToHost));
 #ifdef KMR_DEBUG_HOOKS
 	if (h->superkmer_mode) { if (dbg()) fprintf(stderr, "sk_extract windows: %llu general, %llu fast\n", s.claimed, s.inserted); s.claimed = 0; s.inserted = 0; }
 #endif
@@ -434,10 +441,9 @@
 
 const size_t EXTRACT_SMEM = (size_t)WAVES_PER_BLOCK * 2 * TILE_BUF;
 
-int exclusive_scan(kmr_handle *h, const uint32_t *in, uint64_t n, uint64_t *out);
-
-int prepare_units(kmr_handle *h, ReadsView &rv, uint32_t span = (uint32_t)TILE_SPAN) {
-	rv.u_start = rv.u_end = rv.u_read = nullptr; rv.n_units = 0;
+int exclusive_scan(kmr_handle *h, const uint32_t *in, uint64_t n, uint64_t *out, bool wait = true);
+
+int units_probe(kmr_handle *h, const ReadsView &rv, uint32_t span) {
 	const uint64_t n = rv.n_reads;
 	if (n == 0) return 0;
 	int rc = h->umax.reserve(h, "umax", 4); if (rc) return rc;
@@ -445,9 +451,19 @@
 	rc = h->ucnt.reserve(h, "ucnt", 4 * (n + 1)); if (rc) return rc;
 	hipLaunchKernelGGL(unit_count_kernel, dim3(grid_for(n)), dim3(256), 0, h->stream, rv.offsets, n, h->k, span, h->ucnt.get<uint32_t>(), h->umax.get<unsigned int>());
 	HIPCHK(h, hipGetLastError());
-	unsigned int mx = 0;
-	HIPCHK(h, hipMemcpyAsync(&mx, h->umax.get<unsigned int>(), 4, hipMemcpyDeviceToHost, h->stream));
-	HIPCHK(h, hipStreamSynchronize(h->stream));
+	HIPCHK(h, hipMemcpyAsync(&h->pin->umax, h->umax.get<unsigned int>(), 4, hipMemcpyDeviceToHost, h->stream));
+	return 0;
+}
+int prepare_units(kmr_handle *h, ReadsView &rv, uint32_t span = (uint32_t)TILE_SPAN, bool probed = false) {
+	rv.u_start = rv.u_end = rv.u_read = nullptr; rv.n_units = 0;
+	const uint64_t n = rv.n_reads;
+	if (n == 0) return 0;
+	int rc = 0;
+	if (!probed) {
+		rc = units_probe(h, rv, span); if (rc) return rc;
+		HIPCHK(h, hipStreamSynchronize(h->stream));
+	}
+	const unsigned int mx = h->pin->umax;
 	if (mx <= span) return 0;
 	rc = h->ufirst.reserve(h, "ufirst", 8 * (n + 1)); if (rc) return rc;
 	rc = exclusive_scan(h, h->ucnt.get<uint32_t>(), n, h->ufirst.get<uint64_t>()); if (rc) return rc;
@@ -506,7 +522,7 @@
 
 int add_reads_dev_any(kmr_handle *h, const ReadsView &rv, uint64_t total_bases) { return with_w_ext(h, [&](auto W, auto EXT) { return add_reads_dev_t<W(), EXT()>(h, rv, total_bases); }); }
 
-int exclusive_scan(kmr_handle *h, const uint32_t *in, uint64_t n, uint64_t *out ) {
+int exclusive_scan(kmr_handle *h, const uint32_t *in, uint64_t n, uint64_t *out , bool wait) {
 	const uint64_t nblocks = (n + SCAN_ITEMS - 1) / SCAN_ITEMS;
 	const size_t eb = sizeof(unsigned long long);
 	int rc = h->scan_sums.reserve(h, "scan_sums", eb * (nblocks + 1), eb * std::max<uint64_t>(nblocks + 1, 4096)); if (rc) return rc;
@@ -515,7 +531,7 @@
 	hipLaunchKernelGGL(scan_sums_kernel, dim3(1), dim3(256), 0, h->stream, sums, nblocks, total);
 	hipLaunchKernelGGL(scan_apply_kernel, dim3((unsigned)nblocks), dim3(256), 0, h->stream, in, n, sums, out);
 	HIPCHK(h, hipGetLastError());
-	HIPCHK(h, hipStreamSynchronize(h->stream));
+	if (wait) HIPCHK(h, hipStreamSynchronize(h->stream));
 	return 0;
 }
 
@@ -975,7 +991,7 @@
 }
 int add_reads_partition(kmr_handle *h, const ReadsView &rv, uint64_t total_bases) { return with_w_ext(h, [&](auto W, auto EXT) { return add_reads_partition_t<W(), EXT()>(h, rv, total_bases); }); }
 
-int build_csr(kmr_handle *h, HostPool &p, uint64_t nl, uint32_t first, uint64_t **list_start, uint64_t **list_chunks, uint32_t *n_chunks_out) {
+int build_csr(kmr_handle *h, HostPool &p, uint64_t nl, uint32_t first, uint64_t **list_start, uint64_t **list_chunks, uint32_t *n_chunks_out, bool wait = true) {
 	unsigned int used = 0;
 	HIPCHK(h, hipStreamSynchronize(h->stream));
 	HIPCHK(h, hipMemcpy(&used, p.head.get<unsigned int>(), 4, hipMemcpyDeviceToHost));
@@ -987,7 +1003,7 @@
 	HIPCHK(h, hipMemsetAsync(cnt, 0, 4 * nl, h->stream));
 	const unsigned csr_grid = (unsigned)(((uint64_t)used + CSR_THREADS * CSR_ITEMS - 1) / (CSR_THREADS * CSR_ITEMS));
 	if (used) hipLaunchKernelGGL(chunk_hist_kernel, dim3(csr_grid), dim3(CSR_THREADS), 0, h->stream, p.chunk_list.get<uint32_t>() + first, used, cnt, (uint32_t)nl);
-	int rc = exclusive_scan(h, cnt, nl, *list_start); if (rc) return rc;
+	int rc = exclusive_scan(h, cnt, nl, *list_start, wait); if (rc) return rc;
 	HIPCHK(h, hipMemsetAsync(cnt, 0, 4 * nl, h->stream));
 	if (used) hipLaunchKernelGGL(chunk_scatter_kernel, dim3(csr_grid), dim3(CSR_THREADS), 0, h->stream, p.chunk_list.get<uint32_t>() + first, p.chunk_count.get<uint32_t>() + first, used, first, *list_start, cnt, *list_chunks, (uint32_t)nl);
 	HIPCHK(h, hipGetLastError());
@@ -1242,8 +1258,9 @@
 	unsigned int mx = 0;
 	if (!bits2) {
 		hipLaunchKernelGGL(bb_pad_kernel, dim3(grid_for(bins1)), dim3(256), 0, h->stream, (const uint32_t *)hist1, bins1, (uint32_t *)nullptr, dmax);
-		HIPCHK(h, hipMemcpyAsync(&mx, dmax, 4, hipMemcpyDeviceToHost, h->stream));
+		HIPCHK(h, hipMemcpyAsync(&h->pin->mx, dmax, 4, hipMemcpyDeviceToHost, h->stream));
 		rc = exclusive_scan(h, hist1, bins1, start1); if (rc) return rc;
+		mx = h->pin->mx;
 		if (mx > bb_group_cap<W>()) return 0;
 		rc = scratch(wn); if (rc) return rc;
 		hipLaunchKernelGGL(bb_cursor_init_kernel, dim3(grid_for(bins1)), dim3(256), 0, h->stream, (const uint64_t *)start1, bins1, cursor);
@@ -1253,9 +1270,9 @@
 		return 0;
 	}
 	hipLaunchKernelGGL(bb_pad_kernel, dim3(grid_for(bins1)), dim3(256), 0, h->stream, (const uint32_t *)hist1, bins1, pad1, dmax);
-	rc = exclusive_scan(h, pad1, bins1, start1); if (rc) return rc;
-	uint64_t padded_total = 0;
-	HIPCHK(h, hipMemcpy(&padded_total, start1 + bins1, 8, hipMemcpyDeviceToHost));
+	rc = exclusive_scan(h, pad1, bins1, start1, false); if (rc) return rc;
+	HIPCHK(h, hipMemcpyAsync(&h->pin->padded_total, start1 + bins1, 8, hipMemcpyDeviceToHost, h->stream)); HIPCHK(h, hipStreamSynchronize(h->stream));
+	const uint64_t padded_total = h->pin->padded_total;
 	rc = scratch(std::max(padded_total, wn)); if (rc) return rc;
 	hipLaunchKernelGGL(bb_cursor_init_kernel, dim3(grid_for(bins1)), dim3(256), 0, h->stream, (const uint64_t *)start1, bins1, cursor);
 	hipLaunchKernelGGL(bb_scatter_kernel<W>, dim3(scatter_grid(wslots)), dim3(BB_THREADS), 0, h->stream, in1, shift1, bits1, h->hkb, nb, cursor, h->ue2.get<uint64_t>());
@@ -1265,8 +1282,9 @@
 	grid = hist_grid(padded_total, tpb);
 	hipLaunchKernelGGL(bb_hist_kernel<W>, dim3(grid), dim3(BB_THREADS), 0, h->stream, in2, shift2, bits2, h->hkb, nb, tpb, hist2);
 	hipLaunchKernelGGL(bb_pad_kernel, dim3(grid_for(groups)), dim3(256), 0, h->stream, (const uint32_t *)hist2, groups, (uint32_t *)nullptr, dmax);
-	HIPCHK(h, hipMemcpyAsync(&mx, dmax, 4, hipMemcpyDeviceToHost, h->stream));
+	HIPCHK(h, hipMemcpyAsync(&h->pin->mx, dmax, 4, hipMemcpyDeviceToHost, h->stream));
 	rc = exclusive_scan(h, hist2, groups, gstart); if (rc) return rc;
+	mx = h->pin->mx;
 	if (mx > bb_group_cap<W>() || packed_entries(h, h->ue) < wn) return 0;
 	hipLaunchKernelGGL(bb_cursor_init_kernel, dim3(grid_for(groups)), dim3(256), 0, h->stream, (const uint64_t *)gstart, groups, cursor);
 	hipLaunchKernelGGL(bb_scatter_kernel<W>, dim3(scatter_grid(padded_total)), dim3(BB_THREADS), 0, h->stream, in2, shift2, bits2, h->hkb, nb, cursor, h->ue.get<uint64_t>());
@@ -1389,8 +1407,8 @@
 	HIPCHK(h, hipGetLastError());
 	return 0;
 }
-int sk_uniform_weight(kmr_handle *h, const ReadsView &rv, bool &lean, float &wK) {
-	lean = false; wK = 1.0f;
+int sk_uniform_weight(kmr_handle *h, const ReadsView &rv, bool &lean, float &wK, bool &waited) {
+	lean = false; wK = 1.0f; waited = false;
 	if (h->tune.no_lean_extract) return 0;
 	if (!rv.quals && h->uniform_q_hint < 0) { lean = true; return 0; }
 	if (h->qual_mixed || rv.n_reads == 0) return 0;
@@ -1406,9 +1424,10 @@
 	HIPCHK(h, hipMemcpyAsync(h->qrange.get<unsigned int>(), init, 8, hipMemcpyHostToDevice, h->stream));
 	hipLaunchKernelGGL(sk_qual_range_kernel, dim3(num_cus(h) * 8), dim3(256), 0, h->stream, rv.quals, rv.offsets, rv.n_reads, h->qrange.get<unsigned int>());
 	HIPCHK(h, hipGetLastError());
-	unsigned int got[2] = {0, 0};
-	HIPCHK(h, hipMemcpyAsync(got, h->qrange.get<unsigned int>(), 8, hipMemcpyDeviceToHost, h->stream));
+	HIPCHK(h, hipMemcpyAsync(h->pin->qrange, h->qrange.get<unsigned int>(), 8, hipMemcpyDeviceToHost, h->stream));
 	HIPCHK(h, hipStreamSynchronize(h->stream));
+	const unsigned int got[2] = {h->pin->qrange[0], h->pin->qrange[1]};
+	waited = true;
 	if (got[0] != got[1]) { h->qual_mixed = got[0] < got[1]; return 0; }
 	const unsigned int q0 = got[0];
 	if (q0 == 127) { lean = true; wK = 1.0f; return 0; }
@@ -1429,7 +1448,13 @@
 	const DevParams dp = dev_params(h);
 	const bool filt = dp.subsample > 1 || dp.num_parts > 1 || (dp.sub_wnb | dp.sub_snb) != 0 || (dp.world > 1 && !h->sk_exchange);
 	bool lean = false; float wK = 1.0f;
-	if (!filt && !h->ext && !sp_debug_extract(h)) { int rcq = sk_uniform_weight(h, rvAll, lean, wK); if (rcq) return rcq; }
+	const uint64_t avg = n ? std::max<uint64_t>(1, total_bases / n) : 1;
+	const uint64_t sub_bases = h->tune.sub_batch_bases ? h->tune.sub_batch_bases : (1ull << 31);
+	const uint64_t chunk = std::max<uint64_t>(64, (sub_bases / avg) & ~63ull);
+	const uint32_t unit_span = h->packed_direct ? SK_PACKED_SPAN : (uint32_t)TILE_SPAN;
+	bool probed = false, waited = false;
+	if (n && n <= chunk) { int rcu = units_probe(h, rvAll, unit_span); if (rcu) return rcu; probed = true; }
+	if (!filt && !h->ext && !sp_debug_extract(h)) { int rcq = sk_uniform_weight(h, rvAll, lean, wK, waited); if (rcq) return rcq; }
 	if (h->packed_direct && (!lean || h->cfg.size_tracker)) return fail(h, KMR_ERR_STATE, "internal: a packed batch handed to an extraction that wants text");
 	if (rvAll.n_reads) {
 		uint32_t wb; memcpy(&wb, &wK, 4);
@@ -1457,9 +1482,6 @@
 		hipLaunchKernelGGL(sk_state_init_kernel, dim3(grid_for(nl0)), dim3(256), 0, h->stream, h->sk_state.get<unsigned long long>(), nl0);
 		HIPCHK(h, hipGetLastError());
 	}
-	const uint64_t avg = n ? std::max<uint64_t>(1, total_bases / n) : 1;
-	const uint64_t sub_bases = h->tune.sub_batch_bases ? h->tune.sub_batch_bases : (1ull << 31);
-	const uint64_t chunk = std::max<uint64_t>(64, (sub_bases / avg) & ~63ull);
 	if (h->cfg.size_tracker && n) {
 		h->trk_n = 0;
 		{ int rc = h->trk.reserve(h, "trk", n * sizeof(SkTrackRec)); if (rc) return rc; }
@@ -1468,7 +1490,8 @@
 	for (uint64_t r = 0; r < n; r += chunk) {
 		const uint64_t m = std::min(chunk, n - r);
 		ReadsView rv = reads_slice(rvAll, r, m);
-		int rc = prepare_units(h, rv, h->packed_direct ? SK_PACKED_SPAN : (uint32_t)TILE_SPAN); if (rc) return rc;
+		if (probed && !waited) { HIPCHK(h, hipStreamSynchronize(h->stream)); waited = true; }
+		int rc = prepare_units(h, rv, unit_span, probed); if (rc) return rc;
 		const uint64_t bases = m * avg + avg;
 		if (!h->l1.base && r == 0 && h->cfg.world_size <= 1 && !h->sk_exchange && (h->cfg.estimated_raw_kmers || h->call_bases_hint > total_bases)) {
 			const double job_bases = h->cfg.estimated_raw_kmers ? (double)h->cfg.estimated_raw_kmers * (double)avg / (double)(avg > h->k ? avg - h->k + 1 : 1) : (double)h->call_bases_hint;
@@ -1684,6 +1707,7 @@
 	uint32_t *wc = nullptr, *sc = nullptr; FinalizeCounters *fc = nullptr; unsigned long long *cursors = nullptr;
 	SkTrackView tv{};
 	SkLong<W> lgMain{}, lgItems{}; uint64_t n_items = 0;
+	bool items_pending = false; unsigned long long *items_dn = nullptr; uint64_t items_cap = 0;
 	uint64_t early_slots = 0; FinalizeCounters early_c{};
 	FinalizeCounters c{}; unsigned long long cur[2] = {0, 0};
 };
@@ -1771,7 +1795,7 @@
 	return 0;
 }
 template <int W> int sk_long_items(kmr_handle *h, SkFinalize<W> &p) {
-	p.lgItems = p.lgMain; p.n_items = 0;
+	p.lgItems = p.lgMain; p.n_items = 0; p.items_pending = false;
 	const uint64_t LONG_CHUNKS = p.ext ? std::min<uint64_t>(h->tune.long_list_chunks ? h->tune.long_list_chunks : SK_EXT_LONG_CHUNKS, SK_EXT_LONG_CHUNKS) : (h->tune.long_list_chunks ? h->tune.long_list_chunks : 1024), PIECE = std::max<uint64_t>(1, LONG_CHUNKS / 2);
 	if (p.tracking || p.nch <= LONG_CHUNKS) return 0;
 	const uint64_t cap = (uint64_t)p.nch / PIECE + 2 * 1024 + 16;
@@ -1780,14 +1804,9 @@
 	HIPCHK(h, hipMemsetAsync(dn, 0, 8, h->stream));
 	hipLaunchKernelGGL(sk_long_items_kernel, dim3(grid_for(p.nl)), dim3(256), 0, h->stream, p.ls, p.nl, LONG_CHUNKS, PIECE, ic0, ic1, cap, dn);
 	HIPCHK(h, hipGetLastError());
-	unsigned long long hn = 0;
-	HIPCHK(h, hipMemcpyAsync(&hn, dn, 8, hipMemcpyDeviceToHost, h->stream)); HIPCHK(h, hipStreamSynchronize(h->stream));
-	if (hn > cap) return fail(h, KMR_ERR_CAPACITY, "long-list work items (internal sizing error)");
-	p.n_items = hn;
-	if (p.n_items) {
-		p.lgMain.long_threshold = LONG_CHUNKS;
-		p.lgItems.item_c0 = ic0; p.lgItems.item_c1 = ic1; p.lgItems.n_items = p.n_items; p.lgItems.merge_used = dn;
-	}
+	p.lgMain.long_threshold = LONG_CHUNKS;
+	p.lgItems.item_c0 = ic0; p.lgItems.item_c1 = ic1; p.lgItems.merge_used = dn;
+	p.items_pending = true; p.items_dn = dn; p.items_cap = cap;
 	return 0;
 }
 CountOut count_out(kmr_handle *h, bool packed, unsigned long long *cursors, uint32_t *wc, uint32_t *sc, FinalizeCounters *fc) {
@@ -1802,7 +1821,7 @@
 template <int W> int sk_count_pass(kmr_handle *h, SkFinalize<W> &p, bool &overflowed) {
 	overflowed = false;
 	const bool ext = p.ext, keepSing = p.keepSing, tracking = p.tracking; const uint32_t vw = ext ? 15 : 3;
-	uint64_t &wcap = p.wcap, &scap = p.scap; const uint64_t wmax = p.wmax, smax = p.smax, nl = p.nl, n_items = p.n_items;
+	uint64_t &wcap = p.wcap, &scap = p.scap; const uint64_t wmax = p.wmax, smax = p.smax, nl = p.nl; uint64_t &n_items = p.n_items;
 	uint32_t *wc = p.wc, *sc = p.sc; FinalizeCounters *fc = p.fc; unsigned long long *cursors = p.cursors;
 	FinalizeCounters &c = p.c; unsigned long long *cur = p.cur; const SkTrackView &tv = p.tv; const FinalizeParams &f = p.f;
 	int rc = 0;
@@ -1830,7 +1849,27 @@
 		hipLaunchKernelGGL(k.kern, dim3(grid), dim3(SKC_THREADS), k.smem, h->stream, pool_view(h, h->l1), p.ls, p.lc, nl, h->k, out, f, h->work_counter.get<unsigned int>(), sk_dbg_flags("KMR_SK_COUNT_DBG"), tv, p.lgMain);
 		HIPCHK(h, hipGetLastError());
 		DevBuf mslots, mext;
+		uint32_t cerr = 0;
+		auto read_back = [&]() -> int {
+			HostPin *pin = h->pin;
+			HIPCHK(h, hipMemcpyAsync(&pin->c, fc, sizeof(c), hipMemcpyDeviceToHost, h->stream)); HIPCHK(h, hipMemcpyAsync(pin->cur, cursors, 16, hipMemcpyDeviceToHost, h->stream));
+			HIPCHK(h, hipMemcpyAsync(&pin->cerr, h->derr.get<uint32_t>(), 4, hipMemcpyDeviceToHost, h->stream));
+			HIPCHK(h, hipStreamSynchronize(h->stream));
+			c = pin->c; cur[0] = pin->cur[0]; cur[1] = pin->cur[1]; cerr = pin->cerr;
+			return 0;
+		};
+		bool fresh = false;
+		if (p.items_pending) {
+			HIPCHK(h, hipMemcpyAsync(&h->pin->hn, p.items_dn, 8, hipMemcpyDeviceToHost, h->stream));
+			rc = read_back(); if (rc) return rc;
+			const unsigned long long hn = h->pin->hn;
+			p.items_pending = false;
+			if (hn > p.items_cap) { time_end(h, KMR_TIME_COUNT, tca, tcb); return fail(h, KMR_ERR_CAPACITY, "long-list work items (internal sizing error)"); }
+			n_items = hn; p.lgItems.n_items = hn;
+			fresh = true;
+		}
 		if (n_items) {
+			fresh = false;
 			SkLong<W> &lgItems = p.lgItems;
 			if (mslots.alloc(sizeof(Slot<W>) << merge_log2) != hipSuccess) return fail(h, KMR_ERR_OOM, "merge table of the long lists");
 			if (ext && mext.alloc(sizeof(ExtSlot) << merge_log2) != hipSuccess) return fail(h, KMR_ERR_OOM, "merge table of the long lists");
@@ -1843,10 +1882,7 @@
 			hipLaunchKernelGGL(sk_merge_emit_kernel<W>, dim3(grid_for(1ull << merge_log2)), dim3(256), 0, h->stream, lgItems.merge, out, f);
 			if (hipGetLastError() != hipSuccess) return fail(h, KMR_ERR_HIP, "long-list launches");
 		}
-		uint32_t cerr = 0;
-		HIPCHK(h, hipMemcpyAsync(&c, fc, sizeof(c), hipMemcpyDeviceToHost, h->stream)); HIPCHK(h, hipMemcpyAsync(cur, cursors, 16, hipMemcpyDeviceToHost, h->stream));
-		HIPCHK(h, hipMemcpyAsync(&cerr, h->derr.get<uint32_t>(), 4, hipMemcpyDeviceToHost, h->stream));
-		HIPCHK(h, hipStreamSynchronize(h->stream));
+		if (!fresh) { rc = read_back(); if (rc) return rc; }
 		if (n_items && (cerr & ERR_TABLE_FULL) && merge_log2 < 30) {
 			cerr &= ~(uint32_t)(ERR_TABLE_FULL | ERR_ENTRIES_FULL);
 			HIPCHK(h, hipMemcpy(h->derr.get<uint32_t>(), &cerr, 4, hipMemcpyHostToDevice));
@@ -1898,7 +1934,7 @@
 	}
 	p.refined = h->sk_state && h->sk_fine_shift > 0;
 	if (p.refined) { rc = sk_refine_lists(h, p.nl); if (rc) return rc; }
-	rc = build_csr(h, h->l1, p.nl, 0, &p.ls, &p.lc, &p.nch); if (rc) return rc;
+	rc = build_csr(h, h->l1, p.nl, 0, &p.ls, &p.lc, &p.nch, false); if (rc) return rc;
 	rc = sk_entry_buffers<W>(h, p, h->stats.raw_good_kmers); if (rc) return rc;
 	rc = sk_count_uniform<W>(h, p.tracking, p.uni, p.f.uni_wbits); if (rc) return rc;
 	h->last_count_uniform = p.uni;
@@ -2030,6 +2066,8 @@
 		if (cfg->device >= 0) { if (hipSetDevice(cfg->device) != hipSuccess) { rc = fail(nullptr, KMR_ERR_NO_DEVICE, "hipSetDevice failed"); break; } }
 		if (hipGetDevice(&h->device) != hipSuccess) { rc = fail(nullptr, KMR_ERR_NO_DEVICE, "hipGetDevice failed"); break; }
 		if (hipStreamCreate(&h->stream) != hipSuccess) { rc = fail(nullptr, KMR_ERR_HIP, "hipStreamCreate failed"); break; }
+		if (hipHostMalloc((void **)&h->pin, sizeof(HostPin), hipHostMallocDefault) != hipSuccess) { h->pin = nullptr; rc = fail(nullptr, KMR_ERR_HIP, "hipHostMalloc of the read-back block failed"); break; }
+		memset(h->pin, 0, sizeof(HostPin));
 		uint64_t w = cfg->num_buckets_weak, s = cfg->num_buckets_singleton;
 		const double depth = cfg->estimated_depth > 0 ? cfg->estimated_depth : 20.0;
 		const uint32_t kpb = cfg->kmers_per_bucket ? cfg->kmers_per_bucket : 32;
@@ -2091,6 +2129,7 @@
 	exchange_destroy_comm(h);
 	release<ExchangeMem>(h);
 	if (h->stream) hipStreamDestroy(h->stream);
+	if (h->pin) hipHostFree(h->pin);
 	delete h;
 }
 
```
